# DLR-RB/QUEASARS

Hardware: AMD Instinct MI355X
Metric: circuit-evals/sec (EVQE population) at n qubits; achieved HBM GB/s vs roofline (higher is better)
Workload: dtype f64; 1 GPU; 20-qubit EVQE population=64 per GPU, 4 layers, random Ising Hamiltonian (210 terms), fp64 (BASELINE.json configs[1]); n_qubits=20, population_per_gpu=64, layers=4, pauli_terms=210, parallelism=1 GPU

## Files before the change

include/qsv.h:

```cpp
#ifndef QSV_H
#define QSV_H

#include <stddef.h>
#include <stdint.h>

#ifdef __cplusplus
extern "C" {
#endif

typedef struct qsv_handle qsv_t;

enum { QSV_OP_ID = 0, QSV_OP_U = 1, QSV_OP_CU3 = 2 };
enum { QSV_F64 = 0, QSV_F32 = 1 };
enum { QSV_NO_CONTROL = 0xFF };

enum {
    QSV_OK = 0,
    QSV_E_ARG = -1,
    QSV_E_DEVICE = -2,
    QSV_E_STATE = -3,
    QSV_E_UNSUPPORTED = -4
};

typedef struct qsv_op {
    uint8_t kind;
    uint8_t target;
    uint8_t control;
    uint8_t flags;
    int32_t p_theta, p_phi, p_lambda;
    double theta, phi, lambda;
} qsv_op;

typedef struct qsv_plan_config {
    int32_t tile_bits;
    int32_t reg_bits;
    int32_t low_bits;
    int32_t group;
    int32_t exchange;
} qsv_plan_config;

typedef struct qsv_profile {
    uint64_t n_evals;
    uint64_t n_pass_launches;
    uint64_t n_state_passes;
    uint64_t n_gates;
    uint64_t state_bytes;
    double pass_ms;
    double expect_ms;
    double total_ms;
    double pass_window_ms;
    uint64_t moved_bytes;
    uint64_t kernel_launches[3];
    double kernel_ms[3];
    uint64_t kernel_bytes[3];
    uint64_t kernel_moved_bytes[3];
    double kernel_flops[3];
    uint64_t kernel_states[3];
} qsv_profile;


int qsv_create(int n_qubits, int dtype, int device, const qsv_plan_config* cfg , qsv_t** out);
void qsv_destroy(qsv_t* h);
const char* qsv_last_error(const qsv_t* h);
int qsv_set_stream(qsv_t* h, void* hip_stream);
int qsv_n_qubits(const qsv_t* h);


int qsv_set_operator(qsv_t* h, int n_terms, const uint64_t* x_mask, const uint64_t* z_mask,
                     const double* coeff_re, const double* coeff_im);


int qsv_circuit_create(qsv_t* h, int n_ops, const qsv_op* ops, int n_params, int* out_circuit_id);
int qsv_circuits_create(qsv_t* h, int n_circuits, const int64_t* op_offsets, const qsv_op* ops, const int* n_params,
                        int* out_circuit_ids);
int qsv_circuit_destroy(qsv_t* h, int circuit_id);

int qsv_prefix_create(qsv_t* h, int n_states, const int* circuit_ids, const int64_t* param_offsets, const double* params,
                      int* out_prefix_ids);
int qsv_prefix_destroy(qsv_t* h, int n_states, const int* prefix_ids);
int qsv_prefix_count(const qsv_t* h);
int qsv_circuit_create_on_prefix(qsv_t* h, int prefix_id, int n_ops, const qsv_op* ops, int n_params, int* out_circuit_id);
int qsv_circuits_create_on_prefixes(qsv_t* h, int n_circuits, const int64_t* op_offsets, const qsv_op* ops, const int* n_params,
                                    const int* prefix_ids, int* out_circuit_ids);

enum { QSV_ROUTE_ONE_TILE = 0, QSV_ROUTE_SPLIT_ONE_LAUNCH = 1, QSV_ROUTE_SPLIT = 2, QSV_ROUTE_PASSES = 3 };
typedef struct qsv_circuit_cost_t {
    int32_t route;
    int32_t n_keys;
    int32_t n_passes;
    int32_t on_kept_state;
    double microseconds;
} qsv_circuit_cost_t;
int qsv_circuit_cost(qsv_t* h, int circuit_id, qsv_circuit_cost_t* out);

typedef struct qsv_circuit_form_t {
    int32_t route;
    int32_t n_keys;
    int32_t n_virtual[2];
    int32_t amps_per_thread;
    int32_t halves;
    int32_t outer[2];
    int32_t one_launch;
    int32_t split_sampled;
    uint32_t mask_x, mask_y;
} qsv_circuit_form_t;
int qsv_circuit_form(qsv_t* h, int circuit_id, qsv_circuit_form_t* out);
int qsv_circuit_launch_form(qsv_t* h, int circuit_id, qsv_circuit_form_t* out);

int qsv_eval_circuits(qsv_t* h, int n_evals, const int* circuit_ids, const int64_t* param_offsets,
                      const double* params, double* out_expectations);

int qsv_eval_coalesced(qsv_t* h, int circuit_id, const double* params, int n_params, double window_us,
                       double* out_expectation);

int qsv_eval_begin(qsv_t* h, int n_evals, const int* circuit_ids, const int64_t* param_counts);
int qsv_eval_push(qsv_t* h, int first, int count, const double* values);
int qsv_eval_staging(qsv_t* h, int first, int count, double** values);
int qsv_eval_push_device(qsv_t* h, int first, int count, const double* device_values, void* ready_event);
int qsv_eval_end(qsv_t* h, double* out_expectations);
int qsv_eval_set_output(qsv_t* h, double* device_out);
int qsv_eval_results_seen(qsv_t* h);
typedef struct qsv_spsa_step_args {
    int32_t n_runs, width;
    double* x;
    uint8_t* active;
    int64_t* iterations;
    const double* delta_accept;
    const double* values;
    const double* delta_propose;
    double* points;
    double eps, lr;
    int32_t trust_region, maxiter;
    int32_t window;
    int32_t reserved;
    double min_rel;
    int64_t maxfev;
    double* previous;
    int64_t* n_values;
    double* changes;
} qsv_spsa_step_args;
int qsv_spsa_step(qsv_t* h, const qsv_spsa_step_args* args);
typedef struct qsv_nft_step_args {
    int32_t n_runs, width;
    int32_t columns_stride;
    int32_t reserved;
    double* x;
    const int32_t* sizes;
    const int32_t* columns;
    double* recycled;
    int32_t accept, accept_with_base;
    int64_t accept_iteration;
    int32_t propose, propose_with_base;
    int64_t propose_iteration;
    const double* values;
    double* points;
} qsv_nft_step_args;
int qsv_nft_step(qsv_t* h, const qsv_nft_step_args* args);
typedef struct qsv_adam_step_args {
    int32_t n_runs, width;
    int32_t columns_stride, grad_width;
    double* x;
    const int32_t* sizes;
    const int32_t* columns;
    double* m;
    double* v;
    const double* gradient;
    uint8_t* active;
    int64_t* iterations;
    double lr, beta_1, beta_2, one_minus_beta_1, one_minus_beta_2, eps, tol;
    double bias_1, bias_2;
    int64_t maxiter;
} qsv_adam_step_args;
int qsv_adam_step(qsv_t* h, const qsv_adam_step_args* args);
int qsv_eval_suggested_pushes(const qsv_t* h);
int qsv_group_size(const qsv_t* h);

int qsv_eval_batch(qsv_t* h, int n_evals, const int64_t* op_offsets, const qsv_op* ops,
                   const int64_t* param_offsets, const double* params, double* out_expectations);

int qsv_statevector(qsv_t* h, int circuit_id, const double* params, int n_params, double* out_re_im);

int qsv_probabilities(qsv_t* h, int circuit_id, const double* params, int n_params, double* out_probs);

int qsv_sample(qsv_t* h, int circuit_id, const double* params, int n_params, int shots, uint64_t seed,
               uint64_t* out_states);

int qsv_sample_batch(qsv_t* h, int n_evals, const int* circuit_ids, const int64_t* param_offsets, const double* params,
                     int shots, uint64_t seed, uint64_t* out_states, double* out_values );

int qsv_sample_cvar_batch(qsv_t* h, int n_evals, const int* circuit_ids, const int64_t* param_offsets, const double* params,
// ... 138 lines not shown
```

queasars_amd/_build.py:

```python

from __future__ import annotations

import os
import shutil
import subprocess
from pathlib import Path

PKG_DIR = Path(__file__).resolve().parent
CSRC = PKG_DIR / "csrc"
LIB_PATH = PKG_DIR / "libqsv.so"
PYHELP_PATH = PKG_DIR / "_qsvpyhelp.so"
SOURCES = ["kernels.hip", "qsv_api.hip", "plan.cpp", "split.cpp", "sort.hip", "gradient.hip", "value_cache.hip", "adjoint.hip", "adjoint_plan.cpp", "moments.hip", "covariance.hip", "overlap.hip"]
HEADERS = ["kernels.hpp", "plan.hpp", "split.hpp", "gradient.hpp", "value_cache.hpp", "adjoint.hpp", "adjoint_plan.hpp", "moments.hpp", "covariance.hpp", "overlap.hpp", "operator_row.hpp", "gate_loop_gen.inc", "../../include/qsv.h"]
ARCH = "gfx950"


def _hipcc() -> str:
    for cand in (os.environ.get("HIPCC"), shutil.which("hipcc"), "/opt/rocm/bin/hipcc"):
        if cand and Path(cand).exists():
            return cand
    raise RuntimeError("hipcc not found; libqsv cannot be built")


def have_hipcc() -> bool:
    try:
        _hipcc()
        return True
    except RuntimeError:
        return False


def pyhelp_stale() -> bool:
    src = CSRC / "pyhelp.c"
    return not PYHELP_PATH.exists() or PYHELP_PATH.stat().st_mtime < src.stat().st_mtime


def build_pyhelp(force: bool = False) -> "Path | None":
    import sysconfig

    src = CSRC / "pyhelp.c"
    if (PYHELP_PATH.exists() and not force and PYHELP_PATH.stat().st_mtime >= src.stat().st_mtime
            and (not LIB_PATH.exists() or PYHELP_PATH.stat().st_mtime >= LIB_PATH.stat().st_mtime)):
        return PYHELP_PATH
    include = sysconfig.get_paths().get("include")
    gcc = shutil.which("gcc")
    if not gcc or not include or not (Path(include) / "Python.h").exists():
        return None
    tmp = PYHELP_PATH.with_suffix(f".so.{os.getpid()}.tmp")
    if not LIB_PATH.exists():
        return None
    res = subprocess.run([gcc, "-O2", "-shared", "-fPIC", f"-I{include}", str(src), "-o", str(tmp), f"-L{PKG_DIR}", "-lqsv",
                          "-Wl,-rpath,$ORIGIN"], stdout=subprocess.PIPE, stderr=subprocess.STDOUT, text=True)
    if res.returncode != 0:
        tmp.unlink(missing_ok=True)
        return None
    os.replace(tmp, PYHELP_PATH)
    return PYHELP_PATH


def needs_build() -> bool:
    if not LIB_PATH.exists():
        return True
    built = LIB_PATH.stat().st_mtime
    return any((CSRC / f).resolve().stat().st_mtime > built for f in SOURCES + HEADERS)


def build(force: bool = False, verbose: bool = False, defines: tuple = (), lib_path: Path = LIB_PATH) -> Path:
    if not force and not defines and not needs_build():
        build_pyhelp(False)
        return LIB_PATH
    obj_dir = PKG_DIR / ("build" if not defines else "build_" + "".join(c if c.isalnum() else "_" for c in "_".join(defines).lower()))
    obj_dir.mkdir(exist_ok=True)
    hipcc = _hipcc()
    common = [f"--offload-arch={ARCH}", "-O3", "-std=c++17", "-fPIC", "-Wall", "-Wno-unused-function"]
    common += [f"-D{d}" for d in defines]
    procs = []
    objs = []
    for src in SOURCES:
        obj = obj_dir / (src + ".o")
        objs.append(str(obj))
        cmd = [hipcc, *common, "-c", str(CSRC / src), "-o", str(obj)]
        if src.endswith(".cpp"):
            cmd.insert(1, "-x")
            cmd.insert(2, "hip")
        if verbose:
            print(" ".join(cmd))
        procs.append((src, subprocess.Popen(cmd, stdout=subprocess.PIPE, stderr=subprocess.STDOUT, text=True)))
    for src, proc in procs:
        out, _ = proc.communicate()
        if proc.returncode != 0:
            raise RuntimeError(f"hipcc failed on {src}:\n{out}")
        if verbose and out.strip():
            print(out)
    tmp = lib_path.with_suffix(f".so.{os.getpid()}.tmp")
    link = [hipcc, f"--offload-arch={ARCH}", "-shared", "-fPIC", "-o", str(tmp), *objs]
    res = subprocess.run(link, stdout=subprocess.PIPE, stderr=subprocess.STDOUT, text=True)
    if res.returncode != 0:
        raise RuntimeError(f"link failed:\n{res.stdout}")
    os.replace(tmp, lib_path)
    if not defines:
        build_pyhelp(True)
    return lib_path


if __name__ == "__main__":
    print(build(force=True, verbose=True))
```

queasars_amd/_lib.py:

```python

from __future__ import annotations

import ctypes as C
import os
import threading
from pathlib import Path

import numpy as np

from queasars_amd import _build

QSV_OK, QSV_E_ARG, QSV_E_DEVICE, QSV_E_STATE, QSV_E_UNSUPPORTED = 0, -1, -2, -3, -4
QSV_F64, QSV_F32 = 0, 1


class QsvOp(C.Structure):
    _fields_ = [
        ("kind", C.c_uint8),
        ("target", C.c_uint8),
        ("control", C.c_uint8),
        ("flags", C.c_uint8),
        ("p_theta", C.c_int32),
        ("p_phi", C.c_int32),
        ("p_lambda", C.c_int32),
# ... 126 lines not shown
    _fields_ = [
        ("route", C.c_int32),
        ("n_keys", C.c_int32),
        ("n_virtual", C.c_int32 * 2),
        ("amps_per_thread", C.c_int32),
        ("halves", C.c_int32),
        ("outer", C.c_int32 * 2),
        ("one_launch", C.c_int32),
        ("split_sampled", C.c_int32),
        ("mask_x", C.c_uint32),
        ("mask_y", C.c_uint32),
    ]


class QsvGradientStats(C.Structure):

    _fields_ = [
        ("n_shifted", C.c_int64),
        ("n_chunks", C.c_int64),
        ("n_allocations", C.c_int64),
        ("scratch_bytes", C.c_int64),
    ]


class QsvGradientPlanStats(C.Structure):

    _fields_ = [
        ("n_shifted", C.c_int64),
        ("n_chunks", C.c_int64),
        ("n_runs", C.c_int64),
        ("n_host_waits", C.c_int64),
        ("table_bytes", C.c_int64),
    ]


class QsvAdjointStats(C.Structure):

    _fields_ = [
        ("n_gates", C.c_int64),
        ("n_runs", C.c_int64),
        ("n_state_sweeps", C.c_int64),
        ("scratch_bytes", C.c_int64),
        ("n_allocations", C.c_int64),
    ]


class QsvValueCacheStats(C.Structure):

    _fields_ = [
        ("entries", C.c_int64),
        ("slots", C.c_int64),
        ("samples_looked_up", C.c_int64),
        ("hits", C.c_int64),
        ("new_entries", C.c_int64),
        ("rehashes", C.c_int64),
        ("clears", C.c_int64),
    ]


ROUTE_NAMES = ("one tile", "split, one launch", "split", "gate passes")

assert C.sizeof(QsvOp) == 40

_P = C.c_void_p
SIGNATURES = {
    "qsv_version": (C.c_char_p, []),
    "qsv_create": (C.c_int, [C.c_int, C.c_int, C.c_int, C.POINTER(QsvPlanConfig), C.POINTER(_P)]),
    "qsv_destroy": (None, [_P]),
    "qsv_last_error": (C.c_char_p, [_P]),
    "qsv_set_stream": (C.c_int, [_P, _P]),
    "qsv_n_qubits": (C.c_int, [_P]),
    "qsv_set_operator": (C.c_int, [_P, C.c_int, _P, _P, _P, _P]),
    "qsv_circuit_create": (C.c_int, [_P, C.c_int, _P, C.c_int, C.POINTER(C.c_int)]),
    "qsv_circuits_create": (C.c_int, [_P, C.c_int, _P, _P, _P, _P]),
    "qsv_circuit_destroy": (C.c_int, [_P, C.c_int]),
    "qsv_prefix_create": (C.c_int, [_P, C.c_int, _P, _P, _P, _P]),
    "qsv_prefix_destroy": (C.c_int, [_P, C.c_int, _P]),
    "qsv_prefix_count": (C.c_int, [_P]),
    "qsv_circuit_create_on_prefix": (C.c_int, [_P, C.c_int, C.c_int, _P, C.c_int, C.POINTER(C.c_int)]),
    "qsv_circuits_create_on_prefixes": (C.c_int, [_P, C.c_int, _P, _P, _P, _P, _P]),
    "qsv_circuit_cost": (C.c_int, [_P, C.c_int, C.POINTER(QsvCircuitCost)]),
    "qsv_circuit_form": (C.c_int, [_P, C.c_int, C.POINTER(QsvCircuitForm)]),
    "qsv_circuit_launch_form": (C.c_int, [_P, C.c_int, C.POINTER(QsvCircuitForm)]),
    "qsv_eval_circuits": (C.c_int, [_P, C.c_int, _P, _P, _P, _P]),
    "qsv_eval_coalesced": (C.c_int, [_P, C.c_int, _P, C.c_int, C.c_double, C.POINTER(C.c_double)]),
    "qsv_eval_begin": (C.c_int, [_P, C.c_int, _P, _P]),
    "qsv_eval_push": (C.c_int, [_P, C.c_int, C.c_int, _P]),
    "qsv_eval_staging": (C.c_int, [_P, C.c_int, C.c_int, C.POINTER(_P)]),
    "qsv_eval_push_device": (C.c_int, [_P, C.c_int, C.c_int, _P, _P]),
    "qsv_spsa_step": (C.c_int, [_P, _P]),
    "qsv_nft_step": (C.c_int, [_P, _P]),
    "qsv_adam_step": (C.c_int, [_P, _P]),
    "qsv_eval_end": (C.c_int, [_P, _P]),
    "qsv_eval_set_output": (C.c_int, [_P, _P]),
    "qsv_eval_results_seen": (C.c_int, [_P]),
    "qsv_eval_suggested_pushes": (C.c_int, [_P]),
    "qsv_group_size": (C.c_int, [_P]),
    "qsv_eval_batch": (C.c_int, [_P, C.c_int, _P, _P, _P, _P, _P]),
    "qsv_statevector": (C.c_int, [_P, C.c_int, _P, C.c_int, _P]),
    "qsv_probabilities": (C.c_int, [_P, C.c_int, _P, C.c_int, _P]),
    "qsv_sample": (C.c_int, [_P, C.c_int, _P, C.c_int, C.c_int, C.c_uint64, _P]),
    "qsv_sample_batch": (C.c_int, [_P, C.c_int, _P, _P, _P, C.c_int, C.c_uint64, _P, _P]),
    "qsv_sample_cvar_batch": (C.c_int, [_P, C.c_int, _P, _P, _P, C.c_int, C.c_uint64, C.c_double, _P]),
    "qsv_exact_cvar_batch": (C.c_int, [_P, C.c_int, _P, _P, _P, C.c_double, _P]),
    "qsv_top_states": (C.c_int, [_P, C.c_int, _P, _P, _P, C.c_int, _P, _P, _P]),
    "qsv_cvar_device": (C.c_int, [_P, C.c_int, _P, C.c_int, _P, _P, C.c_int, C.c_uint64, C.c_double, _P, C.c_int, _P]),
    "qsv_value_cache_create": (C.c_int, [_P, C.c_int, C.c_int, _P]),
    "qsv_value_cache_destroy": (C.c_int, [_P, C.c_int]),
    "qsv_value_cache_clear": (C.c_int, [_P, C.c_int]),
    "qsv_value_cache_stats": (C.c_int, [_P, C.c_int, _P]),
    "qsv_sample_lookup": (C.c_int, [_P, C.c_int, C.c_int, _P, _P, _P, C.c_int, C.c_uint64, _P, _P]),
    "qsv_sample_lookup_finish": (C.c_int, [_P, C.c_int, C.c_int64, _P, C.c_double, _P, _P]),
    "qsv_gradient_describe": (C.c_int, [C.c_int, _P, C.c_int, _P]),
    "qsv_gradient_circuits": (C.c_int, [_P, C.c_int, _P, _P, _P, _P, _P, _P, _P]),
    "qsv_gradient_device": (C.c_int, [_P, C.c_int, _P, C.c_int, _P, _P, _P, _P, C.c_int, _P, _P]),
    "qsv_gradient_stats": (C.c_int, [_P, C.POINTER(QsvGradientStats)]),
    "qsv_gradient_plan_create": (C.c_int, [_P, C.c_int, _P, C.c_int, _P, _P, C.c_int, C.POINTER(C.c_int), C.POINTER(C.c_int64)]),
    "qsv_gradient_plan_run": (C.c_int, [_P, C.c_int, _P, _P, _P]),
    "qsv_gradient_plan_destroy": (C.c_int, [_P, C.c_int]),
    "qsv_gradient_plan_stats": (C.c_int, [_P, C.c_int, C.POINTER(QsvGradientPlanStats)]),
    "qsv_adjoint_describe": (C.c_int, [C.c_int, C.c_int, _P, C.c_int, C.c_int, _P, C.c_int, _P, _P, _P, C.POINTER(C.c_int64),
                                       C.POINTER(C.c_int32), C.POINTER(C.c_int32)]),
    "qsv_adjoint_gradient_circuits": (C.c_int, [_P, C.c_int, _P, _P, _P, _P, _P, _P, _P]),
    "qsv_adjoint_gradient_device": (C.c_int, [_P, C.c_int, _P, C.c_int, _P, _P, _P, _P, C.c_int, _P, _P]),
    "qsv_adjoint_stats": (C.c_int, [_P, C.POINTER(QsvAdjointStats)]),
    "qsv_variance_circuits": (C.c_int, [_P, C.c_int, _P, _P, _P, _P, _P]),
    "qsv_observables_covariance": (C.c_int, [_P, C.c_int, C.c_int, _P, _P, _P, _P, _P]),
    "qsv_overlap_circuits": (C.c_int, [_P, C.c_int, _P, C.c_int, C.c_int, _P, _P, _P, _P, _P]),
    "qsv_observables_create": (C.c_int, [_P, C.c_int, _P, _P, _P, _P, _P, C.POINTER(C.c_int)]),
    "qsv_observables_destroy": (C.c_int, [_P, C.c_int]),
    "qsv_eval_observables": (C.c_int, [_P, C.c_int, C.c_int, _P, _P, _P, _P]),
    "qsv_set_option": (C.c_int, [_P, C.c_char_p, C.c_int]),
    "qsv_fitness_table_wait": (C.c_int, [C.c_void_p, C.c_int, C.c_void_p, C.c_int, C.c_int, C.c_int, C.c_int64, C.c_int]),
    "qsv_replayed_pushes": (C.c_longlong, [_P]),
    "qsv_live_entries": (C.c_int, [C.c_int, C.c_uint, C.POINTER(C.c_int)]),
    "qsv_set_profiling": (C.c_int, [_P, C.c_int]),
    "qsv_get_profile": (C.c_int, [_P, C.POINTER(QsvProfile)]),
    "qsv_bench_gate": (C.c_int, [_P, C.c_int, C.c_int, C.c_double, C.c_double, C.c_double, C.c_int, C.POINTER(C.c_double)]),
    "qsv_bench_ops": (C.c_int, [_P, C.c_int, _P, C.c_int, C.POINTER(C.c_double), C.POINTER(C.c_int)]),
    "qsv_split_describe": (
        C.c_int,
        [C.c_int, C.c_int, _P, C.c_int, C.POINTER(C.c_uint64), _P, C.c_int, C.POINTER(C.c_int), _P, C.c_int, C.POINTER(C.c_int)],
    ),
    "qsv_split_describe_reduced": (
        C.c_int,
        [C.c_int, C.c_int, _P, C.c_int, C.POINTER(C.c_uint64), _P, C.c_int, C.POINTER(C.c_int), _P, C.c_int, C.POINTER(C.c_int),
         _P, _P, _P, _P],
    ),
    "qsv_plan_build": (
        C.c_int,
        [C.c_int, C.c_int, C.c_int, _P, C.POINTER(QsvPlanConfig), _P, C.c_size_t, C.POINTER(C.c_size_t)],
    ),
}

_lock = threading.Lock()
_lib = None


class QsvLibraryError(RuntimeError):
    """libqsv is missing or could not be loaded.  There is deliberately no fallback."""


def library_path() -> Path:
    override = os.environ.get("QSV_LIBRARY")
    return Path(override) if override else _build.LIB_PATH

# ... 38 lines not shown
```

queasars_amd/circuit_evaluation/circuit_evaluation.py:

```python

from __future__ import annotations

import ctypes as C
import os
import threading
import uuid
import weakref
from collections import OrderedDict
from itertools import count
from abc import ABC, abstractmethod
from typing import Optional, Sequence

from array import array

import numpy as np

from queasars_amd import _lib
from queasars_amd.circuit_evaluation.bitstring_evaluation import BitstringEvaluator
from queasars_amd.circuit_evaluation.expectation_calculation import (
    get_expectation_with_bitstring_evaluator,
    get_expectation_with_operator,
)
from queasars_amd.ir import OP_ID, QSV_OP_DTYPE, CircuitIR, PauliOperator

# ... 411 lines not shown
        for c in fresh:
            if c.n_qubits != self._n_qubits:
                raise ValueError(f"circuit has {c.n_qubits} qubits, the evaluator {self._n_qubits}")
        with self._reg_lock:
            fresh = [c for c in fresh if self._serial not in c._registered]
            continued = [c for c in fresh if c._kept_state is not None]
            if continued:
                fresh = [c for c in fresh if c._kept_state is None]
                if len(continued) >= 2:
                    self._register_continued(continued)
            if len(fresh) < 2:
                return
            joined = b"".join([c._bytes for c in fresh])
            ops = np.frombuffer(joined, dtype=QSV_OP_DTYPE) if joined else np.zeros(1, dtype=QSV_OP_DTYPE)
            offsets = np.zeros(len(fresh) + 1, dtype=np.int64)
            np.cumsum([len(c._bytes) for c in fresh], out=offsets[1:])
            offsets //= QSV_OP_DTYPE.itemsize
            counts = np.asarray([c.num_parameters for c in fresh], dtype=np.int32)
            out = np.zeros(len(fresh), dtype=np.int32)
            self._check(self._lib.qsv_circuits_create(self._handle, len(fresh), _lib.as_ptr(offsets), _lib.as_ptr(ops),
                                                      _lib.as_ptr(counts), _lib.as_ptr(out)))
            for c, cid in zip(fresh, out.tolist()):
                c._registered[self._serial] = cid
                self._watch(c, cid)

    def _register_continued(self, circuits: Sequence[CircuitIR]) -> None:
        joined = b"".join([c._bytes for c in circuits])
        ops = np.frombuffer(joined, dtype=QSV_OP_DTYPE) if joined else np.zeros(1, dtype=QSV_OP_DTYPE)
        offsets = np.zeros(len(circuits) + 1, dtype=np.int64)
        np.cumsum([len(c._bytes) for c in circuits], out=offsets[1:])
        offsets //= QSV_OP_DTYPE.itemsize
        counts = np.asarray([c.num_parameters for c in circuits], dtype=np.int32)
        states = np.asarray([self._kept_id(c._kept_state) for c in circuits], dtype=np.int32)
        out = np.zeros(len(circuits), dtype=np.int32)
        self._check(self._lib.qsv_circuits_create_on_prefixes(self._handle, len(circuits), _lib.as_ptr(offsets), _lib.as_ptr(ops),
                                                              _lib.as_ptr(counts), _lib.as_ptr(states), _lib.as_ptr(out)))
        for c, cid in zip(circuits, out.tolist()):
            c._registered[self._serial] = cid
            self._watch(c, cid)

    def _kept_id(self, kept: "KeptState") -> int:
        if kept._serial != self._serial or kept._id < 0:
            raise ValueError("the circuit continues a state that is not kept on this device (or was released)")
        return kept._id

    def keep_states(self, circuits: Sequence[CircuitIR], parameter_values: Sequence[Sequence[float]]) -> list[KeptState]:
        n = len(circuits)
        if len(parameter_values) != n:
            raise ValueError("circuits and parameter_values must have the same length")
        if n == 0:
            return []
        if any(c._kept_state is not None for c in circuits):
            raise ValueError("a kept state of a circuit that itself continues a kept state is not supported")
        self._register_many([c for c in circuits if self._serial not in c._registered])
        ids = np.fromiter((self.circuit_id(c) for c in circuits), dtype=np.int32, count=n)
        offsets, flat = _pack_batch(parameter_values, np.fromiter((c.num_parameters for c in circuits), dtype=np.int64, count=n))
        out = np.zeros(n, dtype=np.int32)
        with self._reg_lock:
            self._reap()
        self._check(self._lib.qsv_prefix_create(self._handle, n, _lib.as_ptr(ids), _lib.as_ptr(offsets), _lib.as_ptr(flat), _lib.as_ptr(out)))
        return [KeptState(self, pid) for pid in out.tolist()]

    def forget_last_batch(self) -> None:
        self._last_batch = None
        self._row_counts = None
        self._ids_address = None

    def kept_state_count(self) -> int:
        with self._reg_lock:
            self._reap()
        return int(self._lib.qsv_prefix_count(self._handle))

    def circuit_cost(self, circuit: CircuitIR) -> dict:
        cost = _lib.QsvCircuitCost()
        self._check(self._lib.qsv_circuit_cost(self._handle, self.circuit_id(circuit), C.byref(cost)))
        return {"route": _lib.ROUTE_NAMES[cost.route], "n_keys": cost.n_keys, "n_passes": cost.n_passes,
                "on_kept_state": bool(cost.on_kept_state), "microseconds": cost.microseconds}

    def circuit_form(self, circuit: CircuitIR) -> dict:
        return self._form(self._lib.qsv_circuit_form, circuit)

    def circuit_launch_form(self, circuit: CircuitIR) -> dict:
        return self._form(self._lib.qsv_circuit_launch_form, circuit)

    def _form(self, call, circuit: CircuitIR) -> dict:
        form = _lib.QsvCircuitForm()
        self._check(call(self._handle, self.circuit_id(circuit), C.byref(form)))
        return {"route": form.route, "n_keys": form.n_keys, "n_virtual": tuple(form.n_virtual),
                "amps_per_thread": form.amps_per_thread, "halves": bool(form.halves), "outer": tuple(form.outer),
                "one_launch": bool(form.one_launch), "split_sampled": bool(form.split_sampled), "mask_x": form.mask_x,
                "mask_y": form.mask_y}

    def _watch(self, circuit: CircuitIR, cid: int) -> None:
        ref = weakref.ref(circuit, self._gone)
        self._watched[id(ref)] = (ref, cid)

    def _reap(self) -> None:
        while self._dead:
            cid = self._dead.pop()
            if self._handle:
                self._lib.qsv_circuit_destroy(self._handle, cid)
        while self._dead_states:
            pid = C.c_int(self._dead_states.pop())
            if self._handle:
                self._lib.qsv_prefix_destroy(self._handle, 1, C.byref(pid))

    def _batch_metadata(self, circuits: Sequence[CircuitIR]) -> tuple[np.ndarray, np.ndarray, int]:
        n = len(circuits)
        cached = self._last_batch
        if cached is not None and cached[0][0] == CircuitIR.edits_of_registered:
            fast = _load_pyhelp_module()
            if fast is not None:
                if fast.same_objects(cached[1], circuits):
                    return cached[2], cached[3], cached[4]
            elif cached[0] == (CircuitIR.edits_of_registered, *map(id, circuits)):
                return cached[2], cached[3], cached[4]
        if self._dead or self._dead_states:
            with self._reg_lock:
                self._reap()
        self._register_many([c for c in circuits if self._serial not in c._registered])
        ids = np.fromiter((self.circuit_id(c) for c in circuits), dtype=np.int32, count=n)
        need = np.fromiter((c.num_parameters for c in circuits), dtype=np.int64, count=n)
        total = int(need.sum())
        self._last_batch = ((CircuitIR.edits_of_registered, *map(id, circuits)), list(circuits), ids, need, total)
        return ids, need, total

    def _batch_arguments(self, circuits: Sequence[CircuitIR], parameter_values: Sequence[Sequence[float]]) -> tuple[np.ndarray, np.ndarray, np.ndarray]:
        ids, need, _ = self._batch_metadata(circuits)
        return (ids, *_pack_batch(parameter_values, need))

    def results_seen(self) -> None:
        self._check(self._lib.qsv_eval_results_seen(self._handle))

    def expectation_values_to_device(
        self, circuits: Sequence[CircuitIR], parameter_values: Sequence[Sequence[float]], device_pointer: int
    ) -> None:
        n = len(circuits)
        if len(parameter_values) != n:
            raise ValueError("circuits and parameter_values must have the same length")
        if n == 0:
            return
        ids, need, total = self._batch_metadata(circuits)
        helper = None if os.environ.get("QSV_LIBRARY") else _load_pyhelp()
        if helper is not None:
            scratch = np.empty(total + 1, dtype=np.float64)
            self._check(helper.qsv_py_expectation_values_device(self._handle, n, ids.ctypes.data, need.ctypes.data,
                                                                parameter_values, scratch.ctypes.data, total,
                                                                C.c_void_p(device_pointer)))
            return
        counts = np.fromiter(map(len, parameter_values), dtype=np.int64, count=n)
        if (counts < need).any():
            i = int(np.argmax(counts < need))
            raise ValueError(f"circuit {i} needs {int(need[i])} parameter values, got {int(counts[i])}")
        lib, handle = self._lib, self._handle
        self._check(lib.qsv_eval_begin(handle, n, _lib.as_ptr(ids), _lib.as_ptr(counts)))
        rc = lib.qsv_eval_set_output(handle, C.c_void_p(device_pointer))
        if rc == _lib.QSV_OK:
            packed = _pack_slice(parameter_values, 0, n, int(counts.sum()))
            rc = lib.qsv_eval_push(handle, 0, n, _lib.as_ptr(packed))
        rc_end = lib.qsv_eval_end(handle, None)
        self._check(rc if rc != _lib.QSV_OK else rc_end)

    def expectation_values_of_device_parameters(
        self,
        circuits: Sequence[CircuitIR],
        device_pointer: int,
# ... 1332 lines not shown
```

queasars_amd/csrc/gen_gate_loop.py:

```python
#!/usr/bin/env python3

from __future__ import annotations

import sys
from pathlib import Path

OUT = Path(__file__).resolve().parent / "gate_loop_gen.inc"

import os

ABL = set(filter(None, os.environ.get("QSV_GEN_ABL", "").split(",")))

AMP0 = 8


def amp_re(e: int) -> str:
    return f"v[{AMP0 + 4 * e}:{AMP0 + 4 * e + 1}]"


def amp_im(e: int) -> str:
    return f"v[{AMP0 + 4 * e + 2}:{AMP0 + 4 * e + 3}]"


def amp_operands(nr: int) -> list[str]:
    outs = []
    for e in range(nr):
        outs.append(f'"+{{{amp_re(e)}}}"(amp[{e}].re)')
        outs.append(f'"+{{{amp_im(e)}}}"(amp[{e}].im)')
    return outs


MAT = {"A": 40, "B": 56}
DESC = {"A": 72, "B": 76}
SAVE = "s[80:81]"
T0 = "s82"
TP = "s[82:83]"
BASEP = "s[96:97]"
RP, MP, N = 84, 86, 88
CLOBBER_RANGE = list(range(40, 89)) + [96, 97]


def sreg2(base: int) -> str:
    return f"s[{base}:{base + 1}]"


def gate(lines: list[str], r: int, x: str, tag: str) -> None:
    m, d = MAT[x], DESC[x]
    w0, ct, cg = f"s{d}", f"s{d + 1}", f"s{d + 2}"
    cgpair = sreg2(d + 2)
    m00, m00i, m01r, m01i = sreg2(m), sreg2(m + 2), sreg2(m + 4), sreg2(m + 6)
    m10r, m10i, m11r, m11i = sreg2(m + 8), sreg2(m + 10), sreg2(m + 12), sreg2(m + 14)
    e = lines.append
    e(f"s_and_b64 {TP}, {BASEP}, {cgpair}")
    e(f"s_cmp_eq_u64 {TP}, {cgpair}")
    e(f"s_cbranch_scc0 Lskip{tag}_%=")
    e(f"v_and_b32 %[vt], {ct}, %[tid]")
    e(f"v_cmp_eq_u32 vcc, {ct}, %[vt]")
    e(f"s_and_saveexec_b64 {SAVE}, vcc")
    e(f"s_cbranch_execz Lrest{tag}_%=")
    e(f"s_bitcmp1_b32 {w0}, 24")
    e(f"s_cbranch_scc1 Lgen{tag}_%=")
    for general in (False, True):
        x = "g" if general else ""
        if general:
            e(f"Lgen{tag}_%=:")
        if r > 1:
            e(f"s_and_b32 {T0}, {w0}, 0xff")
            for j in range(r - 1):
                e(f"s_cmp_eq_u32 {T0}, {j}")
                e(f"s_cbranch_scc1 Lj{x}{j}{tag}_%=")
        order = [r - 1] + list(range(r - 1))
        for pos, j in enumerate(order):
            if j != r - 1:
                e(f"Lj{x}{j}{tag}_%=:")
            pair = 0
            for e0 in range(1 << r):
                if e0 & (1 << j):
                    continue
                e1 = e0 | (1 << j)
                a0r, a0i, a1r, a1i = amp_re(e0), amp_im(e0), amp_re(e1), amp_im(e1)
                if "pairtest" not in ABL:
                    e(f"s_bitcmp1_b32 {w0}, {16 + pair}")
                    e(f"s_cbranch_scc0 Ln{x}{j}_{pair}{tag}_%=")
                if "gatevalu" not in ABL:
                    e(f"v_mul_f64 %[p], {m10r}, {a0r}")
                    e(f"v_mul_f64 %[q], {m10r}, {a0i}")
                    e(f"v_mul_f64 %[u], {m00}, {a0r}")
                    e(f"v_mul_f64 %[w], {m00}, {a0i}")
                    e(f"v_fma_f64 %[p], -{m10i}, {a0i}, %[p]")
                    e(f"v_fma_f64 %[q], {m10i}, {a0r}, %[q]")
                    if general:
                        e(f"v_fma_f64 %[u], -{m00i}, {a0i}, %[u]")
                        e(f"v_fma_f64 %[w], {m00i}, {a0r}, %[w]")
                        e(f"v_fma_f64 %[p], {m11r}, {a1r}, %[p]")
                        e(f"v_fma_f64 %[q], {m11i}, {a1r}, %[q]")
                    e(f"v_fma_f64 %[u], {m01r}, {a1r}, %[u]")
                    e(f"v_fma_f64 %[w], {m01r}, {a1i}, %[w]")
                    if not general:
                        e(f"v_fma_f64 %[p], {m11r}, {a1r}, %[p]")
                        e(f"v_fma_f64 %[q], {m11i}, {a1r}, %[q]")
                    e(f"v_fma_f64 {a0r}, -{m01i}, {a1i}, %[u]")
                    e(f"v_fma_f64 {a0i}, {m01i}, {a1r}, %[w]")
                    e(f"v_fma_f64 {a1r}, -{m11i}, {a1i}, %[p]")
                    e(f"v_fma_f64 {a1i}, {m11r}, {a1i}, %[q]")
                e(f"Ln{x}{j}_{pair}{tag}_%=:")
                pair += 1
            if not (general and pos + 1 == len(order)):
                e(f"s_branch Lrest{tag}_%=")
    e(f"Lrest{tag}_%=:")
    e(f"s_mov_b64 exec, {SAVE}")
    e(f"Lskip{tag}_%=:")


def loop_body(r: int) -> list[str]:
    rp, mp = sreg2(RP), sreg2(MP)
    lines: list[str] = []
    e = lines.append
    e(f"s_mov_b64 {rp}, %[rp]")
    e(f"s_mov_b64 {mp}, %[mp]")
    e(f"s_mov_b32 s{N}, %[n]")
    e("s_mov_b32 s96, %[base]")
    e("s_not_b32 s97, %[base]")
    gate_loop_core(lines, r)
    return lines


def gate_loop_core(lines: list[str], r: int) -> None:
    a, b = MAT["A"], MAT["B"]
    da, db = DESC["A"], DESC["B"]
    rp, mp = sreg2(RP), sreg2(MP)
    n = f"s{N}"
    e = lines.append
    e(f"s_load_dwordx4 s[{da}:{da + 3}], {rp}, 0x0")
    e(f"s_load_dwordx16 s[{a}:{a + 15}], {mp}, 0x0")
    e("Lloop_%=:")
    e("s_waitcnt lgkmcnt(0)")
    e(f"s_load_dwordx4 s[{db}:{db + 3}], {rp}, 0x10")
    e(f"s_load_dwordx16 s[{b}:{b + 15}], {mp}, 0x40")
    gate(lines, r, "A", "a")
    e(f"s_sub_u32 {n}, {n}, 1")
    e(f"s_cmp_eq_u32 {n}, 0")
    e("s_cbranch_scc1 Ldone_%=")
    e("s_waitcnt lgkmcnt(0)")
    e(f"s_load_dwordx4 s[{da}:{da + 3}], {rp}, 0x20")
    e(f"s_load_dwordx16 s[{a}:{a + 15}], {mp}, 0x80")
    gate(lines, r, "B", "b")
    e(f"s_add_u32 s{RP}, s{RP}, 32")
    e(f"s_addc_u32 s{RP + 1}, s{RP + 1}, 0")
    e(f"s_add_u32 s{MP}, s{MP}, 128")
    e(f"s_addc_u32 s{MP + 1}, s{MP + 1}, 0")
    e(f"s_sub_u32 {n}, {n}, 1")
    e(f"s_cmp_lg_u32 {n}, 0")
    e("s_cbranch_scc1 Lloop_%=")
    e("Ldone_%=:")
    e("s_waitcnt lgkmcnt(0)")


def emit(r: int) -> str:
    nr = 1 << r
    out = []
    out.append(f"// R = {r}: {nr} amplitudes per thread")
    out.append("template <>")
    out.append(f"struct GateLoopF64<{r}> {{")
    out.append(
        f"    static __device__ __forceinline__ void run(cx<double> (&amp)[{nr}], cu32p rp, cf64p mp,\n"
        "                                               uint32_t n_gates, uint32_t base, uint32_t tid) {"
    )
    out.append("        // uniform by construction; say so to the compiler, which otherwise may hand a VGPR to an \"s\" operand")
    out.append("        base = __builtin_amdgcn_readfirstlane(base);")
    out.append("        n_gates = __builtin_amdgcn_readfirstlane(n_gates);")
    out.append("        double u, w, p, q;")
    out.append("        uint32_t vt;")
    out.append("        asm volatile(")
    for line in loop_body(r):
        out.append(f'            "{line}\\n\\t"')
    outs = amp_operands(nr)
    outs += ['[u] "=&v"(u)', '[w] "=&v"(w)', '[p] "=&v"(p)', '[q] "=&v"(q)', '[vt] "=&v"(vt)']
    out.append("            : " + ",\n              ".join(outs))
    out.append('            : [rp] "s"(rp), [mp] "s"(mp), [n] "s"(n_gates), [base] "s"(base), [tid] "v"(tid)')
    clob = ['"vcc"', '"scc"'] + [f'"s{i}"' for i in CLOBBER_RANGE]
    rows = [", ".join(clob[i : i + 12]) for i in range(0, len(clob), 12)]
    out.append("            : " + ",\n              ".join(rows) + ");")
    out.append("    }")
    out.append("};")
    return "\n".join(out)


def swap_case(lines: list[str], r: int, v: int, u: int) -> None:
    e = lines.append
    pairs = [(e0, e0 | (1 << v)) for e0 in range(1 << r) if not e0 & (1 << v)]
    regs = [(f"v{AMP0 + 4 * a + d}", f"v{AMP0 + 4 * b + d}") for a, b in pairs for d in range(4)]
    e("s_nop 1")
    if "swapvalu" in ABL:
        return
    if u >= 4:
        op = "v_permlane32_swap_b32" if u == 5 else "v_permlane16_swap_b32"
        for a, b in regs:
            e(f"{op} {a}, {b}")
    elif u >= 2:
        n = 1 << u
        upper, lower = ("0xa", "0x5") if u == 2 else ("0xc", "0x3")
        for i in range(0, len(regs), 2):
            chunk = regs[i : i + 2]
            temps = ["%[t0]", "%[t1]"]
            for (a, _b), t in zip(chunk, temps):
                e(f"v_mov_b32 {t}, {a}")
            for (a, b), _t in zip(chunk, temps):
                e(f"v_mov_b32_dpp {a}, {b} row_shr:{n} row_mask:0xf bank_mask:{upper}")
            for (_a, b), t in zip(chunk, temps):
                e(f"v_mov_b32_dpp {b}, {t} row_shl:{n} row_mask:0xf bank_mask:{lower}")
    else:
        perm = "quad_perm:[1,0,3,2]" if u == 0 else "quad_perm:[2,3,0,1]"
        e(f"v_and_b32 %[t0], {1 << u}, %[lane]")
        e("v_cmp_ne_u32 vcc, 0, %[t0]")
        for i in range(0, len(regs), 2):
            chunk = regs[i : i + 2]
            temps = ["%[t0]", "%[t1]"]
            for (_a, b), t in zip(chunk, temps):
                e(f"v_mov_b32_dpp {t}, {b} {perm} row_mask:0xf bank_mask:0xf")
            for (a, b), _t in zip(chunk, temps):
                e(f"v_cndmask_b32_dpp {b}, {a}, {b}, vcc {perm} row_mask:0xf bank_mask:0xf")
            for (a, _b), t in zip(chunk, temps):
                e(f"v_cndmask_b32 {a}, {a}, {t}, vcc")


def dispatch_tree(lines: list[str], lo: int, hi: int, labels: list[str], tag: str) -> None:
    if hi - lo == 1:
        lines.append(f"s_branch {labels[lo]}")
        return
    mid = (lo + hi) // 2
    lines.append(f"s_cmp_lt_u32 %[sel], {mid}")
    lines.append(f"s_cbranch_scc1 Lt{tag}{lo}_{mid}_%=")
    dispatch_tree(lines, mid, hi, labels, tag)
    lines.append(f"Lt{tag}{lo}_{mid}_%=:")
    dispatch_tree(lines, lo, mid, labels, tag)


def emit_swap(r: int) -> str:
    nr = 1 << r
    lines: list[str] = []
    e = lines.append
    cases = [(v, u) for v in range(r) for u in range(6)]
    labels = [f"Lc{v}_{u}_%=" for v, u in cases]
    dispatch_tree(lines, 0, len(cases), labels, "s")
    for (v, u), label in zip(cases, labels):
        e(f"{label}:")
        swap_case(lines, r, v, u)
        e("s_branch Lend_%=")
    e("Lend_%=:")
    out = []
    out.append(f"// R = {r}: lane swap of the {nr} amplitudes of a thread, both component planes (sel = 6 V + U < {6 * r})")
    out.append("template <>")
    out.append(f"struct SwapF64<{r}> {{")
    out.append(f"    static __device__ __forceinline__ void run(cx<double> (&amp)[{nr}], uint32_t sel, uint32_t lane) {{")
    out.append("        sel = __builtin_amdgcn_readfirstlane(sel);")
    out.append("        uint32_t t0, t1;")
    out.append("        asm volatile(")
    for line in lines:
        out.append(f'            "{line}\\n\\t"')
    outs = amp_operands(nr) + ['[t0] "=&v"(t0)', '[t1] "=&v"(t1)']
    out.append("            : " + ",\n              ".join(outs))
    out.append('            : [sel] "s"(sel), [lane] "v"(lane)')
    out.append('            : "vcc", "scc");')
    out.append("    }")
    out.append("};")
    return "\n".join(out)


RH, ROUNDS, FLAGS, T1, T2, T3 = 89, 90, 91, 83, 92, 93
SAVE2 = "s[94:95]"
NEXT_RP, NEXT_MP = "s[92:93]", "s[94:95]"
ROUND_CLOBBERS = range(40, 98)
WC, RC = 40, 56
K_THREAD_COLS = 9


def emit_rounds(r: int) -> str:
    nr = 1 << r
    rp, mp = sreg2(RP), sreg2(MP)
    lines: list[str] = []
    e = lines.append
    e(f"s_mov_b64 {rp}, %[rp]")
    e(f"s_mov_b64 {mp}, %[mp]")
    e(f"s_mov_b32 s{ROUNDS}, %[rounds]")
    e(f"s_mov_b32 s{FLAGS}, %[flags]")
    e("s_mov_b32 s96, %[base]")
    e("s_not_b32 s97, %[base]")
    e("Lround_%=:")
    e(f"s_load_dword s{RH}, {rp}, 0x0")
    e("s_waitcnt lgkmcnt(0)")
    e(f"s_bitcmp1_b32 s{RH}, 16")
    e("s_cbranch_scc1 Lexch_%=")
    e(f"s_bitcmp1_b32 s{RH}, 18")
    e("s_cbranch_scc1 Lswap_%=")
    e(f"s_add_u32 s{RP}, s{RP}, 4")
    e(f"s_addc_u32 s{RP + 1}, s{RP + 1}, 0")
    e("Lgates_%=:")
    e(f"s_and_b32 s{N}, s{RH}, 0xffff")
    e(f"s_cmp_eq_u32 s{N}, 0")
    e("s_cbranch_scc1 Lnext_%=")
    e(f"s_lshl_b32 s{T1}, s{N}, 4")
    e(f"s_add_u32 s92, s{RP}, s{T1}")
    e(f"s_addc_u32 s93, s{RP + 1}, 0")
    e(f"s_lshl_b32 s{T1}, s{N}, 6")
    e(f"s_add_u32 s94, s{MP}, s{T1}")
    e(f"s_addc_u32 s95, s{MP + 1}, 0")
    if "gateloop" not in ABL:
        gate_loop_core(lines, r)
    e(f"s_mov_b64 {rp}, {NEXT_RP}")
    e(f"s_mov_b64 {mp}, {NEXT_MP}")
    e("Lnext_%=:")
    e(f"s_sub_u32 s{ROUNDS}, s{ROUNDS}, 1")
    e(f"s_cmp_lg_u32 s{ROUNDS}, 0")
    e("s_cbranch_scc1 Lround_%=")
    e("s_branch Lfinish_%=")

    e("Lswap_%=:")
    e(f"s_load_dwordx4 s[40:43], {rp}, 0x4")
    e(f"s_add_u32 s{RP}, s{RP}, 20")
    e(f"s_addc_u32 s{RP + 1}, s{RP + 1}, 0")
    e("s_waitcnt lgkmcnt(0)")
    e("Lswapnext_%=:")
    e("s_cmp_eq_u32 s40, -1")
    e("s_cbranch_scc1 Lgates_%=")
    e(f"s_and_b32 {T0}, s40, 0xff")
    e(f"s_mul_i32 {T0}, {T0}, 6")
    e(f"s_bfe_u32 s{T1}, s40, 0x80008")
    e(f"s_add_u32 {T0}, {T0}, s{T1}")
    cases = [(v, u) for v in range(r) for u in range(6)]
    labels = [f"Lc{v}_{u}_%=" for v, u in cases]
    tree: list[str] = []
    dispatch_tree(tree, 0, len(cases), labels, "r")
    lines.extend(x.replace("%[sel]", T0) for x in tree)
    for (v, u), label in zip(cases, labels):
        e(f"{label}:")
        swap_case(lines, r, v, u)
        e("s_branch Lswapdone_%=")
    e("Lswapdone_%=:")
    e("s_mov_b32 s40, s41")
    e("s_mov_b32 s41, s42")
    e("s_mov_b32 s42, s43")
    e("s_mov_b32 s43, -1")
    e("s_branch Lswapnext_%=")

    e("Lexch_%=:")
    for base, off in ((WC, 4), (RC, 4 + 52)):
        e(f"s_load_dwordx8 s[{base}:{base + 7}], {rp}, {hex(off)}")
        e(f"s_load_dwordx4 s[{base + 8}:{base + 11}], {rp}, {hex(off + 32)}")
        e(f"s_load_dword s{base + 12}, {rp}, {hex(off + 48)}")
    e(f"s_add_u32 s{RP}, s{RP}, {4 + 104}")
    e(f"s_addc_u32 s{RP + 1}, s{RP + 1}, 0")
    e(f"s_bitcmp1_b32 s{RH}, 17")
    e(f"s_cselect_b32 s{T2}, 2, 1")
    e(f"s_and_b32 s{T2}, s{FLAGS}, s{T2}")
    e("s_cbranch_scc0 Lnobar_%=")
    e("s_waitcnt lgkmcnt(0)")
    e("s_barrier")
    e(f"s_andn2_b32 s{FLAGS}, s{FLAGS}, 2")
    e("Lnobar_%=:")
    e("s_waitcnt lgkmcnt(0)")
    e("v_mov_b32 %[vt], 0")
    e("v_mov_b32 %[t0], 0")
    for u in range(6):
        e(f"v_bfe_i32 %[t2], %[tid], {u}, 1")
        e(f"v_and_b32 %[t3], s{WC + u}, %[t2]")
        e("v_xor_b32 %[vt], %[vt], %[t3]")
        e(f"v_and_b32 %[t3], s{RC + u}, %[t2]")
        e("v_xor_b32 %[t0], %[t0], %[t3]")
    e(f"s_mov_b32 s{T2}, 0")
    e(f"s_mov_b32 s{T3}, 0")
    for u in range(6, K_THREAD_COLS):
        e(f"s_bitcmp1_b32 %[wave], {u - 6}")
        e(f"s_cselect_b32 s94, s{WC + u}, 0")
        e(f"s_cselect_b32 s95, s{RC + u}, 0")
        e(f"s_xor_b32 s{T2}, s{T2}, s94")
        e(f"s_xor_b32 s{T3}, s{T3}, s95")
    e(f"v_xor_b32 %[vt], s{T2}, %[vt]")
    e(f"v_xor_b32 %[t0], s{T3}, %[t0]")
    e("v_lshlrev_b32 %[vt], 3, %[vt]")
    e("v_lshlrev_b32 %[t0], 3, %[t0]")
    e("v_add_u32 %[vt], %[lds], %[vt]")
    e("v_add_u32 %[t0], %[lds], %[t0]")
    for v in range(r):
        e(f"s_lshl_b32 s{WC + K_THREAD_COLS + v}, s{WC + K_THREAD_COLS + v}, 3")
        e(f"s_lshl_b32 s{RC + K_THREAD_COLS + v}, s{RC + K_THREAD_COLS + v}, 3")

    def gray(i: int) -> int:
        return i ^ (i >> 1)

    def ctz(i: int) -> int:
        return (i & -i).bit_length() - 1

    def barrier_unless_intra(tag: str) -> None:
        e(f"s_bitcmp1_b32 s{RH}, 17")
        e(f"s_cbranch_scc1 Lib{tag}_%=")
        e("s_waitcnt lgkmcnt(0)")
        e("s_barrier")
        e(f"Lib{tag}_%=:")

    for plane, reg in (("re", amp_re), ("im", amp_im)):
        e(f"s_mov_b64 {SAVE2}, exec")
        e(f"s_and_b64 exec, exec, %[active]")
        e("v_mov_b32 %[t1], %[vt]")
        for i in range(nr):
            if i:
                e(f"v_xor_b32 %[t1], s{WC + K_THREAD_COLS + ctz(i)}, %[t1]")
            e(f"ds_write_b64 %[t1], {reg(gray(i))}")
        e(f"s_mov_b64 exec, {SAVE2}")
        barrier_unless_intra("w" + plane)
        e("v_mov_b32 %[t1], %[t0]")
        for i in range(nr):
            if i:
                e(f"v_xor_b32 %[t1], s{RC + K_THREAD_COLS + ctz(i)}, %[t1]")
            e(f"ds_read_b64 {reg(gray(i))}, %[t1]")
        if plane == "re":
            barrier_unless_intra("r" + plane)
    e("s_waitcnt lgkmcnt(0)")
    e(f"s_or_b32 s{FLAGS}, s{FLAGS}, 1")
    e(f"s_bitcmp1_b32 s{RH}, 17")
    e("s_cbranch_scc1 Lgates_%=")
    e(f"s_or_b32 s{FLAGS}, s{FLAGS}, 2")
    e("s_branch Lgates_%=")

    e("Lfinish_%=:")
    e(f"s_mov_b32 %[flags], s{FLAGS}")

    out = []
    out.append(f"// R = {r}: every round of a tile (LDS exchanges in mode 2, lane swaps, gates)")
    out.append("template <>")
    out.append(f"struct RoundLoopF64<{r}> {{")
    out.append(
        f"    static __device__ __forceinline__ void run(cx<double> (&amp)[{nr}], cu32p rp, cf64p mp, uint32_t n_rounds,\n"
        "                                               uint32_t base, uint32_t tid, uint32_t wave, uint64_t active,\n"
        "                                               uint32_t lds, uint32_t& flags) {"
    )
    out.append("        base = __builtin_amdgcn_readfirstlane(base);")
    out.append("        n_rounds = __builtin_amdgcn_readfirstlane(n_rounds);")
    out.append("        wave = __builtin_amdgcn_readfirstlane(wave);")
    out.append("        lds = __builtin_amdgcn_readfirstlane(lds);")
    out.append("        uint32_t fl = __builtin_amdgcn_readfirstlane(flags);")
    out.append("        double u, w, p, q;")
    out.append("        uint32_t vt, t0, t1, t2, t3;")
    out.append("        asm volatile(")
    for line in lines:
        out.append(f'            "{line}\\n\\t"')
    outs = amp_operands(nr)
    outs += ['[u] "=&v"(u)', '[w] "=&v"(w)', '[p] "=&v"(p)', '[q] "=&v"(q)', '[vt] "=&v"(vt)', '[t0] "=&v"(t0)',
             '[t1] "=&v"(t1)', '[t2] "=&v"(t2)', '[t3] "=&v"(t3)', '[flags] "+s"(fl)']
    out.append("            : " + ",\n              ".join(outs))
    out.append('            : [rp] "s"(rp), [mp] "s"(mp), [rounds] "s"(n_rounds), [base] "s"(base), [tid] "v"(tid), [wave] "s"(wave),\n'
               '              [active] "s"(active), [lds] "s"(lds), [lane] "v"(tid & 63u)')
    clob = ['"vcc"', '"scc"', '"memory"'] + [f'"s{i}"' for i in ROUND_CLOBBERS]
    rows = [", ".join(clob[i : i + 12]) for i in range(0, len(clob), 12)]
    out.append("            : " + ",\n              ".join(rows) + ");")
    out.append("        flags = fl;")
    out.append("    }")
    out.append("};")
    return "\n".join(out)


def amp32(e: int) -> str:
    return f"v[{AMP0 + 2 * e}:{AMP0 + 2 * e + 1}]"


def amp32_operands(nr: int) -> list[str]:
    outs = []
    for e in range(nr):
        outs.append(f'"+{{v{AMP0 + 2 * e}}}"(amp[{e}].re)')
        outs.append(f'"+{{v{AMP0 + 2 * e + 1}}}"(amp[{e}].im)')
    return outs


def vregs32(r: int) -> dict:
    base = AMP0 + 2 * (1 << r)
    names = {"m00": base, "m01": base + 2, "m10": base + 4, "m11": base + 6, "p": base + 8, "u": base + 10}
    scal = {"vt": base + 12, "t0": base + 13, "t1": base + 14, "t2": base + 15, "t3": base + 16}
    return {"pairs": names, "scal": scal, "last": base + 16}


def gate32(lines: list[str], r: int, x: str, tag: str) -> None:
    m, d = MAT[x], DESC[x]
    w0, ct = f"s{d}", f"s{d + 1}"
    cgpair = sreg2(d + 2)
    vr = vregs32(r)
    P = {k: f"v[{v}:{v + 1}]" for k, v in vr["pairs"].items()}
    vt = f"v{vr['scal']['vt']}"
    e = lines.append
    e(f"s_and_b64 {TP}, {BASEP}, {cgpair}")
    e(f"s_cmp_eq_u64 {TP}, {cgpair}")
    e(f"s_cbranch_scc0 Lskip{tag}_%=")
    e(f"v_and_b32 {vt}, {ct}, %[tid]")
    e(f"v_cmp_eq_u32 vcc, {ct}, {vt}")
    e(f"s_and_saveexec_b64 {SAVE}, vcc")
    e(f"s_cbranch_execz Lrest{tag}_%=")
    for i, name in enumerate(("m00", "m01", "m10", "m11")):
        P[name] = sreg2(m + 2 * i)
    if r > 1:
        e(f"s_and_b32 {T0}, {w0}, 0xff")
        for j in range(r - 1):
            e(f"s_cmp_eq_u32 {T0}, {j}")
            e(f"s_cbranch_scc1 Lj{j}{tag}_%=")
    order = [r - 1] + list(range(r - 1))
    first, second = "op_sel:[0,0] op_sel_hi:[0,1]", "op_sel:[1,1,0] op_sel_hi:[1,0,1] neg_lo:[1,0,0]"
    first3 = "op_sel:[0,0,0] op_sel_hi:[0,1,1]"
    for pos, j in enumerate(order):
        if j != r - 1:
            e(f"Lj{j}{tag}_%=:")
        pair = 0
        for e0 in range(1 << r):
            if e0 & (1 << j):
                continue
            e1 = e0 | (1 << j)
            a0, a1 = amp32(e0), amp32(e1)
            if "pairtest" not in ABL:
                e(f"s_bitcmp1_b32 {w0}, {16 + pair}")
                e(f"s_cbranch_scc0 Ln{j}_{pair}{tag}_%=")
            if "gatevalu" not in ABL:
                e(f"v_pk_mul_f32 {P['p']}, {P['m10']}, {a0} {first}")
                e(f"v_pk_mul_f32 {P['u']}, {P['m00']}, {a0} {first}")
                e(f"v_pk_fma_f32 {P['p']}, {P['m10']}, {a0}, {P['p']} {second}")
                e(f"v_pk_fma_f32 {P['u']}, {P['m00']}, {a0}, {P['u']} {second}")
                e(f"v_pk_fma_f32 {P['p']}, {P['m11']}, {a1}, {P['p']} {first3}")
                e(f"v_pk_fma_f32 {P['u']}, {P['m01']}, {a1}, {P['u']} {first3}")
                e(f"v_pk_fma_f32 {a0}, {P['m01']}, {a1}, {P['u']} {second}")
                e(f"v_pk_fma_f32 {a1}, {P['m11']}, {a1}, {P['p']} {second}")
            e(f"Ln{j}_{pair}{tag}_%=:")
            pair += 1
        if pos + 1 != len(order):
            e(f"s_branch Lrest{tag}_%=")
    e(f"Lrest{tag}_%=:")
    e(f"s_mov_b64 exec, {SAVE}")
    e(f"Lskip{tag}_%=:")


def gate_loop_core32(lines: list[str], r: int) -> None:
# ... 188 lines not shown
    e(f"s_mov_b64 {SAVE2}, exec")
    e("s_and_b64 exec, exec, %[active]")
    e(f"v_mov_b32 {t1}, {vt}")
    for i in range(nr):
        if i:
            e(f"v_xor_b32 {t1}, s{WC + K_THREAD_COLS + ctz(i)}, {t1}")
        e(f"ds_write_b64 {t1}, {amp32(gray(i))}")
    e(f"s_mov_b64 exec, {SAVE2}")
    e(f"s_bitcmp1_b32 s{RH}, 17")
    e("s_cbranch_scc1 Libw_%=")
    e("s_waitcnt lgkmcnt(0)")
    e("s_barrier")
    e("Libw_%=:")
    e(f"v_mov_b32 {t1}, {t0}")
    for i in range(nr):
        if i:
            e(f"v_xor_b32 {t1}, s{RC + K_THREAD_COLS + ctz(i)}, {t1}")
        e(f"ds_read_b64 {amp32(gray(i))}, {t1}")
    e("s_waitcnt lgkmcnt(0)")
    e(f"s_or_b32 s{FLAGS}, s{FLAGS}, 1")
    e(f"s_bitcmp1_b32 s{RH}, 17")
    e("s_cbranch_scc1 Lgates_%=")
    e(f"s_or_b32 s{FLAGS}, s{FLAGS}, 2")
    e("s_branch Lgates_%=")

    e("Lfinish_%=:")
    e(f"s_mov_b32 %[flags], s{FLAGS}")

    out = []
    out.append(f"// R = {r}: every round of a tile in single precision (LDS exchanges in mode 0, lane swaps, gates in packed arithmetic)")
    out.append("template <>")
    out.append(f"struct RoundLoopF32<{r}> {{")
    out.append(
        f"    static __device__ __forceinline__ void run(cx<float> (&amp)[{nr}], cu32p rp, cf64p mp, uint32_t n_rounds,\n"
        "                                               uint32_t base, uint32_t tid, uint32_t wave, uint64_t active,\n"
        "                                               uint32_t lds, uint32_t& flags) {"
    )
    out.append("        base = __builtin_amdgcn_readfirstlane(base);")
    out.append("        n_rounds = __builtin_amdgcn_readfirstlane(n_rounds);")
    out.append("        wave = __builtin_amdgcn_readfirstlane(wave);")
    out.append("        lds = __builtin_amdgcn_readfirstlane(lds);")
    out.append("        uint32_t fl = __builtin_amdgcn_readfirstlane(flags);")
    out.append("        asm volatile(")
    for line in lines:
        out.append(f'            "{line}\\n\\t"')
    outs = amp32_operands(nr) + ['[flags] "+s"(fl)']
    out.append("            : " + ",\n              ".join(outs))
    out.append('            : [rp] "s"(rp), [mp] "s"(mp), [rounds] "s"(n_rounds), [base] "s"(base), [tid] "v"(tid), [wave] "s"(wave),\n'
               '              [active] "s"(active), [lds] "s"(lds), [lane] "v"(tid & 63u)')
    first_free = AMP0 + 2 * nr
    clob = ['"vcc"', '"scc"', '"memory"'] + [f'"s{i}"' for i in ROUND_CLOBBERS] + [f'"v{i}"' for i in range(first_free, vr["last"] + 1)]
    rows = [", ".join(clob[i : i + 12]) for i in range(0, len(clob), 12)]
    out.append("            : " + ",\n              ".join(rows) + ");")
    out.append("        flags = fl;")
    out.append("    }")
    out.append("};")
    return "\n".join(out)


def render() -> str:
    head = (
        "// GENERATED by gen_gate_loop.py -- do not edit; regenerate with `python gen_gate_loop.py`.\n"
        "// fp64 gate loop of pass_kernel in gfx950 assembly: see the generator's docstring for the design.\n"
        "// Included inside namespace qsv by kernels.hip, after cx<> is defined.\n\n"
        "template <int R>\nstruct GateLoopF64;  // specialised below for R = 1 .. 4\n\n"
    )
    swap_head = (
        "\n\n// Lane swaps (plan.hpp \"swap\" rounds), see gen_gate_loop.py.\n"
        "template <int R>\nstruct SwapF64;  // specialised below for R = 1 .. 4\n\n"
    )
    rounds_head = (
        "\n\n// The whole round loop of a tile (exchange mode 2), see gen_gate_loop.py.\n"
        "template <int R>\nstruct RoundLoopF64;  // specialised below for R = 1 .. 4\n\n"
    )
    rounds32_head = (
        "\n\n// The whole round loop of a tile in single precision (exchange mode 0, packed arithmetic), see gen_gate_loop.py.\n"
        "template <int R>\nstruct RoundLoopF32;  // specialised below for R = 1 .. 4\n\n"
    )
    return (head + "\n\n".join(emit(r) for r in (1, 2, 3, 4)) + swap_head + "\n\n".join(emit_swap(r) for r in (1, 2, 3, 4))
            + rounds_head + "\n\n".join(emit_rounds(r) for r in (1, 2, 3, 4))
            + rounds32_head + "\n\n".join(emit_rounds32(r) for r in (1, 2, 3, 4)) + "\n")


if __name__ == "__main__":
    text = render()
    if len(sys.argv) > 1 and sys.argv[1] == "--check":
        sys.exit(0 if OUT.exists() and OUT.read_text() == text else 1)
    out = Path(sys.argv[2]) if len(sys.argv) > 2 and sys.argv[1] == "--out" else OUT
    if ABL and out == OUT:
        sys.exit("QSV_GEN_ABL is set: refusing to overwrite the shipped gate_loop_gen.inc (use --out)")
    out.write_text(text)
    print(f"wrote {out} ({len(text.splitlines())} lines)")
```

queasars_amd/csrc/kernels.hip:

```cpp
#include "kernels.hpp"
#include "plan.hpp"

#include <hip/hip_runtime.h>

#include <type_traits>
#include <utility>

namespace qsv {

template <typename real>
struct alignas(2 * sizeof(real)) cx {
    real re, im;
};

#if defined(__HIP_DEVICE_COMPILE__)
#define QSV_CONST_AS __attribute__((address_space(4)))
#else
#define QSV_CONST_AS
#endif
using cu32p = const QSV_CONST_AS uint32_t*;
using cf64p = const QSV_CONST_AS double*;
template <typename T>
__device__ __forceinline__ const QSV_CONST_AS T* as_constant(const T* p) {
    return (const QSV_CONST_AS T*)(p);
// ... 23 lines not shown
}

__device__ __forceinline__ constexpr int gray_index(int i) { return i ^ (i >> 1); }
__device__ __forceinline__ uint32_t gray_step(int i, uint32_t off, cu32p reg_cols) {
    return i == 0 ? off : off ^ reg_cols[__builtin_ctz(i)];
}

template <typename real, int R, int J, int C>
__device__ __forceinline__ void butterfly(cx<real> (&amp)[1 << R], const real (&m)[7]) {
    constexpr int tbit = 1 << J;
    constexpr int cbit = C >= 0 ? (1 << (C >= 0 ? C : 0)) : 0;
#pragma unroll
    for (int e0 = 0; e0 < (1 << R); ++e0) {
        if ((e0 & tbit) || (e0 & cbit) != cbit) continue;
        const real a0r = amp[e0].re, a0i = amp[e0].im, a1r = amp[e0 | tbit].re, a1i = amp[e0 | tbit].im;
        real u = m[1] * a1r;
        real w = m[1] * a1i;
        real p = m[5] * a1r;
        real q = m[5] * a1i;
        u = fma(-m[2], a1i, u);
        w = fma(m[2], a1r, w);
        p = fma(-m[6], a1i, p);
        q = fma(m[6], a1r, q);
        p = fma(m[3], a0r, p);
        q = fma(m[3], a0i, q);
        amp[e0 | tbit].re = fma(-m[4], a0i, p);
        amp[e0 | tbit].im = fma(m[4], a0r, q);
        amp[e0].re = fma(m[0], a0r, u);
        amp[e0].im = fma(m[0], a0i, w);
    }
}

template <typename real, int R, int J>
__device__ __forceinline__ void butterfly_general(cx<real> (&amp)[1 << R], const real (&m)[8], uint32_t pair_mask) {
    constexpr int tbit = 1 << J;
    int pair = 0;
#pragma unroll
    for (int e0 = 0; e0 < (1 << R); ++e0) {
        if (e0 & tbit) continue;
        if ((pair_mask >> pair) & 1u) {
            const real a0r = amp[e0].re, a0i = amp[e0].im, a1r = amp[e0 | tbit].re, a1i = amp[e0 | tbit].im;
            amp[e0].re = m[0] * a0r - m[1] * a0i + m[2] * a1r - m[3] * a1i;
            amp[e0].im = m[0] * a0i + m[1] * a0r + m[2] * a1i + m[3] * a1r;
            amp[e0 | tbit].re = m[4] * a0r - m[5] * a0i + m[6] * a1r - m[7] * a1i;
            amp[e0 | tbit].im = m[4] * a0i + m[5] * a0r + m[6] * a1i + m[7] * a1r;
        }
        ++pair;
    }
}
template <typename real, int R, int J>
struct GeneralDispatch {
    static __device__ __forceinline__ void run(int j, cx<real> (&amp)[1 << R], const real (&m)[8], uint32_t pair_mask) {
        if (j == J)
            butterfly_general<real, R, J>(amp, m, pair_mask);
        else
            GeneralDispatch<real, R, J - 1>::run(j, amp, m, pair_mask);
    }
};
template <typename real, int R>
struct GeneralDispatch<real, R, -1> {
    static __device__ __forceinline__ void run(int, cx<real> (&)[1 << R], const real (&)[8], uint32_t) {}
};

template <typename real, int R, int SEL>
struct ButterflyDispatch {
    static __device__ __forceinline__ void run(int sel, cx<real> (&amp)[1 << R], const real (&m)[7]) {
        if (sel == SEL) {
            constexpr int J = SEL / (R + 1), C = SEL % (R + 1) - 1;
            if constexpr (C != J) butterfly<real, R, J, C>(amp, m);
        } else {
            ButterflyDispatch<real, R, SEL - 1>::run(sel, amp, m);
        }
    }
};
template <typename real, int R>
struct ButterflyDispatch<real, R, -1> {
    static __device__ __forceinline__ void run(int, cx<real> (&)[1 << R], const real (&)[7]) {}
};

#ifdef QSV_GATE_LOOP_INC
#include QSV_GATE_LOOP_INC
#else
#include "gate_loop_gen.inc"
#endif

template <int U>
__device__ __forceinline__ void swap_words(uint32_t& a, uint32_t& b) {
    if constexpr (U == 5) {
        const auto r = __builtin_amdgcn_permlane32_swap(a, b, false, false);
        a = r[0];
        b = r[1];
    } else if constexpr (U == 4) {
        const auto r = __builtin_amdgcn_permlane16_swap(a, b, false, false);
        a = r[0];
        b = r[1];
    } else if constexpr (U <= 1) {
        constexpr int ctrl = U == 0 ? 0xB1 : 0x4E;
        const uint32_t pb = uint32_t(__builtin_amdgcn_update_dpp(0, int(b), ctrl, 0xF, 0xF, true));
        const uint32_t pa = uint32_t(__builtin_amdgcn_update_dpp(0, int(a), ctrl, 0xF, 0xF, true));
        const bool upper = (__lane_id() >> U) & 1u;
        a = upper ? pb : a;
        b = upper ? b : pa;
    } else {
        constexpr int n = 1 << U;
        constexpr int upper = U == 2 ? 0xA : 0xC;
        constexpr int lower = U == 2 ? 0x5 : 0x3;
        const uint32_t na = uint32_t(__builtin_amdgcn_update_dpp(int(a), int(b), 0x110 + n, 0xF, upper, false));
        const uint32_t nb = uint32_t(__builtin_amdgcn_update_dpp(int(b), int(a), 0x100 + n, 0xF, lower, false));
        a = na;
        b = nb;
    }
}

template <int U>
__device__ __forceinline__ void swap_reals(double& a, double& b) {
    uint32_t alo = uint32_t(__double2loint(a)), ahi = uint32_t(__double2hiint(a));
    uint32_t blo = uint32_t(__double2loint(b)), bhi = uint32_t(__double2hiint(b));
    swap_words<U>(alo, blo);
    swap_words<U>(ahi, bhi);
    a = __hiloint2double(int(ahi), int(alo));
    b = __hiloint2double(int(bhi), int(blo));
}
template <int U>
__device__ __forceinline__ void swap_reals(float& a, float& b) {
    uint32_t x = __float_as_uint(a), y = __float_as_uint(b);
    swap_words<U>(x, y);
    a = __uint_as_float(x);
    b = __uint_as_float(y);
}

template <typename real, int R, int V, int U>
__device__ __forceinline__ void swap_reg_lane(cx<real> (&amp)[1 << R]) {
#pragma unroll
    for (int e0 = 0; e0 < (1 << R); ++e0) {
        if (e0 & (1 << V)) continue;
        swap_reals<U>(amp[e0].re, amp[e0 | (1 << V)].re);
        swap_reals<U>(amp[e0].im, amp[e0 | (1 << V)].im);
    }
}

template <typename real, int R, int SEL>
struct SwapDispatch {
    static __device__ __forceinline__ void run(int sel, cx<real> (&amp)[1 << R]) {
        if (sel == SEL)
            swap_reg_lane<real, R, SEL / 6, SEL % 6>(amp);
        else
            SwapDispatch<real, R, SEL - 1>::run(sel, amp);
    }
};
template <typename real, int R>
struct SwapDispatch<real, R, -1> {
    static __device__ __forceinline__ void run(int, cx<real> (&)[1 << R]) {}
};

#ifdef QSV_STAMPS
#ifdef QSV_STAMPS_WAVE0
#define QSV_STAMP_WAVE_OK (tid < 64u)
#else
#define QSV_STAMP_WAVE_OK true
#endif
__device__ unsigned long long qsv_stamp_table[kStampPasses * kStampPhases];
#define QSV_STAMP_DECL unsigned long long st_acc[kStampPhases] = {}; unsigned long long st_last = qsv_stamp_now();
#define QSV_STAMP_FLUSH(row) do { \
        unsigned long long* tab = reinterpret_cast<unsigned long long*>(lds_raw); \
        __syncthreads(); \
        if (tid < kStampPhases) tab[tid] = 0; \
// ... 500 lines not shown
#pragma unroll
        for (int u = 0; u < int(kMaxThreadBits); ++u) {
            vr[u] = 1.0;
            vi[u] = 0.0;
            if (u < t) {
                const double* v = sv + 4 * uint32_t(__builtin_ctz(hw[kPassLoadColsOffset + u])) + 2 * ((i >> u) & 1u);
                vr[u] = v[0];
                vi[u] = v[1];
            }
        }
        double fr = 1.0, fi = 0.0;
#pragma unroll
        for (int u = 0; u < int(kMaxThreadBits); ++u) {
            const double nr = fr * vr[u] - fi * vi[u];
            fi = fr * vi[u] + fi * vr[u];
            fr = nr;
        }
        sd.ttr = fr;
        sd.tti = fi;
    }
#endif
    uint32_t tile_mask = 0;
#pragma unroll
    for (int j = 0; j < int(kMaxTileBits); ++j)
        if (j < k) tile_mask |= 1u << hw[kPassHeaderWords + j];
    const uint32_t all_qubits = n_qubits >= 32 ? 0xffffffffu : ((1u << n_qubits) - 1u);
    const uint32_t outside = all_qubits & ~tile_mask;
    const uint32_t n_tiles = 1u << (n_qubits - uint32_t(k));
    auto tile_base = [&](uint64_t base) {
#pragma unroll
        for (int j = 0; j < int(kMaxTileBits); ++j)
            if (j < k) {
                const uint32_t ps = hw[kPassHeaderWords + j];
                base = ((base >> ps) << (ps + 1)) | (base & ((uint64_t(1) << ps) - 1));
            }
        return base;
    };
    sd.base1 = n_tiles > 1 ? uint32_t(tile_base(1)) : 0u;
#pragma unroll
    for (uint32_t tile = 0; tile < 2; ++tile) {
        double fr = 1.0, fi = 0.0;
#ifndef QSV_ABL_PREP_TABLES
        if (outside && tile < n_tiles) {
            const uint64_t base = tile ? uint64_t(sd.base1) : 0u;
            for (uint32_t m = outside; m; m &= m - 1u) {
                const uint32_t q = uint32_t(__builtin_ctz(m));
                const double* v = sv + 4 * q + 2 * ((base >> q) & 1u);
                const double nr = fr * v[0] - fi * v[1];
                fi = fr * v[1] + fi * v[0];
                fr = nr;
            }
        }
#endif
        sd.tfr[tile] = fr;
        sd.tfi[tile] = fi;
    }
    QSV_PSTAMP(6);
    sd.n_real = n_real;
    sd.n_qubits = n_qubits;
    sd.pass_off = ch[kCircuitHeaderWords];
    sd.hdr = hdr;
    sd.mat_off = hw[1];
    sd.flags = hw[2];
    QSV_PSTAMP(7);
    return true;
}

template <typename real, bool REDUCED>
__device__ __forceinline__ void fused_factor_tail(const uint32_t* __restrict__ plan_arena, const EvalDesc& ev,
                                                  const cx<real>* __restrict__ slot_tables, uint64_t side_stride,
                                                  const double* __restrict__ diag, const PassScalars& a, unsigned char* lds,
                                                  uint32_t gram_waves, uint32_t lds_table, uint32_t halves_tile QSV_PSTAMP_PARAMS);

template <typename real, int R, int XMODE, bool FIRST, bool FUSED = false, bool REDUCED = false>
__global__ void __launch_bounds__(512, (Occupancy<R, XMODE, FIRST, FUSED>::waves_per_simd))
    pass_kernel(const uint32_t* __restrict__ plan_arena, const double* __restrict__ mats_all,
                const EvalDesc* __restrict__ evals, cx<real>* __restrict__ states, cx<real>* __restrict__ wtabs,
                const double* __restrict__ diag, double* __restrict__ partials, const PassScalars a) {
    using cxr = cx<real>;
    constexpr int NR = 1 << R;
    constexpr int ASH = Log2Size<real>::value + 1;
    constexpr int LSH = XMODE == 0 ? ASH : ASH - 1;
    extern __shared__ __align__(16) unsigned char lds_raw[];

    QSV_STAMP_DECL
#ifdef QSV_ABL_EMPTY
    if constexpr (FUSED) return;
#endif
    const bool tile_major = !FIRST && (a.mode & kModeTileMajor);
    const uint32_t block_x = tile_major ? blockIdx.y : blockIdx.x, grid_x = tile_major ? gridDim.y : gridDim.x;
    const uint32_t block_y = tile_major ? blockIdx.x : blockIdx.y;
    if constexpr (!FUSED) {
        if (__builtin_expect(a.mode & kModeMasked, 0)) {
            const size_t slot = size_t(block_y) + size_t(blockIdx.z) * a.region_stride;
            const bool prepares = FIRST && (a.mode & kModeFusedPrepare);
            const EvalDesc* d = (prepares ? a.host_evals : evals) + slot;
            if (!(d->flags & kEvalNull) && masked_out(a.active, a.active_stride, d->out_index)) {
                if (prepares && threadIdx.x == 0 && block_x == 0) a.evals_out[slot] = *d;
                return;
            }
        }
    }
    EvalDesc ev;
    const double* mats_base = mats_all;
    bool prepared_here = false;
    if constexpr (FIRST) prepared_here = a.mode & kModeFusedPrepare;
    bool side_prepared = false;
    [[maybe_unused]] SidePrep sprep = {};
    if (prepared_here) {
        const size_t slot = size_t(block_y) + size_t(blockIdx.z) * a.region_stride;
        ev = a.host_evals[slot];
        if (threadIdx.x == 0 && block_x == 0) a.evals_out[slot] = ev;
        if (ev.flags & kEvalNull) return;
        bool side_route = false;
        if constexpr (FUSED) side_route = (a.mode & kModeSidePrepare) && (a.mode & kModeFusedFactor) && (ev.flags & kEvalFused);
        if (side_route) {
            if constexpr (FUSED) {
                if (block_x > 0 && !(ev.flags & kEvalHalves)) return;
                uint32_t ch[kSidePrepHeaderWords];
                load_words<kSidePrepHeaderWords>(as_constant(plan_arena) + ev.plan_base, ch);
                if (block_x > 0 && (ch[2] != uint32_t(kFusedLdsRowsBits) || block_x > 1)) return;
#ifdef QSV_STAMPS
                QSV_STAMP(0);
                side_prepared = side_prepare(plan_arena, ev, ch, a.host_params, a.mats_out, reinterpret_cast<double*>(lds_raw), std::is_same<real, float>::value, sprep, st_acc, &st_last);
#else
                side_prepared = side_prepare(plan_arena, ev, ch, a.host_params, a.mats_out, reinterpret_cast<double*>(lds_raw), std::is_same<real, float>::value, sprep);
#endif
            }
        } else {
            const uint32_t* c0 = plan_arena + ev.plan_base;
            const uint32_t* p0 = c0 + c0[kCircuitHeaderWords];
            const uint32_t f0 = p0[2];
            const uint32_t tiles0 = (f0 & kPassCompactStore) ? 1u << ((f0 >> 8) & 0xffu) : 1u << (c0[2] - (p0[0] & 0xffu));
            if (block_x >= tiles0) return;
            if (FUSED && block_x > 0 && (ev.flags & kEvalFused) && !((ev.flags & kEvalHalves) && c0[2] == uint32_t(kFusedLdsRowsBits)) && (a.mode & kModeFusedFactor)) return;
        }
        if (!side_prepared) {
#ifdef QSV_STAMPS
            if (!side_route) QSV_STAMP(0);
            prepare_eval(plan_arena, ev, a.host_params, a.mats_out, reinterpret_cast<double*>(lds_raw), std::is_same<real, float>::value, st_acc, &st_last);
#else
            prepare_eval(plan_arena, ev, a.host_params, a.mats_out, reinterpret_cast<double*>(lds_raw), std::is_same<real, float>::value);
#endif
        }
        __builtin_amdgcn_s_waitcnt(0);
        __syncthreads();
        __builtin_amdgcn_s_dcache_inv();
        __builtin_amdgcn_s_waitcnt(0);
        asm volatile("" : "+s"(mats_base)::"memory");
        QSV_STAMP(13);
#ifdef QSV_ABL_AFTER_PREP
        if constexpr (FUSED) return;
#endif
    } else {
        cu32p e = as_constant(reinterpret_cast<const uint32_t*>(evals + block_y + size_t(blockIdx.z) * a.region_stride));
        ev.plan_base = e[0];
        ev.mat_base = e[1];
        ev.state_slot = e[2];
        ev.out_index = e[3];
        ev.flags = e[6];
        ev.split_base = e[7];
    }
    if (ev.flags & kEvalNull) return;
    const bool side = ev.flags & kEvalSide;
    cu32p cp = as_constant(plan_arena) + ev.plan_base;
    uint32_t n_passes, n_real, n_qubits, pass_off;
// ... 15 lines not shown
        hdr = sprep.hdr;
        pass_mat_off = sprep.mat_off;
        pass_flags = sprep.flags;
    } else {
        hdr = pp[0];
        pass_mat_off = pp[1];
        pass_flags = pp[2];
    }
    const int k = hdr & 0xff, t = (hdr >> 16) & 0xff, n_rounds = hdr >> 24;
    const uint32_t tid = threadIdx.x;
    const uint32_t tid_ext = tid | (~tid & ((1u << kMaxThreadBits) - 1u)) << kMaxThreadBits;
    const bool all_active = blockDim.x == (1u << t);
    const bool active = tid < (1u << t);
    const uint32_t wave = __builtin_amdgcn_readfirstlane(tid >> 6);
    const uint32_t wave_base = wave << 6;

    cu32p pos = pp + kPassHeaderWords;
    cu32p glr = pp + kPassLoadColsOffset + kMaxThreadBits;
    cu32p gsr = pp + kPassStoreColsOffset + kMaxThreadBits;
    cu32p rounds0 = pp + kPassRoundsOffset;
    cf64p mats0 = as_constant(mats_base) + ev.mat_base + size_t(pass_mat_off) * 8;
    cf64p vecs = as_constant(mats_base) + ev.mat_base + size_t(n_real) * 8;

    constexpr bool synth = FIRST;
    const bool last = a.pass_index + 1 == n_passes;
    const bool do_probs = last && (a.mode & kModeFinalProbs) && !side;
    const bool do_store = (!last || (a.mode & kModeFinalStore) || side) && !do_probs;
    const bool do_diag = last && (a.mode & kModeFinalDiag) && !side;
    cxr* __restrict__ wt0 = wtabs + uint64_t(ev.state_slot) * a.wtab_stride;
    cxr* __restrict__ st0 = side ? wt0 + ((ev.flags & kEvalSideB) ? a.wtab_stride >> 1 : 0)
                                 : states + uint64_t(ev.state_slot) * a.state_stride;
    const cxr* __restrict__ ld0 = st0;
    if constexpr (!FIRST)
        if ((ev.flags & kEvalPrefix) && a.pass_index == 0)
            ld0 = static_cast<const cxr*>(a.prefix_states) + uint64_t(ev.split_base) * a.state_stride;
    const bool wide = n_qubits + uint32_t(ASH) > 32u;
    const bool cstore = synth && (pass_flags & kPassCompactStore);
    const bool cload = !FIRST && a.pass_index == 1 && (a.mode & kModeSynthFirst) && (pass_flags & kPassCompactLoad);
    const uint32_t total_tiles = cstore ? 1u << ((pass_flags >> 8) & 0xffu) : 1u << (n_qubits - uint32_t(k));
    const bool streaming = (a.mode & kModeStreaming) && !cload && !cstore && !side;
#ifdef QSV_ABL_NO_THROUGH
    const bool through = false;
#else
    const bool through = FUSED && side && (ev.flags & kEvalFused) && (a.mode & kModeFusedFactor);
#endif
    const bool half_side = FUSED && through && (ev.flags & kEvalHalves) && n_qubits == uint32_t(kFusedLdsRowsBits);
    const bool table_in_lds = through && std::is_same<real, double>::value && (a.mode & kModeFusedLdsTable) &&
                              (n_qubits <= uint32_t(kFusedLdsTableBits) || (half_side && plan_arena[ev.split_base] < uint32_t(kFusedLdsRowsKeys)));
    bool table_lds_rows = false;
    if constexpr (FUSED && std::is_same<real, double>::value)
        table_lds_rows = through && (a.mode & kModeFusedLdsTable) && n_qubits == uint32_t(kFusedLdsRowsBits) &&
                         plan_arena[ev.split_base] == uint32_t(kFusedLdsRowsKeys) &&
                         (uint32_t(k) == uint32_t(kFusedLdsRowsBits) || half_side);

    const uint32_t tg = xor_columns(pp + kPassLoadColsOffset, tid, wave);
    const uint32_t sg = xor_columns(pp + kPassStoreColsOffset, tid, wave);

    cf64p thread_factor = vecs + 4 * size_t(n_qubits) + kMatPadDoubles;
    cf64p tile_factor = thread_factor + (size_t(2) << t);
    cu32p tile_info = reinterpret_cast<cu32p>(tile_factor + (size_t(2) << (n_qubits - uint32_t(k))) +
                                              size_t(a.pass_index) * (size_t(2) << (n_qubits - uint32_t(k))));
    double ttr = 1.0, tti = 0.0;
    if (side_prepared) {
        ttr = sprep.ttr;
        tti = sprep.tti;
    } else if (synth && active) {
        ttr = thread_factor[2 * tid];
        tti = thread_factor[2 * tid + 1];
    }
    const bool sweeps = FUSED && side && (ev.flags & kEvalFused) && !half_side && (a.mode & kModeFusedFactor);
    const uint32_t tile0 = block_x, tile_step = sweeps ? 1u : grid_x;
    if (tile0 >= total_tiles) return;
    const uint32_t n_tiles = sweeps ? total_tiles
                             : (total_tiles - tile0 + tile_step - 1) / tile_step < a.tiles_per_block
                                 ? (total_tiles - tile0 + tile_step - 1) / tile_step
                                 : a.tiles_per_block;
    uint32_t wthr = 0, fthr = 0;
    if (cload) {
        wthr = xor_columns(pp + kPassCompactWCols, tid, wave);
        fthr = xor_columns(pp + kPassCompactFCols, tid, wave);
    }
    cxr amp[NR];
    double acc = 0.0;
    uint32_t xflags = 0;
    const uint64_t active_mask = __ballot(active);
    bool lds_dirty = false;
    bool cross_pending = false;

    if constexpr (!FIRST) {
        if (a.dephase && (block_x & 1u))
            for (uint32_t i = 0; i < a.dephase; ++i) __builtin_amdgcn_s_sleep(127);
    }
#ifdef QSV_TIMELINE
    unsigned long long* tl_rec = nullptr;
    if constexpr (!FIRST) {
        uint32_t slot = 0;
        if (threadIdx.x == 0) slot = atomicAdd(&qsv_timeline_count, 1u);
        slot = __builtin_amdgcn_readfirstlane(slot);
        if (threadIdx.x < 64 && slot < kTimelineWgs) {
            tl_rec = qsv_timeline + size_t(slot) * kTimelineWords;
            if (threadIdx.x == 0) {
                const uint32_t hw = __builtin_amdgcn_s_getreg((31 << 11) | 4), xcc = __builtin_amdgcn_s_getreg((3 << 11) | 20);
                tl_rec[0] = uint64_t(hw) | uint64_t(xcc) << 32;
                tl_rec[1] = uint64_t(block_x) | uint64_t(a.pass_index) << 32 | uint64_t(block_y) << 40;
                tl_rec[2] = n_tiles;
                tl_rec[3] = qsv_realtime_now();
            }
        }
    }
#endif
    QSV_STAMP(0);
    for (uint32_t j = 0; j < n_tiles; ++j) {
        QSV_TL(0);
        uint32_t ti[4];
        const bool second_tile = side_prepared && tile0 + j * tile_step != 0u;
        if (side_prepared) {
            ti[0] = second_tile ? sprep.base1 : 0u;
            ti[1] = ti[2] = ti[3] = 0u;
        } else {
            load_words<4>(tile_info + 4 * size_t(tile0 + j * tile_step), ti);
        }
        const uint64_t base = uint64_t(ti[0]) | uint64_t(ti[1]) << 32;
        uint32_t tgv = tg, sgv = sg;
        asm volatile("" : "+v"(tgv), "+v"(sgv));
        if constexpr (synth) {
            double tfr, tfi;
            if (side_prepared) {
                tfr = second_tile ? sprep.tfr[1] : sprep.tfr[0];
                tfi = second_tile ? sprep.tfi[1] : sprep.tfi[0];
            } else {
                tfr = cstore ? 1.0 : tile_factor[2 * size_t(tile0 + j * tile_step)];
                tfi = cstore ? 0.0 : tile_factor[2 * size_t(tile0 + j * tile_step) + 1];
            }
            amp[0].re = real(tfr * ttr - tfi * tti);
            amp[0].im = real(tfr * tti + tfi * ttr);
#pragma unroll
            for (int v = 0; v < R; ++v) {
                const uint32_t q = __builtin_ctz(glr[v]);
                const real v0r = real(vecs[4 * q]), v0i = real(vecs[4 * q + 1]);
                const real v1r = real(vecs[4 * q + 2]), v1i = real(vecs[4 * q + 3]);
#pragma unroll
                for (int e = 0; e < (1 << v); ++e) {
                    const cxr x = amp[e];
                    amp[e | (1 << v)].re = x.re * v1r - x.im * v1i;
                    amp[e | (1 << v)].im = x.re * v1i + x.im * v1r;
                    amp[e].re = x.re * v0r - x.im * v0i;
                    amp[e].im = x.re * v0i + x.im * v0r;
                }
            }
        } else {
            const uint32_t wbase = ti[2], fbase = ti[3];
            if (active) {
                if (!wide || cload) {
                    const unsigned char* tile = reinterpret_cast<const unsigned char*>(cload ? wt0 : ld0 + base);
                    cu32p rcols = cload ? pp + kPassCompactWCols + kMaxThreadBits : glr;
                    uint32_t ob = (cload ? wbase ^ wthr : tgv) << ASH;
#pragma unroll
                    for (int i = 0; i < NR; ++i) {
                        if (i) ob ^= rcols[__builtin_ctz(i)] << ASH;
#ifndef QSV_ABL_NOLOAD
                        if (streaming) {
                            typedef real vec2 __attribute__((ext_vector_type(2)));
                            const vec2 v = __builtin_nontemporal_load(reinterpret_cast<const vec2*>(tile + ob));
                            amp[gray_index(i)].re = v.x;
                            amp[gray_index(i)].im = v.y;
                        } else {
                            amp[gray_index(i)] = *reinterpret_cast<const cxr*>(tile + ob);
                        }
#else
                        amp[gray_index(i)].re = real(ob);
                        amp[gray_index(i)].im = real(i);
#endif
                    }
                } else {
                    uint32_t off = tgv;
#pragma unroll
                    for (int i = 0; i < NR; ++i) {
                        off = gray_step(i, off, glr);
                        amp[gray_index(i)] = ld0[base + off];
                    }
                }
#ifndef QSV_ABL_NOF
                if (cload) {
                    const unsigned char* ftab = reinterpret_cast<const unsigned char*>(
                        mats_base + ev.mat_base + size_t(n_real) * 8 + 4 * size_t(n_qubits) + kMatPadDoubles + (size_t(2) << t));
                    cu32p frc = pp + kPassCompactFCols + kMaxThreadBits;
                    const uint32_t fo = (fbase ^ fthr) << 4;
                    constexpr int HB = NR > 1 ? NR / 2 : 1;
#pragma unroll
                    for (int h = 0; h < NR / HB; ++h) {
                        uint32_t fh = h ? fo ^ (frc[R - 1] << 4) : fo;
                        double fr[HB], fi[HB];
#pragma unroll
                        for (int i = 0; i < HB; ++i) {
                            if (i) fh ^= frc[__builtin_ctz(i)] << 4;
                            fr[gray_index(i)] = *reinterpret_cast<const double*>(ftab + fh);
                            fi[gray_index(i)] = *reinterpret_cast<const double*>(ftab + fh + 8);
                        }
#pragma unroll
                        for (int e = 0; e < HB; ++e) {
                            const double wr = double(amp[h * HB + e].re), wi = double(amp[h * HB + e].im);
                            amp[h * HB + e].re = real(wr * fr[e] - wi * fi[e]);
                            amp[h * HB + e].im = real(wr * fi[e] + wi * fr[e]);
                        }
                    }
                }
#endif
                __builtin_amdgcn_s_waitcnt(0x0F70);
            }
        }

        QSV_STAMP(1);
        QSV_TL(1);
        cu32p rp = rounds0;
        cf64p mp = mats0;
#if !defined(QSV_STAMPS) || defined(QSV_STAMPS_ASM)
        constexpr bool kAsmRounds = (std::is_same<real, double>::value && XMODE == 2 && R <= 4) ||
                                    (std::is_same<real, float>::value && XMODE == 0 && R <= 4);
#else
        constexpr bool kAsmRounds = false;
#endif
        if constexpr (kAsmRounds) {
            if (n_rounds > 0) {
                if constexpr (std::is_same<real, double>::value)
                    RoundLoopF64<R>::run(amp, rp, mp, uint32_t(n_rounds), uint32_t(base), tid_ext, wave, active_mask,
                                         uint32_t(uintptr_t(lds_raw)), xflags);
                else
                    RoundLoopF32<R>::run(amp, rp, mp, uint32_t(n_rounds), uint32_t(base), tid_ext, wave, active_mask,
                                         uint32_t(uintptr_t(lds_raw)), xflags);
            }
            QSV_STAMP(10);
        } else
        for (int m = 0; m < n_rounds; ++m) {
            const uint32_t rh = rp[0];
            const int n_gates = rh & 0xffff;
            rp += 1;
            if ((rh >> 16) & 1u) {
                cu32p wc = rp;
                cu32p rc = rp + kColumnWords;
                rp += kExchangeWords;
                const uint32_t wt = xor_columns(wc, tid, wave) << LSH, rt = xor_columns(rc, tid, wave) << LSH;
                cu32p wrc = wc + kMaxThreadBits;
                cu32p rrc = rc + kMaxThreadBits;
                const bool intra = (rh >> 17) & 1u;
                if (intra ? cross_pending : lds_dirty) {
                    lds_barrier();
                    cross_pending = false;
                }
                if constexpr (XMODE == 0) {
                    QSV_STAMP(2);
                    if (active) {
{
                            uint32_t o = wt;
#pragma unroll
                            for (int i = 0; i < NR; ++i) {
                                if (i) o ^= wrc[__builtin_ctz(i)] << LSH;
                                const int e = gray_index(i);
                                *reinterpret_cast<cxr*>(lds_raw + o) = amp[e];
                            }
                        }
                    }
                    if (!intra) lds_barrier();
                    {
{
                            uint32_t o = rt;
#pragma unroll
                            for (int i = 0; i < NR; ++i) {
                                if (i) o ^= rrc[__builtin_ctz(i)] << LSH;
                                const int e = gray_index(i);
                                amp[e] = *reinterpret_cast<const cxr*>(lds_raw + o);
                            }
                        }
                    }
                } else if constexpr (XMODE == 1) {
                    QSV_STAMP(2);
                    unsigned char* pim = lds_raw + (size_t(sizeof(real)) << (hdr & 0xff));
                    if (active) {
{
                            uint32_t o = wt;
#pragma unroll
                            for (int i = 0; i < NR; ++i) {
                                if (i) o ^= wrc[__builtin_ctz(i)] << LSH;
                                const int e = gray_index(i);
                                *reinterpret_cast<real*>(lds_raw + o) = amp[e].re; *reinterpret_cast<real*>(pim + o) = amp[e].im;
                            }
                        }
                    }
                    if (!intra) lds_barrier();
                    {
{
                            uint32_t o = rt;
#pragma unroll
                            for (int i = 0; i < NR; ++i) {
                                if (i) o ^= rrc[__builtin_ctz(i)] << LSH;
                                const int e = gray_index(i);
                                amp[e].re = *reinterpret_cast<const real*>(lds_raw + o); amp[e].im = *reinterpret_cast<const real*>(pim + o);
                            }
                        }
                    }
                } else {
                    QSV_STAMP(2);
                    if (active) {
{
                            uint32_t o = wt;
#pragma unroll
                            for (int i = 0; i < NR; ++i) {
                                if (i) o ^= wrc[__builtin_ctz(i)] << LSH;
// ... 3305 lines not shown
```

queasars_amd/csrc/kernels.hpp:

```cpp
#pragma once

#include <hip/hip_runtime.h>

#include <cstdint>

#include "../../include/qsv.h"

namespace qsv {

struct EvalDesc {
    uint32_t plan_base;
    uint32_t mat_base;
    uint32_t state_slot;
    uint32_t out_index;
    uint32_t param_base;
    uint32_t n_params;
    uint32_t flags;
    uint32_t split_base;
};
constexpr uint32_t kEvalSide = 1u, kEvalSideB = 2u, kEvalNull = 4u;
constexpr uint32_t kEvalFused = 8u;
constexpr uint32_t kEvalPrefix = 16u;
constexpr uint32_t kEvalHalves = 32u;
constexpr int kSideExtraBits = 4;
constexpr int kSideMaxOwnBits = 16;
constexpr uint32_t kNoSideDiag = 0xffffffffu;
constexpr uint32_t kSplitLoopCols = 4, kSplitLoopPos = 9, kSplitMaskX = 14, kSplitMaskY = 15, kSplitLaneTable = 16, kSplitWaveTable = 144,
                   kSplitChunkLow = 160, kSplitChunkHigh = 416, kSplitSideDiag = 672, kSplitReduced = 674, kSplitReducedSlots = 676,
                   kSplitBlockWords = 680;
constexpr int kSplitLoopBits = 5, kSplitMaxLoopX = 2;
constexpr uint32_t kSplitFlags = 3, kSplitSwapXY = 1u;

enum PassMode : uint32_t {
    kModeSynthFirst = 1u,
    kModeFinalStore = 2u,
    kModeFinalDiag = 4u,
    kModeDirectResult = 32u,
    kModeFinalProbs = 64u,
    kModeStreaming = 16u,
    kModeSidesOnly = 128u,
    kModeFusedFactor = 256u,
    kModeFusedLdsTable = 512u,
    kModeTileMajor = 1024u,
    kModeFusedPrepare = 8u,
    kModeMasked = 2048u,
    kModeSidePrepare = 4096u,
    kModeFusedReduced = 8192u,
    kModeFusedLive = 16384u,
};
inline __host__ __device__ void live_entry_rows(uint32_t pi, uint32_t* ja_out, uint32_t* jb_out) {
    uint32_t ja = pi, jb = pi;
    if (pi >= 8u) {
        const uint32_t o = (pi - 8u) >> 1;
        ja = (o >= 7u) + (o >= 13u) + (o >= 18u) + (o >= 22u) + (o >= 25u) + (o >= 27u);
        jb = ja + 1u + o - ja * (15u - ja) / 2u;
    }
    *ja_out = ja;
    *jb_out = jb;
}
inline __host__ __device__ bool live_entry(uint32_t key_mask, uint32_t pi, uint32_t* rank_out) {
    uint32_t ja, jb;
    live_entry_rows(pi, &ja, &jb);
    if (rank_out) {
        uint32_t rank = 0;
        for (uint32_t below = 0; below < pi; ++below) {
            uint32_t a, b;
            live_entry_rows(below, &a, &b);
            rank += ((a ^ b) & key_mask) == 0u ? 1u : 0u;
        }
        *rank_out = rank;
    }
    return ((ja ^ jb) & key_mask) == 0u;
}
inline __host__ __device__ uint32_t live_key_mask(uint32_t reduced_x, uint32_t reduced_y) {
    auto of_side = [](uint32_t word) {
        const uint32_t n_final = word & 3u;
        return (n_final > 0u ? 1u << (word >> 4 & 3u) : 0u) | (n_final > 1u ? 1u << (word >> 6 & 3u) : 0u) | (n_final > 2u ? 1u << (word >> 8 & 3u) : 0u);
    };
    return of_side(reduced_x) | of_side(reduced_y);
}
struct ActiveMask {
    const uint8_t* flags = nullptr;
    uint32_t stride = 1;
};
#if defined(__HIPCC__)
__device__ __forceinline__ bool masked_out(const uint8_t* flags, uint32_t stride, uint32_t eval) {
    return flags != nullptr && flags[eval / stride] == 0;
}
#endif

struct PassArgs {
    const uint32_t* plan;
    const double* mats;
    const EvalDesc* evals;
    void* states;
    void* wtab;
    const double* diag;
    double* partials;
    uint64_t state_stride;
    uint64_t wtab_stride;
    uint32_t pass_index;
    uint32_t mode;
    uint32_t tiles_per_block;
    uint32_t region_stride;
    const EvalDesc* host_evals;
    EvalDesc* evals_out;
    const double* host_params;
    double* mats_out;
    double* result_out;
    uint32_t partial_chunks;
    const double* quad;
    double* factor_scratch;
    uint32_t* factor_counters;
    uint32_t n_full;
    const void* prefix_states;
    uint32_t dephase;
    const double* side_diag;
    ActiveMask active;
};
constexpr size_t kFusedFactorLdsBytes = 8 * (18 * 64 + 64) * sizeof(double) + 64;
constexpr int kFusedLdsTableBits = 12;
constexpr size_t kFusedLdsTableOffset = ((kFusedFactorLdsBytes + 1023) / 1024) * 1024;
constexpr size_t kFusedLdsTableEnd = kFusedLdsTableOffset + (size_t(16) << kFusedLdsTableBits);
constexpr int kFusedLdsRowsBits = 13, kFusedLdsRowsKeys = 3;
constexpr size_t kFusedLdsRowPitch = (size_t(1) << (kFusedLdsRowsBits - kFusedLdsRowsKeys)) + 1;
constexpr size_t kFusedLdsRowsDstage = ((kFusedLdsRowPitch * 8 * 16 + 127) / 128) * 128;
constexpr size_t kFusedLdsRowsEnd = kFusedLdsRowsDstage + 8 * 64 * sizeof(double) + 64;
constexpr size_t kFusedHalvesImport = kFusedLdsRowPitch * 4 * 16;
constexpr size_t kFusedHalvesImportPitch = (size_t(1) << (kFusedLdsRowsBits - kFusedLdsRowsKeys - 1)) + 1;
static_assert(kFusedHalvesImport + kFusedHalvesImportPitch * 4 * 16 <= kFusedLdsRowsDstage, "the imported rows end before the staged values of D");
constexpr uint32_t kFactorCountersPerSlot = 4;
// ... 148 lines not shown
```

queasars_amd/csrc/qsv_api.hip:

```cpp
#include <hip/hip_runtime.h>
#include <immintrin.h>

#include <algorithm>
#include <atomic>
#include <chrono>
#include <cmath>
#include <cstdio>
#include <condition_variable>
#include <cstring>
#include <functional>
#include <memory>
#include <mutex>
#include <string>
#include <thread>
#include <unordered_map>
#include <vector>

#include "../../include/qsv.h"
#include "adjoint.hpp"
#include "moments.hpp"
#include "covariance.hpp"
#include "overlap.hpp"
#include "gradient.hpp"
#include "value_cache.hpp"
// ... 139 lines not shown
    int log2_slots = 0, log2_max_slots = 0;
    uint64_t* d_keys = nullptr;
    double* d_vals = nullptr;
    DeviceBuffer d_sample_slot, d_miss_slots, d_counters;
    uint64_t* h_miss = nullptr;
    size_t h_miss_bytes = 0;
    double* h_values = nullptr;
    size_t h_values_bytes = 0;
    uint32_t* h_counters = nullptr;
    int64_t entries = 0;
    bool pending = false;
    int64_t pending_evals = 0, pending_missing = 0;
    int pending_shots = 0;
    int64_t samples_looked_up = 0, hits = 0, new_entries = 0, rehashes = 0, clears = 0;
};

struct qsv_handle {
    int n = 0, dtype = 0, device = 0;
    PlanConfig cfg;
    Geometry geo;
    int group = 1;
    size_t amp_bytes = 16;
    hipStream_t stream = nullptr;
    bool own_stream = false;
    std::vector<hipStream_t> side_streams;
    int n_lane_streams = 0;
    int aux_stream = -1;
    int chain_stream = -1;
    uint64_t epoch = 1;
    bool repeat_enabled = true;
    bool replay_enabled = true;
    uint64_t replayed_pushes = 0;
    struct HostTiming {
        bool on = false, in_push = false;
        uint64_t calls = 0, replays = 0;
        double begin_us = 0, push_us = 0, launch_us = 0, end_us = 0, copy_us = 0;
    } timing;
    bool chain_enabled = true;
    bool fused_lds_table = true;
    bool side_prepare = true;
    int n_cus = 256;
    int max_grid_y = 65535, device_max_grid_y = 65535;
    bool poll_results = true;
    hipStream_t work = nullptr;
    hipEvent_t ev_join = nullptr;
    int n_streams = 2;
    bool split_enabled = true;
    bool split_sampling = true;
    bool factor_enabled = true;
    bool fused_factor = true;
    int split_max_keys = 5;
    bool quadratic = false;
    DeviceBuffer d_quad;
    DeviceBuffer d_fterms;
    uint32_t n_fterms = 0;
    DeviceBuffer d_fpart;
    DeviceBuffer d_factor;
    DeviceBuffer d_factor_count;
    DeviceBuffer d_factor_big;
    DeviceBuffer d_factor_big_count;
    uint32_t stream_mode = 0;
    mutable std::mutex mu;
    std::atomic<std::thread::id> batch_owner{};

    int n_terms = 0;
    bool diagonal = false;
    bool has_diag_part = false;
    int n_groups = 0;
    DeviceBuffer d_z, d_cre, d_diag, d_term_partials, d_groups, d_term_odd;
    DeviceBuffer d_order, d_sorted;
    bool order_valid = false;
    int pauli_nb = 0;

    std::unordered_map<int, Circuit> circuits;
    int next_circuit_id = 1;
    std::unordered_map<int, PrefixState> prefixes;
    int next_prefix_id = 1;
    DeviceBuffer d_prefix;
    DeviceBuffer d_sdiag;
    size_t sdiag_used = 0;
    bool side_diag = true;
    bool final_controls = true;
    bool live_entries = true;
    bool sides_r3 = true;
    size_t prefix_slots = 0;
    std::vector<uint32_t> prefix_free;
    size_t prefix_used = 0;
    std::unordered_map<std::string, int> inline_cache;
    std::unordered_map<int, ObservableSet> obs_sets;
    int next_obs_id = 1;
    DeviceBuffer d_obs_partials, d_obs_values;
    std::unique_ptr<WorkerPool> pool;
    std::mutex pool_mu;

    struct CoalesceRequest {
        int circuit_id = 0;
        const double* params = nullptr;
        int n_params = 0;
        double value = 0.0;
        int rc = QSV_OK;
        std::string err;
        bool done = false;
    };
    std::mutex cq_mu;
    std::condition_variable cq_cv;
    std::vector<CoalesceRequest*> cq;
    std::atomic<size_t> cq_count{0};
    bool cq_collecting = false;
    size_t cq_expected = 0;
    uint64_t cq_batches = 0;

    DeviceBuffer d_arena;
    size_t arena_used_words = 0;
    DeviceBuffer d_states;
    DeviceBuffer d_wtab;
    uint64_t wtab_stride = 0;
    DeviceBuffer d_side;
    uint64_t side_stride = 0;
    int side_slots = 0;
    DeviceBuffer d_batch;
    DeviceBuffer d_mats;
    int tiles_per_block = 1;
    int tiles_per_block_later = 1;
    DeviceBuffer d_partials;
    DeviceBuffer d_out;
    DeviceBuffer d_scratch;
    void* h_batch = nullptr;
    size_t h_batch_bytes = 0;
    void* d_ship = nullptr;
    bool bar_ship = false;
    std::vector<char> ship_shadow;
    uint32_t* h_stage = nullptr;
    size_t h_stage_words = 0;
    double* h_out = nullptr;
    bool repeat_device_descs = true;
    const void* dev_params_checked = nullptr;
    double* out_target = nullptr;
    bool async_pending = false;
    void* h_samples = nullptr;
    size_t h_samples_bytes = 0;
    size_t h_out_count = 0;

    struct Batch {
        bool open = false;
        std::vector<Circuit*> circs;
        std::vector<uint32_t> param_base;
        std::vector<uint32_t> n_params;
        size_t desc_bytes = 0;
        size_t pushed = 0;
        std::vector<std::pair<hipEvent_t, hipEvent_t>> pass_events, exp_events;
        std::vector<std::pair<hipEvent_t, hipEvent_t>> launch_events[3];
        hipEvent_t ev0 = nullptr, ev1 = nullptr;
        bool split_any = false;
        bool reduced = false;
        std::vector<char> split;
        bool cont_any = false;
        size_t snap_n_cont = 0;
        std::vector<uint32_t> eval_at;
        int ways = 1;
        unsigned used_mask = 0;
        bool aux_plain = false;
        bool chain_now = false;
        bool chain_crossed = false;
        bool sentinels = false;
        std::vector<int> cur_ids, snap_ids;
        std::vector<int64_t> cur_counts, snap_counts;
// ... 684 lines not shown
        const size_t want = std::max(need * 2, size_t(1) << 16);
        QSV_HIP(h, hipHostMalloc(reinterpret_cast<void**>(&h->h_stage), want * 4, hipHostMallocDefault));
        h->h_stage_words = want;
    } else {
        h->host_waits += 1;
        QSV_HIP(h, hipStreamSynchronize(h->stream));
    }
    size_t cur = 0;
    std::vector<SideDiagJob> jobs;
    for (Circuit* c : fresh) {
        if (c->split.ok) {
            uint32_t* blk = c->plan.words.data() + c->split.off_block;
            blk[kSplitSideDiag] = blk[kSplitSideDiag + 1] = kNoSideDiag;
            if (h->side_diag && side_diag_doubles(c))
                for (uint32_t xy = 0; xy < 2; ++xy) {
                    blk[kSplitSideDiag + xy] = uint32_t(h->sdiag_used);
                    jobs.push_back(SideDiagJob{uint32_t(h->sdiag_used), blk[kSplitMaskX + xy], blk[1 + xy]});
                    h->sdiag_used += size_t(1) << blk[1 + xy];
                }
            if (c->reduced.ok) {
                uint32_t* rblk = c->plan.words.data() + c->reduced.off_block;
                rblk[kSplitSideDiag] = rblk[kSplitSideDiag + 1] = kNoSideDiag;
                if (side_diag_doubles(c))
                    for (uint32_t xy = 0; xy < 2; ++xy) {
                        rblk[kSplitSideDiag + xy] = uint32_t(h->sdiag_used);
                        jobs.push_back(SideDiagJob{uint32_t(h->sdiag_used), c->reduced_mask[xy], rblk[1 + xy], c->reduced_top[xy]});
                        h->sdiag_used += size_t(1) << rblk[1 + xy];
                    }
            }
        }
        std::memcpy(h->h_stage + cur, c->plan.words.data(), c->plan.words.size() * 4);
        c->plan_base = uint32_t(h->arena_used_words + cur);
        cur += c->plan.words.size();
        c->uploaded = true;
    }
    QSV_HIP(h, hipMemcpyAsync(static_cast<uint32_t*>(h->d_arena.ptr) + h->arena_used_words, h->h_stage, need * 4,
                              hipMemcpyHostToDevice, h->stream));
    h->arena_used_words += need;
    if (getenv("QSV_ARENA_DEBUG"))
        fprintf(stderr, "plan arena: %zu fresh plans, %zu side tables of D (%zu doubles used of %zu), diag %p\n", fresh.size(), jobs.size(), h->sdiag_used,
                h->d_sdiag.bytes / 8, h->d_diag.ptr);
    for (size_t first = 0; first < jobs.size(); first += size_t(kSideDiagJobsPerLaunch)) {
        SideDiagJobs batch{};
        const int n_jobs = int(std::min(jobs.size() - first, size_t(kSideDiagJobsPerLaunch)));
        std::copy(jobs.begin() + long(first), jobs.begin() + long(first) + n_jobs, batch.job);
        QSV_HIP(h, launch_side_diag(static_cast<const double*>(h->d_diag.ptr), static_cast<double*>(h->d_sdiag.ptr), batch, n_jobs, h->stream));
    }
    if (!h->side_streams.empty()) {
        QSV_HIP(h, hipEventRecord(h->ev_join, h->stream));
        for (hipStream_t st : h->side_streams) QSV_HIP(h, hipStreamWaitEvent(st, h->ev_join, 0));
    }
    return QSV_OK;
}

int ensure_host_batch(qsv_t* h, size_t bytes) {
    if (h->h_batch_bytes >= bytes) return QSV_OK;
    if (h->h_batch) {
        QSV_HIP(h, sync_streams(h));
        QSV_HIP(h, hipHostFree(h->h_batch));
        h->h_batch = nullptr;
    }
    size_t want = std::max(bytes * 2, size_t(1) << 16);
    h->epoch += 1;
    QSV_HIP(h, hipHostMalloc(&h->h_batch, want, hipHostMallocDefault));
    h->h_batch_bytes = want;
    if (h->bar_ship) {
        if (h->d_ship) QSV_HIP(h, hipFree(h->d_ship));
        h->d_ship = nullptr;
        h->ship_shadow.clear();
        QSV_HIP(h, hipMalloc(&h->d_ship, want));
    }
    return QSV_OK;
}

const void* ship_base(const qsv_t* h) { return h->bar_ship ? h->d_ship : h->h_batch; }
const EvalDesc* descs_base(const qsv_t* h) {
    if (h->batch.repeat && !h->bar_ship && h->repeat_device_descs) return static_cast<const EvalDesc*>(h->d_batch.ptr);
    return static_cast<const EvalDesc*>(ship_base(h));
}
const double* params_base(const qsv_t* h) {
    if (h->batch.dev_params) return h->batch.dev_params;
    return reinterpret_cast<const double*>(static_cast<const char*>(h->h_batch) + h->batch.desc_bytes);
}

double* result_base(const qsv_t* h) { return h->out_target ? h->out_target : h->h_out; }

void record_args(qsv_t* h, LaunchEntry& e, const PassArgs& a) {
    e.a = a;
    e.host_evals_off = a.host_evals ? int64_t(a.host_evals - descs_base(h)) : -1;
    e.takes_params = a.host_params != nullptr;
    e.result_off = a.result_out ? int64_t(a.result_out - result_base(h)) : -1;
    if ((a.host_params && a.host_params != params_base(h)) || a.active.flags) record_spoil(h);
}

void record_pass(qsv_t* h, int r, dim3 grid, int threads, size_t lds, const PassArgs& a) {
    LaunchEntry* e = record_entry(h, LaunchEntry::Pass, ws(h));
    if (!e) return;
    record_args(h, *e, a);
    e->dtype = h->dtype;
    e->r = r;
    e->xmode = h->cfg.xmode;
    e->grid = grid;
    e->threads = threads;
    e->lds = lds;
}

int ensure_host_out(qsv_t* h, size_t count) {
    if (h->h_out_count >= count) return QSV_OK;
    if (h->h_out) {
        QSV_HIP(h, sync_streams(h));
        QSV_HIP(h, hipHostFree(h->h_out));
        h->h_out = nullptr;
    }
    size_t want = std::max(count * 2, size_t(256));
    QSV_HIP(h, hipHostMalloc(reinterpret_cast<void**>(&h->h_out), want * sizeof(double), hipHostMallocDefault));
    h->h_out_count = want;
    return QSV_OK;
}

struct EventPair {
    hipEvent_t a, b;
};


const SplitInfo& side_form(const qsv_t* h, const Circuit& c) { return h->batch.reduced && c.reduced.ok ? c.reduced : c.split; }

size_t mat_doubles_of(const qsv_t* h, const Circuit& c, bool split, int side) {
    if (!split)
        return mat_region_doubles(uint32_t(c.plan.stats.n_real_gates), uint32_t(h->n), h->geo.t, h->n - h->geo.k,
                                  c.plan.stats.n_passes);
    const SplitInfo& sp = side_form(h, c);
    return mat_region_doubles(uint32_t(sp.stats[side].n_real_gates), uint32_t(sp.n_virtual[side]), sp.t[side],
                              sp.outer[side], sp.stats[side].n_passes);
}

int ensure_factor_big(qsv_t* h, hipStream_t stream, bool in_push) {
    int rc = ensure(h, h->d_factor_big, factor_big_slot_doubles() * sizeof(double) * size_t(h->side_slots));
    if (rc || h->d_factor_big_count.ptr) return rc;
    const size_t cbytes = factor_big_slot_counters() * sizeof(uint32_t) * size_t(h->side_slots);
    if ((rc = ensure(h, h->d_factor_big_count, cbytes))) return rc;
    if (in_push) record_spoil(h);
    QSV_HIP(h, hipMemsetAsync(h->d_factor_big_count.ptr, 0, cbytes, stream));
    h->host_waits += 1;
    QSV_HIP(h, hipStreamSynchronize(stream));
    return QSV_OK;
}

struct SplitRule {
    bool allow = false;
    int max_keys = 3;
    bool reduced = false;
    bool takes(const Circuit& c) const { return allow && c.split.ok && c.split.n_keys <= max_keys && c.prefix_id < 0; }
    size_t count(const std::vector<Circuit*>& circs) const {
        return size_t(std::count_if(circs.begin(), circs.end(), [&](const Circuit* c) { return takes(*c); }));
    }
};

int batch_layout(qsv_t* h, const std::vector<Circuit*>& circs, const std::vector<int64_t>& n_params, SplitRule rule = {}) {
    auto splits = [&](const Circuit* c) { return rule.takes(*c); };
    qsv_handle::Batch& b = h->batch;
    const size_t n_evals = circs.size();
    int rc;
    h->epoch += 1;
    b.repeat = false;
    b.reduced = rule.reduced;
    b.record.entries.clear();
// ... 145 lines not shown
}

unsigned chunks_per_state(const qsv_t* h) {
    const unsigned tpb = unsigned(std::min<uint32_t>(uint32_t(h->tiles_per_block), h->geo.blocks_per_state));
    return h->geo.blocks_per_state / tpb;
}

unsigned partials_per_state(const qsv_t* h) { return chunks_per_state(h) * unsigned(h->geo.threads_launch / 64); }

hipError_t stamp(qsv_t* h, std::vector<std::pair<hipEvent_t, hipEvent_t>>& list, bool begin) {
    if (!h->profiling) return hipSuccess;
    if (begin) {
        std::pair<hipEvent_t, hipEvent_t> p{nullptr, nullptr};
        hipError_t e = hipEventCreate(&p.first);
        if (e != hipSuccess) return e;
        e = hipEventCreate(&p.second);
        if (e != hipSuccess) return e;
        list.push_back(p);
        return hipEventRecord(p.first, ws(h));
    }
    return hipEventRecord(list.back().second, ws(h));
}

bool factor_path(const qsv_t* h) { return h->factor_enabled && h->diagonal && h->quadratic && h->d_quad.ptr != nullptr && h->d_factor.ptr != nullptr; }

bool factor_terms_path(const qsv_t* h) { return h->factor_enabled && !h->diagonal && h->n_fterms > 0 && h->d_side.ptr != nullptr; }

bool fused_route(const qsv_t* h) { return factor_path(h) && h->d_factor_count.ptr != nullptr && h->fused_factor; }
bool reduced_route(const qsv_t* h) { return fused_route(h) && h->final_controls && h->d_diag.ptr != nullptr; }

enum class SplitUse { Expectation, Sampling, Observables };

SplitRule split_rule(const qsv_t* h, SplitUse use) {
    switch (use) {
    case SplitUse::Expectation:
        return {h->n_terms == 0 || h->diagonal || factor_terms_path(h), (h->n_terms == 0 || factor_path(h)) ? kMaxSplitKeys : 3};
    case SplitUse::Sampling:
        return {h->split_sampling, 3};
    case SplitUse::Observables:
        break;
    }
    return {h->factor_enabled && h->d_side.ptr != nullptr && h->n <= 32, 3};
}

size_t working_workgroups(const SplitInfo& sp) {
    return 2u + (sp.halves ? size_t(sp.n_virtual[0] == kFusedLdsRowsBits) + size_t(sp.n_virtual[1] == kFusedLdsRowsBits) : 0u);
}

int run_group(qsv_t* h, const std::vector<Circuit*>& circs, size_t first, size_t count, uint32_t mode) {
    const qsv_handle::Batch& b = h->batch;
    const bool batch_split = b.split_any && b.split.size() == circs.size();
    const bool reordered = (b.split_any || b.cont_any) && b.split.size() == circs.size();
    auto eval_of = [&](size_t pos) { return reordered ? size_t(b.eval_at[pos]) : pos; };
    size_t n_split = 0, n_cont = 0;
    int max_passes = 0;
    for (size_t i = 0; i < count; ++i) {
        const size_t e = eval_of(first + i);
        if (batch_split && b.split[e]) {
            n_split = i + 1;
        } else {
            max_passes = std::max(max_passes, circs[e]->plan.stats.n_passes);
            n_cont += circs[e]->prefix_id >= 0 ? 1 : 0;
        }
    }
    if (n_cont > 0) {
        if (n_cont != count) return fail(h, QSV_E_STATE, "internal: a launch group mixes evaluations on kept states with others");
        mode &= ~uint32_t(kModeSynthFirst | kModeFusedPrepare | kModeDirectResult);
    }
    const bool any_split = n_split > 0;
    if (b.reduced && (mode & kModeSidesOnly)) return fail(h, QSV_E_STATE, "internal: a batch laid out for reduced sides runs its sides only");
    const size_t n_plain = count - n_split;
    if (h->mask.flags) mode |= kModeMasked;
    PassArgs a{};
    a.active = h->mask;
    a.plan = static_cast<const uint32_t*>(h->d_arena.ptr);
    a.mats = static_cast<const double*>(h->d_mats.ptr);
    a.evals = batch_evals(h) + first;
    a.states = h->d_states.ptr;
    a.wtab = h->d_wtab.ptr;
    a.wtab_stride = h->wtab_stride;
    a.diag = static_cast<const double*>(h->d_diag.ptr);
    a.partials = static_cast<double*>(h->d_partials.ptr);
    a.state_stride = uint64_t(1) << h->n;
    a.mode = mode | h->stream_mode;
    a.prefix_states = h->d_prefix.ptr;
    a.side_diag = static_cast<const double*>(h->d_sdiag.ptr);
    {
        static const uint32_t dephase = getenv("QSV_DEPHASE") ? uint32_t(atoi(getenv("QSV_DEPHASE"))) : 0u;
        a.dephase = dephase;
    }
    const unsigned chunks = chunks_per_state(h);
    const unsigned tpb_later = unsigned(std::min<uint32_t>(uint32_t(h->tiles_per_block_later), h->geo.blocks_per_state));
    const unsigned chunks_later = std::max(1u, std::min(chunks, h->geo.blocks_per_state / std::max(1u, tpb_later)));
    a.partial_chunks = chunks;
    a.region_stride = uint32_t(circs.size());
    const uint64_t sweep = (uint64_t(1) << h->n) * h->amp_bytes;
    size_t n_unfused = n_split;
    const bool fuse_ok = fused_route(h) && !(mode & kModeSidesOnly);
    if (fuse_ok) {
        n_unfused = 0;
        while (n_unfused < n_split && !side_form(h, *circs[eval_of(first + n_unfused)]).fused) ++n_unfused;
    }
    const bool two_chains = b.chain_now && h->chain_stream != -1 && n_unfused > 0 && n_split > n_unfused && factor_path(h);
    hipStream_t const chain_st = h->chain_stream >= 0 ? h->side_streams[size_t(h->chain_stream)] : nullptr;
    if (any_split) {
        if (n_plain > 0) return fail(h, QSV_E_STATE, "internal: a launch group mixes split and ordinary evaluations");
        a.wtab = h->d_side.ptr;
        a.wtab_stride = h->side_stride;
        a.quad = static_cast<const double*>(h->d_quad.ptr);
        a.factor_scratch = static_cast<double*>(h->d_factor.ptr);
        a.factor_counters = static_cast<uint32_t*>(h->d_factor_count.ptr);
        a.n_full = uint32_t(h->n);
        a.result_out = h->out_target ? h->out_target : h->h_out;
        a.tiles_per_block = 1;
        a.host_params = params_base(h);
        a.mats_out = static_cast<double*>(h->d_mats.ptr);
        auto shape_of = [&](size_t lo, size_t hi, int* threads, size_t* lds, int* passes, unsigned* tiles) {
            int tile = 0, t = 0;
            *passes = 1;
            *tiles = 1;
            for (size_t i = lo; i < hi; ++i) {
                const SplitInfo& sp = side_form(h, *circs[eval_of(first + i)]);
                for (int s = 0; s < 2; ++s) {
                    tile = std::max(tile, sp.tile_bits[s]);
                    t = std::max(t, sp.t[s]);
                    *passes = std::max(*passes, sp.stats[s].n_passes);
                    *tiles = std::max(*tiles, 1u << sp.outer[s]);
                }
            }
            *threads = std::max(64, 1 << t);
            *lds = (size_t(1) << tile) * h->amp_bytes / (h->cfg.xmode == 2 ? 2 : 1);
        };
        auto at_least_four_waves = [](int threads) { return std::max(256, threads); };
        auto launch_sides = [&](size_t lo, size_t hi, uint32_t extra_mode, int r) -> int {
            int threads, passes;
            size_t lds;
            unsigned tiles;
            shape_of(lo, hi, &threads, &lds, &passes, &tiles);
            if (extra_mode & kModeFusedFactor) threads = at_least_four_waves(threads);
            bool any_halves = false, any_reduced = false;
            if (extra_mode & kModeFusedFactor)
                for (size_t i = lo; i < hi; ++i) {
                    const Circuit& c = *circs[eval_of(first + i)];
                    any_halves |= side_form(h, c).halves;
                    any_reduced |= &side_form(h, c) == &c.reduced;
                }
            a.tiles_per_block = (extra_mode & kModeFusedFactor) ? tiles : 1u;
            const unsigned grid_x = (extra_mode & kModeFusedFactor) ? (any_halves ? 2u : 1u) : tiles;
            a.evals = batch_evals(h) + first + lo;
            a.host_evals = descs_base(h) + first + lo;
            a.evals_out = static_cast<EvalDesc*>(h->d_batch.ptr) + first + lo;
            for (int p = 0; p < passes; ++p) {
                a.pass_index = uint32_t(p);
                a.mode = ((p == 0 ? (mode | kModeFusedPrepare | extra_mode) : mode) & ~uint32_t(kModeSidesOnly)) | h->stream_mode;
                const int kind = p == 0 ? 0 : 1;
                size_t need = lds;
                if (p == 0) need = std::max(need, kFusedPrepareLdsBytes);
                if (p == 0 && (extra_mode & kModeFusedFactor)) need = std::max(need, kFusedFactorLdsBytes);
                size_t working = 0;
                for (size_t i = lo; i < hi; ++i) working += working_workgroups(side_form(h, *circs[eval_of(first + i)]));
                if (p == 0 && (extra_mode & kModeFusedFactor) && h->dtype == QSV_F64 && (h->fused_lds_table || any_halves) && working <= size_t(h->n_cus)) {
                    a.mode |= kModeFusedLdsTable;
                    need = std::max(need, kFusedLdsTableEnd);
                }
                if (p == 0 && (extra_mode & kModeFusedFactor) && h->side_prepare) a.mode |= kModeSidePrepare;
                if (p == 0 && any_reduced) a.mode |= kModeFusedReduced;
                if (p == 0 && any_reduced && h->live_entries) a.mode |= kModeFusedLive;
                if (h->stamping) QSV_HIP(h, stamp(h, h->batch.launch_events[kind], true));
                QSV_LAUNCH(h, launch_pass(h->dtype, r, h->cfg.xmode, dim3(grid_x, unsigned(hi - lo), 2), threads, need, ws(h), a));
                record_pass(h, r, dim3(grid_x, unsigned(hi - lo), 2), threads, need, a);
                if (h->stamping) QSV_HIP(h, stamp(h, h->batch.launch_events[kind], false));
                h->prof.n_pass_launches += 1;
                h->prof.kernel_launches[kind] += 1;
            }
            return QSV_OK;
        };
        int rc2;
        hipStream_t const lane_of_group = h->work;
        if (two_chains) h->work = chain_st;
        auto launch_sides_by_r = [&](size_t lo, size_t hi, uint32_t extra_mode) -> int {
            for (size_t at = lo; at < hi;) {
                const int r = side_form(h, *circs[eval_of(first + at)]).side_r == 3 ? 3 : h->geo.r;
                size_t end = at;
                bool halves_here = false;
                while (end < hi && (side_form(h, *circs[eval_of(first + end)]).side_r == 3 ? 3 : h->geo.r) == r) {
                    halves_here |= side_form(h, *circs[eval_of(first + end)]).halves;
                    ++end;
                }
                for (size_t from = at; from < end;) {
                    size_t to = end;
                    if (halves_here && (extra_mode & kModeFusedFactor)) {
                        size_t wg = 0;
                        for (to = from; to < end && wg + working_workgroups(side_form(h, *circs[eval_of(first + to)])) <= size_t(h->n_cus); ++to)
                            wg += working_workgroups(side_form(h, *circs[eval_of(first + to)]));
                        if (to == from) to = from + 1;
                    }
                    const int rc3 = launch_sides(from, to, extra_mode, r);
                    if (rc3) return rc3;
                    from = to;
                }
                at = end;
            }
            return QSV_OK;
        };
        if (n_unfused > 0 && (rc2 = launch_sides_by_r(0, n_unfused, 0u))) return rc2;
        h->work = lane_of_group;
        size_t n_halved = 0, all_working = 0;
        while (n_unfused + n_halved < n_split && side_form(h, *circs[eval_of(first + n_unfused + n_halved)]).halves) ++n_halved;
        for (size_t i = n_unfused; i < n_split; ++i) all_working += working_workgroups(side_form(h, *circs[eval_of(first + i)]));
        if (n_halved > 0 && n_unfused + n_halved < n_split && all_working > size_t(h->n_cus)) {
            if (b.chain_now && h->chain_stream != -1 && n_unfused == 0) h->work = chain_st;
            if ((rc2 = launch_sides_by_r(n_unfused, n_unfused + n_halved, kModeFusedFactor))) return rc2;
            h->work = lane_of_group;
            if ((rc2 = launch_sides_by_r(n_unfused + n_halved, n_split, kModeFusedFactor))) return rc2;
        } else if (n_split > n_unfused && (rc2 = launch_sides_by_r(n_unfused, n_split, kModeFusedFactor))) return rc2;
        a.mode = mode | h->stream_mode;
        for (size_t i = 0; i < n_split; ++i) {
            const SplitInfo& sp = side_form(h, *circs[eval_of(first + i)]);
            const uint64_t bytes = ((uint64_t(1) << sp.n_virtual[0]) + (uint64_t(1) << sp.n_virtual[1])) * h->amp_bytes;
            h->prof.state_bytes += bytes;
            h->prof.moved_bytes += bytes;
            h->prof.kernel_bytes[0] += bytes;
            h->prof.kernel_moved_bytes[0] += bytes;
        }
        for (size_t i = n_unfused; i < n_split; ++i) {
            const SplitInfo& sp = side_form(h, *circs[eval_of(first + i)]);
            for (int s = 0; s < 2; ++s) {
                const int side_bits = sp.n_virtual[s] - sp.n_keys;
                const uint64_t moved = (uint64_t(1) << sp.n_virtual[s]) * h->amp_bytes + (uint64_t(8) << side_bits);
                h->prof.kernel_bytes[0] += moved;
                h->prof.kernel_moved_bytes[0] += moved;
                h->prof.kernel_flops[0] += double(uint64_t(1) << side_bits) * double(1u << (2 * sp.n_keys)) * (side_bits / 2.0 + 5.0) * 2.0;
                h->prof.kernel_states[0] += 1;
                if (!sp.stats[s].pass_pairs.empty()) h->prof.kernel_flops[0] += 24.0 * sp.stats[s].pass_pairs[0];
            }
            h->prof.kernel_states[2] += 1;
        }
    }
    a.evals = batch_evals(h) + first + n_split;
    const bool direct = mode & kModeDirectResult;
    const bool fused = direct || (mode & kModeFusedPrepare);
    if (mode & kModeFinalProbs) a.partials = static_cast<double*>(h->d_scratch.ptr);
    if (fused) {
        a.mode |= kModeFusedPrepare;
        a.host_evals = descs_base(h) + first + n_split;
        a.evals_out = static_cast<EvalDesc*>(h->d_batch.ptr) + first + n_split;
        a.host_params = params_base(h);
        a.mats_out = static_cast<double*>(h->d_mats.ptr);
        a.result_out = h->out_target ? h->out_target : h->h_out;
    }
    for (int p = 0; p < max_passes && n_plain > 0; ++p) {
        const unsigned chunks_p = p == 0 ? chunks : chunks_later;
        a.tiles_per_block = (h->geo.blocks_per_state + chunks_p - 1) / chunks_p;
        dim3 grid(chunks_p, unsigned(n_plain));
        a.pass_index = uint32_t(p);
        {
            static const bool tile_major = getenv("QSV_TILE_MAJOR") && atoi(getenv("QSV_TILE_MAJOR")) != 0;
            const bool swap = tile_major && !(p == 0 && (mode & kModeSynthFirst)) && n_plain > 1;
            a.mode = swap ? (a.mode | kModeTileMajor) : (a.mode & ~uint32_t(kModeTileMajor));
            if (swap) grid = dim3(unsigned(n_plain), chunks_p);
        }
        const int kind = (p == 0 && (mode & kModeSynthFirst)) ? 0 : 1;
        if (h->stamping) QSV_HIP(h, stamp(h, h->batch.launch_events[kind], true));
        QSV_LAUNCH(h, launch_pass(h->dtype, h->geo.r, h->cfg.xmode, grid, h->geo.threads_launch,
                                  std::max(h->geo.lds_bytes, fused ? kFusedPrepareLdsBytes : size_t(0)), ws(h), a));
        record_pass(h, h->geo.r, grid, h->geo.threads_launch, std::max(h->geo.lds_bytes, fused ? kFusedPrepareLdsBytes : size_t(0)), a);
        if (h->stamping) QSV_HIP(h, stamp(h, h->batch.launch_events[kind], false));
        h->prof.n_pass_launches += 1;
        h->prof.n_state_passes += n_plain;
        h->prof.kernel_launches[kind] += 1;
        for (size_t i = n_split; i < count; ++i) {
            const PlanStats& st = circs[eval_of(first + i)]->plan.stats;
            if (p >= st.n_passes) continue;
            const bool reads = !(p == 0 && (mode & kModeSynthFirst));
            const bool writes = !(p + 1 == st.n_passes && !(mode & kModeFinalStore));
            const uint64_t table = (mode & kModeSynthFirst) && st.compact_bits >= 0
                                       ? (uint64_t(1) << (st.compact_bits + h->geo.k)) * h->amp_bytes
                                       : sweep;
            const uint64_t alg = (reads ? sweep : 0) + (writes ? sweep : 0);
            const uint64_t moved = (reads ? (p == 1 ? table : sweep) : 0) + (writes ? (p == 0 ? table : sweep) : 0);
            h->prof.state_bytes += alg;
            h->prof.moved_bytes += moved;
            h->prof.kernel_bytes[kind] += alg;
            h->prof.kernel_moved_bytes[kind] += moved;
            h->prof.kernel_states[kind] += 1;
            if (size_t(p) < st.pass_pairs.size()) h->prof.kernel_flops[kind] += 24.0 * st.pass_pairs[size_t(p)];
        }
    }
    if (any_split && !(mode & kModeSidesOnly) && factor_path(h)) {
      if (n_unfused > 0) {
        hipStream_t const lane_of_group = h->work;
        struct Restore {
            qsv_t* h;
            hipStream_t st;
            ~Restore() { h->work = st; }
        } restore{h, lane_of_group};
        if (two_chains) h->work = chain_st;
        int most_keys = 0;
        for (size_t i = 0; i < n_unfused; ++i) most_keys = std::max(most_keys, circs[eval_of(first + i)]->split.n_keys);
// ... 870 lines not shown
}


}

extern "C" {

const char* qsv_version(void) { return "libqsv 0.1.0 (gfx950)"; }

int qsv_debug_stamps(unsigned long long* out, int reset) {
    return qsv::read_stamps(out, reset) == hipSuccess ? QSV_OK : QSV_E_UNSUPPORTED;
}

int qsv_debug_timeline(unsigned long long* out, size_t max_words, unsigned int* n_records, int reset) {
    return qsv::read_timeline(out, max_words, n_records, reset) == hipSuccess ? QSV_OK : QSV_E_UNSUPPORTED;
}

int qsv_create(int n_qubits, int dtype, int device, const qsv_plan_config* cfg, qsv_t** out) {
    if (!out) return fail(nullptr, QSV_E_ARG, "out is null");
    *out = nullptr;
    if (dtype != QSV_F64 && dtype != QSV_F32) return fail(nullptr, QSV_E_ARG, "dtype must be QSV_F64 or QSV_F32");
    PlanConfig pc;
    Geometry geo;
    try {
        pc = resolve_config(cfg, dtype, n_qubits);
        geo = make_geometry(n_qubits, pc);
    } catch (const std::exception& e) {
        return fail(nullptr, QSV_E_ARG, e.what());
    }
    if (geo.threads_launch > 512) return fail(nullptr, QSV_E_ARG, "tile_bits - reg_bits must be <= 9");
    int n_dev = 0;
    hipError_t e = hipGetDeviceCount(&n_dev);
    if (e != hipSuccess || n_dev == 0)
        return fail(nullptr, QSV_E_DEVICE, std::string("no HIP device available: ") + hipGetErrorString(e));
    if (device < 0 || device >= n_dev) return fail(nullptr, QSV_E_ARG, "device index out of range");
    e = hipSetDevice(device);
    if (e != hipSuccess) return fail(nullptr, QSV_E_DEVICE, std::string("hipSetDevice: ") + hipGetErrorString(e));

    qsv_t* h = new qsv_t();
    h->n = n_qubits;
    h->dtype = dtype;
    h->device = device;
    h->cfg = pc;
    h->geo = geo;
    h->amp_bytes = size_t(pc.amp_bytes);
    const size_t state_bytes = (size_t(1) << n_qubits) * h->amp_bytes;
    int group = cfg && cfg->group > 0 ? cfg->group : 0;
    if (const char* env = getenv("QSV_GROUP")) group = atoi(env);
    if (group <= 0) {
        const size_t budget = size_t(2) << 30;
        group = int(std::max<size_t>(1, std::min<size_t>(256, budget / state_bytes)));
    }
    h->group = group;
    {
        const uint64_t tiles_per_launch = uint64_t(geo.blocks_per_state) * uint64_t(group);
        h->tiles_per_block = (tiles_per_launch >= 4096 && geo.blocks_per_state >= 2) ? 2 : 1;
    }
    h->tiles_per_block_later = h->tiles_per_block;
    if (const char* env = getenv("QSV_TILES_PER_BLOCK")) h->tiles_per_block = h->tiles_per_block_later = std::max(1, atoi(env));
    if (const char* env = getenv("QSV_TILES_PER_BLOCK_LATER")) h->tiles_per_block_later = std::max(1, atoi(env));
    auto bail = [&](hipError_t err, const char* what) {
        std::string msg = std::string(what) + ": " + hipGetErrorString(err);
        qsv_destroy(h);
        return fail(nullptr, QSV_E_DEVICE, msg);
    };
    if ((e = hipStreamCreateWithFlags(&h->stream, hipStreamNonBlocking)) != hipSuccess) return bail(e, "hipStreamCreate");
    h->own_stream = true;
    if (const char* env = getenv("QSV_SPLIT")) h->split_enabled = atoi(env) != 0;
    if (const char* env = getenv("QSV_SPLIT_SAMPLE")) h->split_sampling = atoi(env) != 0;
    if (const char* env = getenv("QSV_FACTOR")) h->factor_enabled = atoi(env) != 0;
    if (getenv("QSV_NO_FUSED_FACTOR")) h->fused_factor = false;
    if (const char* env = getenv("QSV_CHAIN_STREAM")) h->chain_enabled = atoi(env) != 0;
    if (const char* env = getenv("QSV_POLL")) h->poll_results = atoi(env) != 0;
    if (const char* env = getenv("QSV_REPEAT")) h->repeat_enabled = atoi(env) != 0;
    if (const char* env = getenv("QSV_REPLAY")) h->replay_enabled = atoi(env) != 0;
    if (const char* env = getenv("QSV_HOST_TIMING")) h->timing.on = atoi(env) != 0;
    if (const char* env = getenv("QSV_REPEAT_DESCS")) h->repeat_device_descs = atoi(env) != 0;
    if (const char* env = getenv("QSV_FUSED_LDS")) h->fused_lds_table = atoi(env) != 0;
    if (const char* env = getenv("QSV_SIDE_PREPARE")) h->side_prepare = atoi(env) != 0;
    if (const char* env = getenv("QSV_SIDE_DIAG")) h->side_diag = atoi(env) != 0;
    if (const char* env = getenv("QSV_SIDES_R3")) h->sides_r3 = atoi(env) != 0;
    if (const char* env = getenv("QSV_FINAL_CONTROLS")) h->final_controls = atoi(env) != 0;
    if (const char* env = getenv("QSV_LIVE_ENTRIES")) h->live_entries = atoi(env) != 0;
    {
        int cus = 0;
        if (hipDeviceGetAttribute(&cus, hipDeviceAttributeMultiprocessorCount, device) == hipSuccess && cus > 0) h->n_cus = cus;
        int grid_y = 0;
        if (hipDeviceGetAttribute(&grid_y, hipDeviceAttributeMaxGridDimY, device) == hipSuccess && grid_y > 0)
            h->max_grid_y = h->device_max_grid_y = grid_y;
    }
    {
        int large_bar = 0;
        if (hipDeviceGetAttribute(&large_bar, hipDeviceAttributeIsLargeBar, device) != hipSuccess) large_bar = 0;
        h->bar_ship = false;
        if (const char* env = getenv("QSV_BAR")) h->bar_ship = large_bar != 0 && atoi(env) != 0;
    }
    if (const char* env = getenv("QSV_SPLIT_MAX_KEYS")) h->split_max_keys = std::max(0, std::min(kMaxSplitKeys, atoi(env)));
    h->stream_mode = state_bytes > (size_t(256) << 20) ? uint32_t(kModeStreaming) : 0u;
    if (const char* env = getenv("QSV_STREAMING")) h->stream_mode = atoi(env) ? uint32_t(kModeStreaming) : 0u;
    if (const char* env = getenv("QSV_STREAMS")) h->n_streams = std::max(1, std::min(4, atoi(env)));
    for (int i = 1; i < std::max(2, h->n_streams); ++i) {
        hipStream_t st = nullptr;
        if ((e = hipStreamCreateWithFlags(&st, hipStreamNonBlocking)) != hipSuccess) return bail(e, "hipStreamCreate");
        h->side_streams.push_back(st);
    }
    h->n_lane_streams = int(h->side_streams.size());
    if ((e = hipEventCreateWithFlags(&h->ev_join, hipEventDisableTiming)) != hipSuccess) return bail(e, "hipEventCreate");
    if ((e = hipMalloc(&h->d_states.ptr, state_bytes * size_t(group))) != hipSuccess) return bail(e, "hipMalloc(states)");
    h->d_states.bytes = state_bytes * size_t(group);
    h->wtab_stride = std::min<uint64_t>(uint64_t(1) << n_qubits, uint64_t(1) << (geo.k + int(kMaxCompactBits)));
    if ((e = hipMalloc(&h->d_wtab.ptr, size_t(h->wtab_stride) * h->amp_bytes * size_t(group))) != hipSuccess)
        return bail(e, "hipMalloc(compact tables)");
    h->d_wtab.bytes = size_t(h->wtab_stride) * h->amp_bytes * size_t(group);
    if (h->split_enabled && n_qubits > geo.k && n_qubits <= 28) {
        h->side_stride = uint64_t(2) << (geo.k + kSideExtraBits);
        h->side_slots = 256;
        if (const char* env = getenv("QSV_SIDE_SLOTS")) h->side_slots = std::max(8, std::min(1024, atoi(env)));
        if ((e = hipMalloc(&h->d_side.ptr, size_t(h->side_stride) * h->amp_bytes * size_t(h->side_slots))) != hipSuccess)
            return bail(e, "hipMalloc(side tables)");
        h->d_side.bytes = size_t(h->side_stride) * h->amp_bytes * size_t(h->side_slots);
        if (h->factor_enabled) {
            const size_t bytes = factor_slot_doubles() * sizeof(double) * size_t(h->side_slots);
            if ((e = hipMalloc(&h->d_factor.ptr, bytes)) != hipSuccess) return bail(e, "hipMalloc(partial Gram matrices)");
            h->d_factor.bytes = bytes;
            const size_t cbytes = sizeof(uint32_t) * size_t(kFactorCountersPerSlot) * size_t(h->side_slots);
            if ((e = hipMalloc(&h->d_factor_count.ptr, cbytes)) != hipSuccess) return bail(e, "hipMalloc(hand-off counters)");
            h->d_factor_count.bytes = cbytes;
            if ((e = hipMemset(h->d_factor_count.ptr, 0, cbytes)) != hipSuccess) return bail(e, "hipMemset(hand-off counters)");
        }
    }
    {
        const int side_tile = std::max(geo.k, std::min(geo.r + 9, int(kMaxTileBits)));
        const size_t plane = (size_t(1) << side_tile) * h->amp_bytes / (pc.xmode == 2 ? 2 : 1);
        const size_t most = std::max({geo.lds_bytes, plane, kFusedPrepareLdsBytes, kFusedFactorLdsBytes, kFusedLdsTableEnd});
        if ((e = configure_pass_kernels(dtype, geo.r, pc.xmode, most)) != hipSuccess) return bail(e, "hipFuncSetAttribute");
        if (geo.r != 3 && (e = configure_pass_kernels(dtype, 3, pc.xmode, most)) != hipSuccess) return bail(e, "hipFuncSetAttribute");
    }
    *out = h;
    return QSV_OK;
}

void qsv_destroy(qsv_t* h) {
    if (!h) return;
    if (getenv("QSV_COALESCE_DEBUG") && h->cq_batches)
        fprintf(stderr, "qsv_eval_coalesced: %llu batches, last expectation %zu\n", (unsigned long long)h->cq_batches, h->cq_expected);
    if (h->timing.on && h->timing.calls) {
        const qsv_handle::HostTiming& t = h->timing;
        const double per = 1.0 / double(t.calls);
        fprintf(stderr,
                "qsv host timing over %llu qsv_eval_begin calls (%llu replayed pushes), us per call: begin %.2f  push without launch calls %.2f  "
                "launch calls %.2f  end and poll %.2f  copy-out %.2f\n",
                (unsigned long long)t.calls, (unsigned long long)t.replays, t.begin_us * per, (t.push_us - t.launch_us) * per,
                t.launch_us * per, (t.end_us - t.copy_us) * per, t.copy_us * per);
    }
    (void)hipSetDevice(h->device);
    if (h->stream) (void)hipStreamSynchronize(h->stream);
    for (hipStream_t st : h->side_streams) {
        (void)hipStreamSynchronize(st);
        (void)hipStreamDestroy(st);
    }
    if (h->ev_join) (void)hipEventDestroy(h->ev_join);
    for (DeviceBuffer* b : {&h->d_z, &h->d_cre, &h->d_diag, &h->d_order, &h->d_sorted, &h->d_term_partials, &h->d_groups, &h->d_term_odd, &h->d_arena,
                            &h->d_states, &h->d_wtab, &h->d_side, &h->d_factor, &h->d_factor_count, &h->d_factor_big, &h->d_factor_big_count, &h->d_quad, &h->d_fterms, &h->d_fpart, &h->d_batch, &h->d_mats, &h->d_partials, &h->d_out, &h->d_scratch, &h->d_prefix, &h->d_sdiag,
                            &h->d_obs_partials, &h->d_obs_values, &h->d_grad_tab, &h->d_grad_rows, &h->d_grad_values, &h->d_grad_base,
                            &h->d_grad_out, &h->d_adj_lambda, &h->d_adj_tab, &h->d_adj_mats, &h->d_adj_partials, &h->d_adj_epart, &h->d_adj_base,
                            &h->d_adj_out, &h->d_adj_values, &h->d_moments, &h->d_cov, &h->d_overlap})
// ... 330 lines not shown

int qsv_circuit_create_on_prefix(qsv_t* h, int prefix_id, int n_ops, const qsv_op* ops, int n_params, int* out_circuit_id) {
    const int64_t offsets[2] = {0, n_ops};
    return create_on_prefixes(h, "qsv_circuit_create_on_prefix", 1, offsets, ops, &n_params, &prefix_id, out_circuit_id);
}

static bool runs_reduced(const qsv_t* h, const Circuit& c) {
    return c.split.fused && c.reduced.ok && (h->n_terms == 0 ? h->fused_factor && h->final_controls : reduced_route(h));
}

static int circuit_cost_locked(qsv_t* h, int circuit_id, qsv_circuit_cost_t* out) {
    auto it = h->circuits.find(circuit_id);
    if (it == h->circuits.end()) return fail(h, QSV_E_ARG, "unknown circuit id");
    Circuit& c = it->second;
    *out = qsv_circuit_cost_t{};
    const double scale = std::ldexp(1.0, h->n - 20) * (h->dtype == QSV_F64 ? 1.0 : 0.5);
    if (split_rule(h, SplitUse::Expectation).takes(c)) {
        const bool one_launch = c.split.fused && h->fused_factor && (h->n_terms == 0 || factor_path(h));
        const SplitInfo& sp = one_launch && runs_reduced(h, c) ? c.reduced : c.split;
        out->route = one_launch ? QSV_ROUTE_SPLIT_ONE_LAUNCH : QSV_ROUTE_SPLIT;
        out->n_keys = sp.n_keys;
        out->n_passes = std::max(sp.stats[0].n_passes, sp.stats[1].n_passes);
        const double sides = 0.5 * (std::ldexp(1.0, sp.n_virtual[0] - sp.n_keys - 10) + std::ldexp(1.0, sp.n_virtual[1] - sp.n_keys - 10));
        const double per = one_launch ? 0.8 : (sp.n_keys <= 3 ? 1.2 : (sp.n_keys == 4 ? 5.0 : 9.0));
        out->microseconds = per * std::max(1.0, sides) * double(out->n_passes);
        return QSV_OK;
    }
    int rc = ensure_plan(h, c);
    if (rc) return rc;
    out->n_passes = c.plan.stats.n_passes;
    out->on_kept_state = c.prefix_id >= 0 ? 1 : 0;
    if (h->geo.blocks_per_state == 1) {
        out->route = QSV_ROUTE_ONE_TILE;
        out->microseconds = 1.0;
        return QSV_OK;
    }
    out->route = QSV_ROUTE_PASSES;
    {
        const bool synth = c.prefix_id < 0;
        const double moving = double(out->n_passes) - (synth ? 1.0 : 0.0);
        out->microseconds = (4.2 * std::max(0.0, moving) + 0.09 * double(c.plan.stats.n_real_gates) + (synth ? 1.0 : 0.0)) * scale;
    }
    return QSV_OK;
}

int qsv_circuit_cost(qsv_t* h, int circuit_id, qsv_circuit_cost_t* out) {
    if (!h) return QSV_E_ARG;
    if (!out) return fail(h, QSV_E_ARG, "out is null");
    QSV_OPEN(h, "qsv_circuit_cost", kHostOnly);
    return circuit_cost_locked(h, circuit_id, out);
}

static int circuit_form_of(qsv_t* h, int circuit_id, qsv_circuit_form_t* out, bool launched) {
    if (!h) return QSV_E_ARG;
    if (!out) return fail(h, QSV_E_ARG, "out is null");
    QSV_OPEN(h, launched ? "qsv_circuit_launch_form" : "qsv_circuit_form", kHostOnly);
    qsv_circuit_cost_t cost;
    int rc = circuit_cost_locked(h, circuit_id, &cost);
    if (rc) return rc;
    const Circuit& c = h->circuits.find(circuit_id)->second;
    *out = qsv_circuit_form_t{};
    out->route = cost.route;
    out->n_keys = cost.n_keys;
    if (!c.split.ok) return QSV_OK;
    const SplitInfo& sp = launched && cost.route == QSV_ROUTE_SPLIT_ONE_LAUNCH && runs_reduced(h, c) ? c.reduced : c.split;
    const uint32_t* blk = c.plan.words.data() + c.split.off_block;
    const int sx = (blk[kSplitFlags] & kSplitSwapXY) ? 1 : 0;
    for (int xy = 0; xy < 2; ++xy) {
        out->n_virtual[xy] = sp.n_virtual[xy == 0 ? sx : 1 - sx];
        out->outer[xy] = sp.outer[xy == 0 ? sx : 1 - sx];
    }
    out->amps_per_thread = 1 << sp.side_r;
    out->halves = sp.fused && sp.halves ? 1 : 0;
    out->one_launch = sp.fused ? 1 : 0;
    out->split_sampled = split_rule(h, SplitUse::Sampling).takes(c) ? 1 : 0;
    out->mask_x = blk[kSplitMaskX];
    out->mask_y = blk[kSplitMaskY];
    return QSV_OK;
}

int qsv_circuit_form(qsv_t* h, int circuit_id, qsv_circuit_form_t* out) { return circuit_form_of(h, circuit_id, out, false); }

int qsv_circuit_launch_form(qsv_t* h, int circuit_id, qsv_circuit_form_t* out) { return circuit_form_of(h, circuit_id, out, true); }

int qsv_eval_circuits(qsv_t* h, int n_evals, const int* circuit_ids, const int64_t* param_offsets, const double* params,
                      double* out) {
    QSV_OPEN(h, "qsv_eval_circuits", kDevice);
    if (n_evals < 0 || (n_evals > 0 && (!circuit_ids || !param_offsets || !out)))
        return fail(h, QSV_E_ARG, "bad arguments");
    BatchArgs args;
    int rc = resolve_batch(h, size_t(n_evals), circuit_ids, param_offsets, params, args);
    return rc ? rc : eval_all(h, args, out);
}

static void coalesce_lead(qsv_t* h, std::unique_lock<std::mutex>& lock, double window_us) {
    using clock = std::chrono::steady_clock;
    const double window = window_us > 0 ? window_us : 300.0;
    const double quiet = getenv("QSV_COALESCE_QUIET_US") ? atof(getenv("QSV_COALESCE_QUIET_US")) : 60.0;
    lock.unlock();
    const auto t0 = clock::now();
    auto last_arrival = t0;
    size_t seen = h->cq_count.load();
    for (;;) {
        const auto now = clock::now();
        const size_t count = h->cq_count.load();
        if (count != seen) {
            seen = count;
            last_arrival = now;
        }
        const double since_start = std::chrono::duration<double, std::micro>(now - t0).count();
        const double since_arrival = std::chrono::duration<double, std::micro>(now - last_arrival).count();
        if ((h->cq_expected > 1 && count >= h->cq_expected) || since_arrival >= quiet || since_start >= window) break;
        __builtin_ia32_pause();
    }
    lock.lock();
    std::vector<qsv_handle::CoalesceRequest*> batch;
    batch.swap(h->cq);
    h->cq_count.store(0);
    lock.unlock();
    {
        std::lock_guard<std::mutex> hl(h->mu);
        BatchArgs args;
        std::vector<qsv_handle::CoalesceRequest*> valid;
        for (auto* r : batch) {
            auto it = h->circuits.find(r->circuit_id);
            if (it == h->circuits.end() || r->n_params < it->second.n_params) {
                r->rc = QSV_E_ARG;
                r->err = it == h->circuits.end() ? "unknown circuit id " + std::to_string(r->circuit_id)
                                                 : "circuit needs " + std::to_string(it->second.n_params) + " parameter values";
                continue;
            }
            args.circs.push_back(&it->second);
            args.n_params.push_back(r->n_params);
            args.values.insert(args.values.end(), r->params, r->params + r->n_params);
            valid.push_back(r);
        }
        if (!valid.empty()) {
            std::vector<double> values(valid.size(), 0.0);
            args.values.push_back(0.0);
            int rc = hipSetDevice(h->device) == hipSuccess ? QSV_OK : QSV_E_DEVICE;
            if (!rc) rc = eval_all(h, args, values.data());
            const std::string err = rc ? g_handle_error : std::string();
            for (size_t i = 0; i < valid.size(); ++i) {
                valid[i]->rc = rc;
                valid[i]->err = err;
                valid[i]->value = values[i];
            }
        }
    }
    lock.lock();
    h->cq_expected = std::max(batch.size(), h->cq_expected * 7 / 8);
    h->cq_batches += 1;
    for (auto* r : batch) r->done = true;
    h->cq_collecting = false;
    h->cq_cv.notify_all();
}

int qsv_eval_coalesced(qsv_t* h, int circuit_id, const double* params, int n_params, double window_us, double* out) {
    if (!h) return QSV_E_ARG;
    if (!out || n_params < 0 || (n_params > 0 && !params)) return fail(h, QSV_E_ARG, "bad arguments");
    if (h->batch_owner.load() == std::this_thread::get_id()) return refuse_in_batch(h, "qsv_eval_coalesced");
    qsv_handle::CoalesceRequest req;
    req.circuit_id = circuit_id;
    req.params = params;
    req.n_params = n_params;
    std::unique_lock<std::mutex> lock(h->cq_mu);
// ... 1651 lines not shown
    if ((rc = run_whole_states(h, args, G, tiles, d_s, out_count))) return rc;
    const size_t row = K * 2;
    for (size_t j = 0; j < n; ++j) {
        const size_t e = h->batch.eval_at[j];
        std::copy(h->h_out + j * row, h->h_out + (j + 1) * row, out_overlaps + e * row);
        if (op) std::copy(h->h_out + tile_count + j * row, h->h_out + tile_count + (j + 1) * row, out_elements + e * row);
    }
    return QSV_OK;
}

int qsv_sample(qsv_t* h, int circuit_id, const double* params, int n_params, int shots, uint64_t seed,
               uint64_t* out_states) {
    QSV_OPEN(h, "qsv_sample", kDevice);
    if (shots < 0 || n_params < 0 || (shots > 0 && !out_states)) return fail(h, QSV_E_ARG, "bad arguments");
    const int64_t offsets[2] = {0, n_params};
    BatchArgs args;
    int rc = resolve_batch(h, 1, &circuit_id, offsets, params, args, shots ? kNotSampled : nullptr);
    return rc ? rc : sample_batch_locked(h, args, shots, seed, out_states, nullptr);
}

int qsv_fitness_table_wait(const volatile uint64_t* own, int count, volatile int64_t* done, int stride, int world, int rank,
                           int64_t step, int budget_us) {
    if (!own || !done || count < 0 || world < 1 || rank < 0 || rank >= world || stride < 1) return QSV_E_ARG;
    const auto deadline = std::chrono::steady_clock::now() + std::chrono::microseconds(budget_us);
    auto expired = [&](unsigned& spins) {
        __builtin_ia32_pause();
        return (++spins & 255u) == 0 && std::chrono::steady_clock::now() > deadline;
    };
    unsigned spins = 0;
    for (int i = 0; i < count;) {
        if (own[i] != QSV_TABLE_SENTINEL)
            ++i;
        else if (expired(spins))
            return 1;
    }
    __atomic_store_n(&done[size_t(rank) * size_t(stride)], step, __ATOMIC_RELEASE);
    for (int r = 0; r < world;) {
        if (__atomic_load_n(&done[size_t(r) * size_t(stride)], __ATOMIC_ACQUIRE) >= step)
            ++r;
        else if (expired(spins))
            return 2;
    }
    return 0;
}

int qsv_set_option(qsv_t* h, const char* name, int value) {
    if (!h) return QSV_E_ARG;
    if (!name) return fail(h, QSV_E_ARG, "option name is null");
    QSV_OPEN(h, "qsv_set_option", kHostOnly);
    h->epoch += 1;
    const std::string key(name);
    if (key == "split") {
        if (value != 0 && !h->d_side.ptr && h->n > h->geo.k && h->n <= 28)
            return fail(h, QSV_E_ARG, "this handle was created without side tables (QSV_SPLIT=0): splitting cannot be switched on");
        h->split_enabled = value != 0;
    } else if (key == "factor") {
        if (value != 0 && h->split_enabled && h->d_side.ptr && !h->d_factor.ptr)
            return fail(h, QSV_E_ARG, "this handle was created without the factorised path (QSV_FACTOR=0)");
        h->factor_enabled = value != 0;
    } else if (key == "fused_factor") {
        h->fused_factor = value != 0;
    } else if (key == "chain_stream") {
        h->chain_enabled = value != 0;
    } else if (key == "poll_results") {
        h->poll_results = value != 0;
    } else if (key == "repeat_layout") {
        h->repeat_enabled = value != 0;
    } else if (key == "replay_launches") {
        h->replay_enabled = value != 0;
    } else if (key == "split_max_keys") {
        if (value < 0 || value > kMaxSplitKeys) return fail(h, QSV_E_ARG, "split_max_keys must be between 0 and 5");
        h->split_max_keys = value;
    } else if (key == "split_sampling") {
        h->split_sampling = value != 0;
    } else if (key == "fused_lds_table") {
        h->fused_lds_table = value != 0;
    } else if (key == "side_prepare") {
        h->side_prepare = value != 0;
    } else if (key == "final_controls") {
        h->final_controls = value != 0;
        h->epoch += 1;
    } else if (key == "live_entries") {
        h->live_entries = value != 0;
    } else if (key == "sides_r3") {
        h->sides_r3 = value != 0;
    } else if (key == "side_diag") {
        if (h->side_diag != (value != 0)) {
            QSV_HIP(h, sync_streams(h));
            for (auto& kv : h->circuits) kv.second.uploaded = false;
            h->sdiag_used = 0;
        }
        h->side_diag = value != 0;
    } else if (key == "streams") {
        if (value < 1 || value > h->n_lane_streams + 1) return fail(h, QSV_E_ARG, "streams must be between 1 and the number the handle was created with");
        h->n_streams = value;
    } else if (key == "max_grid_y") {
        if (value < 0 || value > h->device_max_grid_y) return fail(h, QSV_E_ARG, "max_grid_y must be between 0 and the device's largest gridDim.y");
        h->max_grid_y = value ? value : h->device_max_grid_y;
    } else if (key == "gradient_chunk") {
        if (value < 0 || value > (1 << 20)) return fail(h, QSV_E_ARG, "gradient_chunk must be between 0 and 1048576");
        h->grad_chunk = value ? value : kGradientChunkRows;
    } else if (key == "time_moments") {
        h->time_moments = value != 0;
    } else {
        return fail(h, QSV_E_ARG, "unknown option '" + key + "'");
    }
    return QSV_OK;
}

int qsv_set_profiling(qsv_t* h, int enabled) {
    QSV_OPEN(h, "qsv_set_profiling", kHostOnly);
    h->epoch += 1;
    h->profiling = enabled != 0;
    return QSV_OK;
}

int qsv_live_entries(int n_keys, unsigned key_mask, int* out_pi) {
    if (n_keys != 3 || key_mask > 7u || !out_pi) return QSV_E_ARG;
    for (int i = 0; i < 64; ++i) out_pi[i] = -1;
    int count = 0;
    for (uint32_t pi = 0; pi < 64; ++pi) {
        uint32_t rank = 0;
        if (!live_entry(key_mask, pi, &rank)) continue;
        out_pi[rank] = int(pi);
        ++count;
    }
    return count;
}

long long qsv_replayed_pushes(const qsv_t* h) {
    QSV_OPEN(h, "qsv_replayed_pushes", kHostOnly);
    return (long long)h->replayed_pushes;
}

int qsv_get_profile(const qsv_t* h, qsv_profile* out) {
    if (!out) return QSV_E_ARG;
    QSV_OPEN(h, "qsv_get_profile", kHostOnly);
    *out = h->prof;
    return QSV_OK;
}

static int bench_ops_locked(qsv_t* h, int n_ops, const qsv_op* ops, int reps, double* out_ms_per_rep,
                            int* out_n_passes) {
    if (!out_ms_per_rep || reps < 1) return fail(h, QSV_E_ARG, "bad arguments");
    int id = 0;
    int rc = register_circuit(h, n_ops, ops, 0, &id, false);
    if (rc) return rc;
    Circuit& c = h->circuits.find(id)->second;
    auto cleanup = [&]() { h->circuits.erase(id); };
    std::vector<Circuit*> cc{&c};
    if ((rc = batch_layout(h, cc, std::vector<int64_t>{0})) || (rc = batch_ship(h, 0, 1, kNoValues))) {
        h->batch.circs.clear();
        cleanup();
        return rc;
    }
    h->batch.circs.clear();
    PassArgs a{};
    a.plan = static_cast<const uint32_t*>(h->d_arena.ptr);
    a.mats = static_cast<const double*>(h->d_mats.ptr);
    a.evals = batch_evals(h);
    a.states = h->d_states.ptr;
    a.wtab = h->d_wtab.ptr;
    a.wtab_stride = h->wtab_stride;
    a.state_stride = uint64_t(1) << h->n;
    a.mode = kModeFinalStore | h->stream_mode;
    const unsigned chunks = chunks_per_state(h);
    a.tiles_per_block = (h->geo.blocks_per_state + chunks - 1) / chunks;
    dim3 grid(chunks, 1);
    const int n_passes = c.plan.stats.n_passes;
    auto sweep = [&]() -> hipError_t {
        for (int p = 0; p < n_passes; ++p) {
            a.pass_index = uint32_t(p);
            hipError_t e = launch_pass(h->dtype, h->geo.r, h->cfg.xmode, grid, h->geo.threads_launch, h->geo.lds_bytes, h->stream, a);
            if (e != hipSuccess) return e;
        }
        return hipSuccess;
    };
    hipEvent_t e0, e1;
    QSV_HIP(h, hipEventCreate(&e0));
    QSV_HIP(h, hipEventCreate(&e1));
    QSV_HIP(h, sweep());
    QSV_HIP(h, hipEventRecord(e0, h->stream));
    for (int i = 0; i < reps; ++i) QSV_HIP(h, sweep());
    QSV_HIP(h, hipEventRecord(e1, h->stream));
    QSV_HIP(h, hipStreamSynchronize(h->stream));
    float ms = 0.f;
    QSV_HIP(h, hipEventElapsedTime(&ms, e0, e1));
    (void)hipEventDestroy(e0);
    (void)hipEventDestroy(e1);
    *out_ms_per_rep = double(ms) / reps;
    if (out_n_passes) *out_n_passes = n_passes;
    cleanup();
    return QSV_OK;
}

int qsv_bench_ops(qsv_t* h, int n_ops, const qsv_op* ops, int reps, double* out_ms_per_rep, int* out_n_passes) {
    QSV_OPEN(h, "qsv_bench_ops", kDevice);
    for (int i = 0; i < n_ops; ++i)
        if (ops && ops[i].kind != QSV_OP_ID && (ops[i].p_theta >= 0 || ops[i].p_phi >= 0 || ops[i].p_lambda >= 0))
            return fail(h, QSV_E_ARG, "qsv_bench_ops needs bound (literal) angles");
    return bench_ops_locked(h, n_ops, ops, reps, out_ms_per_rep, out_n_passes);
}

int qsv_bench_gate(qsv_t* h, int target, int control, double theta, double phi, double lambda, int reps,
                   double* out_ms_per_sweep) {
    QSV_OPEN(h, "qsv_bench_gate", kDevice);
    if (target < 0 || target >= h->n || control >= h->n) return fail(h, QSV_E_ARG, "qubit out of range");
    qsv_op op{};
    op.kind = control >= 0 ? QSV_OP_CU3 : QSV_OP_U;
    op.target = uint8_t(target);
    op.control = control >= 0 ? uint8_t(control) : uint8_t(QSV_NO_CONTROL);
    op.p_theta = op.p_phi = op.p_lambda = -1;
    op.theta = theta;
    op.phi = phi;
    op.lambda = lambda;
    return bench_ops_locked(h, 1, &op, reps, out_ms_per_sweep, nullptr);
}

int qsv_split_describe(int n_qubits, int n_ops, const qsv_op* ops, int max_side, uint64_t* mask_a, qsv_op* ops_a,
                       int capacity_a, int* n_ops_a, qsv_op* ops_b, int capacity_b, int* n_ops_b) {
    if (!mask_a || !n_ops_a || !n_ops_b) return fail(nullptr, QSV_E_ARG, "null output") - 100;
    if (n_qubits < 1 || n_qubits > 32) return fail(nullptr, QSV_E_ARG, "n_qubits must be in [1, 32]") - 100;
    if (validate_ops(nullptr, n_qubits, n_ops, ops, 1 << 30)) return QSV_E_ARG - 100;
    std::vector<AngleSource> angles;
    const std::vector<GateIn> gates = gates_of(ops, n_ops, &angles);
    const SplitCircuits sc = find_split(n_qubits, gates, angles, max_side);
    if (!sc.ok) return -1;
    *mask_a = sc.mask[0];
    qsv_op* outs[2] = {ops_a, ops_b};
    const int caps[2] = {capacity_a, capacity_b};
    int* counts[2] = {n_ops_a, n_ops_b};
    for (int s = 0; s < 2; ++s) {
        *counts[s] = int(sc.gates[s].size());
        if (!outs[s] || caps[s] < *counts[s]) continue;
        for (size_t i = 0; i < sc.gates[s].size(); ++i) {
            const GateIn& g = sc.gates[s][i];
            const AngleSource& a = sc.angles[s][size_t(g.op)];
            qsv_op o{};
            o.kind = g.control < 0 ? QSV_OP_U : QSV_OP_CU3;
            o.target = uint8_t(g.target);
            o.control = g.control < 0 ? uint8_t(QSV_NO_CONTROL) : uint8_t(g.control);
            o.p_theta = a.p_theta; o.p_phi = a.p_phi; o.p_lambda = a.p_lambda;
            o.theta = a.theta; o.phi = a.phi; o.lambda = a.lambda;
            outs[s][i] = o;
        }
    }
    return sc.n_keys;
}
// ... 65 lines not shown
```

Baseline: 1.673 million circuit-evals/s.

## Merge lane-controlled multiplexed gate pairs into one entry in the asm round loop

Adds a generated assembly round loop for fp64, exchange mode 2, R=3 that spots two consecutive plan entries forming a multiplexed gate on a lane control. It applies them as a single pass, choosing the per-lane matrix through exec-masked VGPR moves. This halves the passes over the register-held amplitudes for such pairs and cuts the scalar branch overhead. It is enabled by default through a new mode bit, adds 16 clobbered VGPRs that may raise register pressure, and adds a side-plan query API.

```diff
diff --git a/include/qsv.h b/include/qsv.h
--- a/include/qsv.h
+++ b/include/qsv.h
@@ -106,6 +106,7 @@
 } qsv_circuit_form_t;
 int qsv_circuit_form(qsv_t* h, int circuit_id, qsv_circuit_form_t* out);
 int qsv_circuit_launch_form(qsv_t* h, int circuit_id, qsv_circuit_form_t* out);
+int qsv_circuit_side_plan(qsv_t* h, int circuit_id, int side, uint32_t* out_words, size_t capacity_words, size_t* n_words);
 
 int qsv_eval_circuits(qsv_t* h, int n_evals, const int* circuit_ids, const int64_t* param_offsets,
                       const double* params, double* out_expectations);
diff --git a/queasars_amd/_build.py b/queasars_amd/_build.py
--- a/queasars_amd/_build.py
+++ b/queasars_amd/_build.py
@@ -11,7 +11,7 @@
 LIB_PATH = PKG_DIR / "libqsv.so"
 PYHELP_PATH = PKG_DIR / "_qsvpyhelp.so"
 SOURCES = ["kernels.hip", "qsv_api.hip", "plan.cpp", "split.cpp", "sort.hip", "gradient.hip", "value_cache.hip", "adjoint.hip", "adjoint_plan.cpp", "moments.hip", "covariance.hip", "overlap.hip"]
-HEADERS = ["kernels.hpp", "plan.hpp", "split.hpp", "gradient.hpp", "value_cache.hpp", "adjoint.hpp", "adjoint_plan.hpp", "moments.hpp", "covariance.hpp", "overlap.hpp", "operator_row.hpp", "gate_loop_gen.inc", "../../include/qsv.h"]
+HEADERS = ["kernels.hpp", "plan.hpp", "split.hpp", "gradient.hpp", "value_cache.hpp", "adjoint.hpp", "adjoint_plan.hpp", "moments.hpp", "covariance.hpp", "overlap.hpp", "operator_row.hpp", "gate_loop_gen.inc", "gate_loop_merge_gen.inc", "../../include/qsv.h"]
 ARCH = "gfx950"
 
 
@@ -58,7 +58,22 @@
     return PYHELP_PATH
 
 
+def generate_merge_loops(force: bool = False) -> None:
+    import importlib.util
+
+    src, out = CSRC / "gen_gate_loop.py", CSRC / "gate_loop_merge_gen.inc"
+    if not force and out.exists() and out.stat().st_mtime >= src.stat().st_mtime:
+        return
+    spec = importlib.util.spec_from_file_location("qsv_gen_gate_loop", src)
+    gen = importlib.util.module_from_spec(spec)
+    spec.loader.exec_module(gen)
+    if gen.ABL:
+        raise RuntimeError("QSV_GEN_ABL is set: the library is built with the variable unset")
+    gen.write_merge(out)
+
+
 def needs_build() -> bool:
+    generate_merge_loops()
     if not LIB_PATH.exists():
         return True
     built = LIB_PATH.stat().st_mtime
@@ -69,6 +84,7 @@
     if not force and not defines and not needs_build():
         build_pyhelp(False)
         return LIB_PATH
+    generate_merge_loops()
     obj_dir = PKG_DIR / ("build" if not defines else "build_" + "".join(c if c.isalnum() else "_" for c in "_".join(defines).lower()))
     obj_dir.mkdir(exist_ok=True)
     hipcc = _hipcc()
diff --git a/queasars_amd/_lib.py b/queasars_amd/_lib.py
--- a/queasars_amd/_lib.py
+++ b/queasars_amd/_lib.py
@@ -232,6 +232,7 @@
     "qsv_circuit_cost": (C.c_int, [_P, C.c_int, C.POINTER(QsvCircuitCost)]),
     "qsv_circuit_form": (C.c_int, [_P, C.c_int, C.POINTER(QsvCircuitForm)]),
     "qsv_circuit_launch_form": (C.c_int, [_P, C.c_int, C.POINTER(QsvCircuitForm)]),
+    "qsv_circuit_side_plan": (C.c_int, [_P, C.c_int, C.c_int, _P, C.c_size_t, C.POINTER(C.c_size_t)]),
     "qsv_eval_circuits": (C.c_int, [_P, C.c_int, _P, _P, _P, _P]),
     "qsv_eval_coalesced": (C.c_int, [_P, C.c_int, _P, C.c_int, C.c_double, C.POINTER(C.c_double)]),
     "qsv_eval_begin": (C.c_int, [_P, C.c_int, _P, _P]),
diff --git a/queasars_amd/circuit_evaluation/circuit_evaluation.py b/queasars_amd/circuit_evaluation/circuit_evaluation.py
--- a/queasars_amd/circuit_evaluation/circuit_evaluation.py
+++ b/queasars_amd/circuit_evaluation/circuit_evaluation.py
@@ -517,6 +517,16 @@
 
     def circuit_launch_form(self, circuit: CircuitIR) -> dict:
         return self._form(self._lib.qsv_circuit_launch_form, circuit)
+
+    def circuit_side_plan(self, circuit: CircuitIR, side: int):
+        import numpy as np
+
+        cid, n_words = self.circuit_id(circuit), C.c_size_t(0)
+        self._check(self._lib.qsv_circuit_side_plan(self._handle, cid, side, None, 0, C.byref(n_words)))
+        words = np.zeros(n_words.value, dtype=np.uint32)
+        if words.size:
+            self._check(self._lib.qsv_circuit_side_plan(self._handle, cid, side, _lib.as_ptr(words), words.size, C.byref(n_words)))
+        return words
 
     def _form(self, call, circuit: CircuitIR) -> dict:
         form = _lib.QsvCircuitForm()
diff --git a/queasars_amd/csrc/gen_gate_loop.py b/queasars_amd/csrc/gen_gate_loop.py
--- a/queasars_amd/csrc/gen_gate_loop.py
+++ b/queasars_amd/csrc/gen_gate_loop.py
@@ -6,6 +6,7 @@
 from pathlib import Path
 
 OUT = Path(__file__).resolve().parent / "gate_loop_gen.inc"
+MERGE_OUT = Path(__file__).resolve().parent / "gate_loop_merge_gen.inc"
 
 import os
 
@@ -46,18 +47,30 @@
 
 def gate(lines: list[str], r: int, x: str, tag: str) -> None:
     m, d = MAT[x], DESC[x]
-    w0, ct, cg = f"s{d}", f"s{d + 1}", f"s{d + 2}"
+    w0, ct = f"s{d}", f"s{d + 1}"
     cgpair = sreg2(d + 2)
-    m00, m00i, m01r, m01i = sreg2(m), sreg2(m + 2), sreg2(m + 4), sreg2(m + 6)
-    m10r, m10i, m11r, m11i = sreg2(m + 8), sreg2(m + 10), sreg2(m + 12), sreg2(m + 14)
     e = lines.append
     e(f"s_and_b64 {TP}, {BASEP}, {cgpair}")
     e(f"s_cmp_eq_u64 {TP}, {cgpair}")
     e(f"s_cbranch_scc0 Lskip{tag}_%=")
+    gate_lanes(lines, r, w0, ct, [sreg2(m + 2 * i) for i in range(8)], tag)
+    e(f"Lskip{tag}_%=:")
+
+
+def gate_lanes(lines: list[str], r: int, w0: str, ct: str, mat: list[str], tag: str) -> None:
+    e = lines.append
     e(f"v_and_b32 %[vt], {ct}, %[tid]")
     e(f"v_cmp_eq_u32 vcc, {ct}, %[vt]")
     e(f"s_and_saveexec_b64 {SAVE}, vcc")
     e(f"s_cbranch_execz Lrest{tag}_%=")
+    pair_updates(lines, r, w0, mat, tag)
+    e(f"Lrest{tag}_%=:")
+    e(f"s_mov_b64 exec, {SAVE}")
+
+
+def pair_updates(lines: list[str], r: int, w0: str, mat: list[str], tag: str) -> None:
+    m00, m00i, m01r, m01i, m10r, m10i, m11r, m11i = mat
+    e = lines.append
     e(f"s_bitcmp1_b32 {w0}, 24")
     e(f"s_cbranch_scc1 Lgen{tag}_%=")
     for general in (False, True):
@@ -107,9 +120,6 @@
                 pair += 1
             if not (general and pos + 1 == len(order)):
                 e(f"s_branch Lrest{tag}_%=")
-    e(f"Lrest{tag}_%=:")
-    e(f"s_mov_b64 exec, {SAVE}")
-    e(f"Lskip{tag}_%=:")
 
 
 def loop_body(r: int) -> list[str]:
@@ -275,7 +285,114 @@
 K_THREAD_COLS = 9
 
 
-def emit_rounds(r: int) -> str:
+WIN = 72
+CW0, CCT = 98, 99
+MSEL = 100
+K_GENERAL, K_NEGATED, K_MAX_THREAD_BITS = 1 << 24, 1 << 25, 9
+MERGE_CLOBBERS = range(40, 101)
+MERGE_R = (3,)
+MERGE_FLAG_BIT = 2
+
+
+def gate_loop_core_merge(lines: list[str], r: int) -> None:
+    rp, mp = sreg2(RP), sreg2(MP)
+    n = f"s{N}"
+    win = f"s[{WIN}:{WIN + 7}]"
+    w0, ct, cgpair = f"s{WIN}", f"s{WIN + 1}", sreg2(WIN + 2)
+    nw0, nct, ncgpair = f"s{WIN + 4}", f"s{WIN + 5}", sreg2(WIN + 6)
+    mv0 = AMP0 + 4 * (1 << r)
+    mv = [f"v[{mv0 + 2 * i}:{mv0 + 2 * i + 1}]" for i in range(8)]
+    e = lines.append
+
+    def advance(entries: int) -> None:
+        e(f"s_add_u32 s{RP}, s{RP}, {16 * entries}")
+        e(f"s_addc_u32 s{RP + 1}, s{RP + 1}, 0")
+        e(f"s_add_u32 s{MP}, s{MP}, {64 * entries}")
+        e(f"s_addc_u32 s{MP + 1}, s{MP + 1}, 0")
+
+    a0 = MAT["A"]
+    e(f"s_load_dwordx8 {win}, {rp}, 0x0")
+    e(f"s_load_dwordx16 s[{a0}:{a0 + 15}], {mp}, 0x0")
+    for x, other in (("A", "B"), ("B", "A")):
+        tag = x.lower()
+        m, o = MAT[x], MAT[other]
+        e(f"Lloop{tag}_%=:")
+        e("s_waitcnt lgkmcnt(0)")
+        e(f"s_xor_b32 {T0}, {w0}, {nw0}")
+        e(f"s_andn2_b32 {T0}, {T0}, {hex(K_GENERAL)}")
+        e(f"s_cmp_eq_u32 {T0}, s{MSEL}")
+        e(f"s_cbranch_scc1 Lpair{tag}_%=")
+        e(f"Lsingle{tag}_%=:")
+        e(f"s_mov_b64 s[{CW0}:{CCT}], s[{WIN}:{WIN + 1}]")
+        e(f"s_and_b64 {TP}, {BASEP}, {cgpair}")
+        e(f"s_cmp_eq_u64 {TP}, {cgpair}")
+        e(f"s_load_dwordx8 {win}, {rp}, 0x10")
+        e(f"s_load_dwordx16 s[{o}:{o + 15}], {mp}, 0x40")
+        e(f"s_cbranch_scc0 Lskip{tag}_%=")
+        gate_lanes(lines, r, f"s{CW0}", f"s{CCT}", [sreg2(m + 2 * i) for i in range(8)], tag)
+        e(f"Lskip{tag}_%=:")
+        advance(1)
+        e(f"s_sub_u32 {n}, {n}, 1")
+        e(f"s_cmp_eq_u32 {n}, 0")
+        if x == "A":
+            e("s_cbranch_scc1 Ldone_%=")
+        else:
+            e("s_cbranch_scc0 Lloopa_%=")
+            e("s_branch Ldone_%=")
+    for x, other in (("A", "B"), ("B", "A")):
+        tag = x.lower()
+        m, o = MAT[x], MAT[other]
+        e(f"Lpair{tag}_%=:")
+        e(f"s_bitcmp1_b32 {nw0}, 25")
+        e(f"s_cbranch_scc0 Lsingle{tag}_%=")
+        e(f"s_cmp_lt_u32 {n}, 2")
+        e(f"s_cbranch_scc1 Lsingle{tag}_%=")
+        e(f"s_bfe_u32 {T0}, {w0}, 0x80008")
+        e(f"s_cmp_eq_u32 {T0}, 0xff")
+        e(f"s_cbranch_scc0 Lsingle{tag}_%=")
+        e(f"s_or_b64 {TP}, {cgpair}, {ncgpair}")
+        e(f"s_cbranch_scc1 Lsingle{tag}_%=")
+        e(f"s_cmp_lt_u32 {ct}, 64")
+        e(f"s_cbranch_scc0 Lsingle{tag}_%=")
+        e(f"s_bcnt1_i32_b32 {T0}, {ct}")
+        e(f"s_cmp_eq_u32 {T0}, 1")
+        e(f"s_cbranch_scc0 Lsingle{tag}_%=")
+        e(f"s_lshl_b32 {T0}, {ct}, {K_MAX_THREAD_BITS}")
+        e(f"s_cmp_eq_u32 {T0}, {nct}")
+        e(f"s_cbranch_scc0 Lsingle{tag}_%=")
+        e(f"s_load_dwordx16 s[{o}:{o + 15}], {mp}, 0x40")
+        e(f"v_and_b32 %[vt], {ct}, %[tid]")
+        e(f"v_cmp_ne_u32 vcc, {ct}, %[vt]")
+        for i in range(8):
+            e(f"v_mov_b32 v{mv0 + 2 * i}, s{m + 2 * i}")
+            e(f"v_mov_b32 v{mv0 + 2 * i + 1}, s{m + 2 * i + 1}")
+        e("s_waitcnt lgkmcnt(0)")
+        e(f"s_and_saveexec_b64 {SAVE}, vcc")
+        for i in range(8):
+            e(f"v_mov_b32 v{mv0 + 2 * i}, s{o + 2 * i}")
+            e(f"v_mov_b32 v{mv0 + 2 * i + 1}, s{o + 2 * i + 1}")
+        e(f"s_mov_b64 exec, {SAVE}")
+        e(f"s_or_b32 s{CW0}, {w0}, {nw0}")
+        e(f"s_mov_b32 s{CCT}, {0 if x == 'A' else 1}")
+        e(f"s_load_dwordx8 {win}, {rp}, 0x20")
+        e(f"s_load_dwordx16 s[{m}:{m + 15}], {mp}, 0x80")
+        if x == "A":
+            e("s_branch Lmbody_%=")
+    e("Lmbody_%=:")
+    pair_updates(lines, r, f"s{CW0}", mv, "m")
+    e("Lrestm_%=:")
+    advance(2)
+    e(f"s_sub_u32 {n}, {n}, 2")
+    e(f"s_cmp_eq_u32 {n}, 0")
+    e("s_cbranch_scc1 Ldone_%=")
+    e(f"s_cmp_eq_u32 s{CCT}, 0")
+    e("s_cbranch_scc1 Lloopa_%=")
+    e("s_branch Lloopb_%=")
+    e("Ldone_%=:")
+    e("s_waitcnt lgkmcnt(0)")
+
+
+def emit_rounds(r: int, merge: bool = False) -> str:
     nr = 1 << r
     rp, mp = sreg2(RP), sreg2(MP)
     lines: list[str] = []
@@ -286,6 +403,9 @@
     e(f"s_mov_b32 s{FLAGS}, %[flags]")
     e("s_mov_b32 s96, %[base]")
     e("s_not_b32 s97, %[base]")
+    if merge:
+        e(f"s_bitcmp1_b32 s{FLAGS}, {MERGE_FLAG_BIT}")
+        e(f"s_cselect_b32 s{MSEL}, {hex(K_NEGATED)}, -1")
     e("Lround_%=:")
     e(f"s_load_dword s{RH}, {rp}, 0x0")
     e("s_waitcnt lgkmcnt(0)")
@@ -306,7 +426,7 @@
     e(f"s_add_u32 s94, s{MP}, s{T1}")
     e(f"s_addc_u32 s95, s{MP + 1}, 0")
     if "gateloop" not in ABL:
-        gate_loop_core(lines, r)
+        (gate_loop_core_merge if merge else gate_loop_core)(lines, r)
     e(f"s_mov_b64 {rp}, {NEXT_RP}")
     e(f"s_mov_b64 {mp}, {NEXT_MP}")
     e("Lnext_%=:")
@@ -426,9 +546,10 @@
     e(f"s_mov_b32 %[flags], s{FLAGS}")
 
     out = []
-    out.append(f"// R = {r}: every round of a tile (LDS exchanges in mode 2, lane swaps, gates)")
+    out.append(f"// R = {r}: every round of a tile (LDS exchanges in mode 2, lane swaps, gates" + (
+        "; a multiplexed gate on a lane control as ONE entry)" if merge else ")"))
     out.append("template <>")
-    out.append(f"struct RoundLoopF64<{r}> {{")
+    out.append(f"struct {'RoundLoopMergeF64' if merge else 'RoundLoopF64'}<{r}> {{")
     out.append(
         f"    static __device__ __forceinline__ void run(cx<double> (&amp)[{nr}], cu32p rp, cf64p mp, uint32_t n_rounds,\n"
         "                                               uint32_t base, uint32_t tid, uint32_t wave, uint64_t active,\n"
@@ -450,7 +571,9 @@
     out.append("            : " + ",\n              ".join(outs))
     out.append('            : [rp] "s"(rp), [mp] "s"(mp), [rounds] "s"(n_rounds), [base] "s"(base), [tid] "v"(tid), [wave] "s"(wave),\n'
                '              [active] "s"(active), [lds] "s"(lds), [lane] "v"(tid & 63u)')
-    clob = ['"vcc"', '"scc"', '"memory"'] + [f'"s{i}"' for i in ROUND_CLOBBERS]
+    clob = ['"vcc"', '"scc"', '"memory"'] + [f'"s{i}"' for i in (MERGE_CLOBBERS if merge else ROUND_CLOBBERS)]
+    if merge:
+        clob += [f'"v{AMP0 + 4 * nr + i}"' for i in range(16)]
     rows = [", ".join(clob[i : i + 12]) for i in range(0, len(clob), 12)]
     out.append("            : " + ",\n              ".join(rows) + ");")
     out.append("        flags = fl;")
@@ -805,7 +928,32 @@
             + rounds32_head + "\n\n".join(emit_rounds32(r) for r in (1, 2, 3, 4)) + "\n")
 
 
+def render_merge() -> str:
+    head = (
+        "// GENERATED by gen_gate_loop.py at build time -- not committed, do not edit.\n"
+        "// The round loop of a tile (exchange mode 2) that runs a multiplexed gate on a lane control as ONE entry, see gen_gate_loop.py.\n"
+        "// Included inside namespace qsv by kernels.hip, behind gate_loop_gen.inc.\n\n"
+        "template <int R>\nstruct RoundLoopMergeF64;  // specialised below for R = " + ", ".join(str(r) for r in MERGE_R) + "\n\n"
+    )
+    return head + "\n\n".join(emit_rounds(r, True) for r in MERGE_R) + "\n"
+
+
+def write_merge(out: Path = MERGE_OUT) -> bool:
+    text = render_merge()
+    if out.exists() and out.read_text() == text:
+        return False
+    tmp = out.with_suffix(f".inc.{os.getpid()}.tmp")
+    tmp.write_text(text)
+    os.replace(tmp, out)
+    return True
+
+
 if __name__ == "__main__":
+    if len(sys.argv) > 1 and sys.argv[1] == "--merge":
+        if ABL:
+            sys.exit("QSV_GEN_ABL is set: the merging loops are generated with the variable unset")
+        print(f"{MERGE_OUT}: {'written' if write_merge() else 'up to date'}")
+        sys.exit(0)
     text = render()
     if len(sys.argv) > 1 and sys.argv[1] == "--check":
         sys.exit(0 if OUT.exists() and OUT.read_text() == text else 1)
diff --git a/queasars_amd/csrc/kernels.hip b/queasars_amd/csrc/kernels.hip
--- a/queasars_amd/csrc/kernels.hip
+++ b/queasars_amd/csrc/kernels.hip
@@ -129,6 +129,7 @@
 #include QSV_GATE_LOOP_INC
 #else
 #include "gate_loop_gen.inc"
+#include "gate_loop_merge_gen.inc"
 #endif
 
 template <int U>
@@ -795,6 +796,7 @@
     constexpr int ASH = Log2Size<real>::value + 1;
     constexpr int LSH = XMODE == 0 ? ASH : ASH - 1;
     extern __shared__ __align__(16) unsigned char lds_raw[];
+    constexpr bool kMergeLanes = FUSED && std::is_same<real, double>::value && XMODE == 2 && R == 3;
 
     QSV_STAMP_DECL
 #ifdef QSV_ABL_EMPTY
@@ -976,7 +978,7 @@
     }
     cxr amp[NR];
     double acc = 0.0;
-    uint32_t xflags = 0;
+    uint32_t xflags = kMergeLanes && (a.mode & kModeMergeLaneMux) ? 4u : 0u;
     const uint64_t active_mask = __ballot(active);
     bool lds_dirty = false;
     bool cross_pending = false;
@@ -1117,6 +1119,10 @@
         if constexpr (kAsmRounds) {
             if (n_rounds > 0) {
                 if constexpr (std::is_same<real, double>::value)
+                    if constexpr (kMergeLanes)
+                        RoundLoopMergeF64<R>::run(amp, rp, mp, uint32_t(n_rounds), uint32_t(base), tid_ext, wave, active_mask,
+                                                  uint32_t(uintptr_t(lds_raw)), xflags);
+                    else
                     RoundLoopF64<R>::run(amp, rp, mp, uint32_t(n_rounds), uint32_t(base), tid_ext, wave, active_mask,
                                          uint32_t(uintptr_t(lds_raw)), xflags);
                 else
diff --git a/queasars_amd/csrc/kernels.hpp b/queasars_amd/csrc/kernels.hpp
--- a/queasars_amd/csrc/kernels.hpp
+++ b/queasars_amd/csrc/kernels.hpp
@@ -47,6 +47,7 @@
     kModeSidePrepare = 4096u,
     kModeFusedReduced = 8192u,
     kModeFusedLive = 16384u,
+    kModeMergeLaneMux = 32768u,
 };
 inline __host__ __device__ void live_entry_rows(uint32_t pi, uint32_t* ja_out, uint32_t* jb_out) {
     uint32_t ja = pi, jb = pi;
diff --git a/queasars_amd/csrc/qsv_api.hip b/queasars_amd/csrc/qsv_api.hip
--- a/queasars_amd/csrc/qsv_api.hip
+++ b/queasars_amd/csrc/qsv_api.hip
@@ -245,6 +245,7 @@
     bool side_diag = true;
     bool final_controls = true;
     bool live_entries = true;
+    bool merge_lane_mux = true;
     bool sides_r3 = true;
     size_t prefix_slots = 0;
     std::vector<uint32_t> prefix_free;
@@ -1095,6 +1096,7 @@
     if (h->batch.dev_params) return h->batch.dev_params;
     return reinterpret_cast<const double*>(static_cast<const char*>(h->h_batch) + h->batch.desc_bytes);
 }
+uint32_t launch_mode(const qsv_t* h) { return h->stream_mode | (h->merge_lane_mux ? uint32_t(kModeMergeLaneMux) : 0u); }
 
 double* result_base(const qsv_t* h) { return h->out_target ? h->out_target : h->h_out; }
 
@@ -1406,7 +1408,7 @@
     a.diag = static_cast<const double*>(h->d_diag.ptr);
     a.partials = static_cast<double*>(h->d_partials.ptr);
     a.state_stride = uint64_t(1) << h->n;
-    a.mode = mode | h->stream_mode;
+    a.mode = mode | launch_mode(h);
     a.prefix_states = h->d_prefix.ptr;
     a.side_diag = static_cast<const double*>(h->d_sdiag.ptr);
     {
@@ -1476,7 +1478,7 @@
             a.evals_out = static_cast<EvalDesc*>(h->d_batch.ptr) + first + lo;
             for (int p = 0; p < passes; ++p) {
                 a.pass_index = uint32_t(p);
-                a.mode = ((p == 0 ? (mode | kModeFusedPrepare | extra_mode) : mode) & ~uint32_t(kModeSidesOnly)) | h->stream_mode;
+                a.mode = ((p == 0 ? (mode | kModeFusedPrepare | extra_mode) : mode) & ~uint32_t(kModeSidesOnly)) | launch_mode(h);
                 const int kind = p == 0 ? 0 : 1;
                 size_t need = lds;
                 if (p == 0) need = std::max(need, kFusedPrepareLdsBytes);
@@ -1538,7 +1540,7 @@
             h->work = lane_of_group;
             if ((rc2 = launch_sides_by_r(n_unfused + n_halved, n_split, kModeFusedFactor))) return rc2;
         } else if (n_split > n_unfused && (rc2 = launch_sides_by_r(n_unfused, n_split, kModeFusedFactor))) return rc2;
-        a.mode = mode | h->stream_mode;
+        a.mode = mode | launch_mode(h);
         for (size_t i = 0; i < n_split; ++i) {
             const SplitInfo& sp = side_form(h, *circs[eval_of(first + i)]);
             const uint64_t bytes = ((uint64_t(1) << sp.n_virtual[0]) + (uint64_t(1) << sp.n_virtual[1])) * h->amp_bytes;
@@ -2575,6 +2577,7 @@
     if (const char* env = getenv("QSV_SIDES_R3")) h->sides_r3 = atoi(env) != 0;
     if (const char* env = getenv("QSV_FINAL_CONTROLS")) h->final_controls = atoi(env) != 0;
     if (const char* env = getenv("QSV_LIVE_ENTRIES")) h->live_entries = atoi(env) != 0;
+    if (const char* env = getenv("QSV_MERGE_LANE_MUX")) h->merge_lane_mux = atoi(env) != 0;
     {
         int cus = 0;
         if (hipDeviceGetAttribute(&cus, hipDeviceAttributeMultiprocessorCount, device) == hipSuccess && cus > 0) h->n_cus = cus;
@@ -3071,6 +3074,24 @@
 int qsv_circuit_form(qsv_t* h, int circuit_id, qsv_circuit_form_t* out) { return circuit_form_of(h, circuit_id, out, false); }
 
 int qsv_circuit_launch_form(qsv_t* h, int circuit_id, qsv_circuit_form_t* out) { return circuit_form_of(h, circuit_id, out, true); }
+
+int qsv_circuit_side_plan(qsv_t* h, int circuit_id, int side, uint32_t* out_words, size_t capacity_words, size_t* n_words) {
+    if (!h) return QSV_E_ARG;
+    if (!n_words || side < 0 || side > 1) return fail(h, QSV_E_ARG, "bad arguments");
+    QSV_OPEN(h, "qsv_circuit_side_plan", kHostOnly);
+    qsv_circuit_cost_t cost;
+    int rc = circuit_cost_locked(h, circuit_id, &cost);
+    if (rc) return rc;
+    const Circuit& c = h->circuits.find(circuit_id)->second;
+    *n_words = 0;
+    if (!c.split.ok) return QSV_OK;
+    const SplitInfo& sp = cost.route == QSV_ROUTE_SPLIT_ONE_LAUNCH && runs_reduced(h, c) ? c.reduced : c.split;
+    const uint32_t* blk = c.plan.words.data() + c.split.off_block;
+    const int s = ((blk[kSplitFlags] & kSplitSwapXY) ? 1 : 0) ^ side;
+    *n_words = c.plan.words.size() - sp.off_side[s];
+    if (out_words && capacity_words >= *n_words) std::memcpy(out_words, c.plan.words.data() + sp.off_side[s], *n_words * 4);
+    return QSV_OK;
+}
 
 int qsv_eval_circuits(qsv_t* h, int n_evals, const int* circuit_ids, const int64_t* param_offsets, const double* params,
                       double* out) {
@@ -4888,6 +4909,8 @@
         h->epoch += 1;
     } else if (key == "live_entries") {
         h->live_entries = value != 0;
+    } else if (key == "merge_lane_mux") {
+        h->merge_lane_mux = value != 0;
     } else if (key == "sides_r3") {
         h->sides_r3 = value != 0;
     } else if (key == "side_diag") {
@@ -4969,7 +4992,7 @@
     a.wtab = h->d_wtab.ptr;
     a.wtab_stride = h->wtab_stride;
     a.state_stride = uint64_t(1) << h->n;
-    a.mode = kModeFinalStore | h->stream_mode;
+    a.mode = kModeFinalStore | launch_mode(h);
     const unsigned chunks = chunks_per_state(h);
     a.tiles_per_block = (h->geo.blocks_per_state + chunks - 1) / chunks;
     dim3 grid(chunks, 1);
```

After: 1.669 million circuit-evals/s. No clear change (-0.2%).
